# NVIDIA/makani

Measured on AMD Instinct MI355X. Metric: SFNO train samples/sec at 721x1440x73ch, higher is better.
Workload: dtype bf16; 1 GPU; sfno_sc3_layers8_edim384; grid=721x1440, channels=73, global_batch=1, parallelism=dp1, spectral_arithmetic=x3, multistep_count=1, multistep_checkpoint=False, launch=hipGraph replay of the captured step, channel_gemm=hip (csrc/conv1x1.hip)

## Files before the change

include/makani_amd.h:

```cpp
#ifndef MAKANI_AMD_H
#define MAKANI_AMD_H

#ifdef __cplusplus
extern "C" {
#endif

#define MK_F32 0
#define MK_BF16 1

#define MK_EINVAL -1
#define MK_EUNSUP -2

#define MK_TRI_NONE 0
#define MK_TRI_ROW_GE 1
#define MK_TRI_K_GE 2
#define MK_TRI_ROW_LE 3
#define MK_TRI_K_LE 4

typedef struct MkGemm {
    const float* A;
    const float* B;
    float* C;
    long long a_batch, a_row, a_k;
    long long b_batch, b_col, b_k;
    long long c_batch, c_row, c_col;
    long long a_inner, b_inner, c_inner;
    long long a_im, b_im, c_im;
    int M, N, K, batch;
    int inner;
    int tri_mode;
    int tri_off;
    int conj_a, conj_b;
    int beta;
} MkGemm;

const char* mk_last_error(void);
int mk_version(void);

int mk_sgemm_batched(const MkGemm* g, void* stream);
int mk_cgemm_batched(const MkGemm* g, void* stream);
int mk_sgemm_split_batched(const MkGemm* g, int limbs, void* stream);
int mk_cgemm_split_batched(const MkGemm* g, int limbs, void* stream);
int mk_cgemm_split2_batched(const MkGemm* g, int limbs, void* stream);
long long mk_cgemm_split2_ssq_count(const MkGemm* g);
int mk_cgemm_split2_batched_ssq(const MkGemm* g, int limbs, float* ssq_part, void* stream);
int mk_sgemm_presplit_batched(const MkGemm* g, const void* a_planes, long long pl_stride, long long pl_batch,
                              long long pl_k, int limbs, const int* band_lo, const int* band_hi, int band_mode,
                              void* stream);

int mk_vlegendre(const void* planes0, const void* planes1, long long pl_stride, long long pl_batch, long long pl_k,
                 int limbs, const float* in, float* out, int mode, int rows, int K, int orders, int Rp, int tri_off,
                 const int* band_lo, const int* band_hi, void* stream);

int mk_rfft_rows(const void* x, int x_dtype, float* F, const float* twiddle, const int* radix, int nradix,
                 int B, int C, int Cp, int nlat, int nlon, int mmax, float w_dc, float w_pos, float w_nyq,
                 void* stream);
int mk_irfft_rows(const float* F, void* x, int x_dtype, const float* twiddle, const int* radix, int nradix,
                  int B, int C, int Cp, int nlat, int nlon, int mmax, float w_dc, float w_pos, float w_nyq,
                  void* stream);

#define MK_FFT_SEG_MAX 8
typedef struct MkFftSeg {
    int nw, nh;
    int m_off[MK_FFT_SEG_MAX + 1];
    int r_off[MK_FFT_SEG_MAX + 1];
    long long base[MK_FFT_SEG_MAX][MK_FFT_SEG_MAX];
    int xseg;
    long long x_stride;
    int x_nlat;
} MkFftSeg;
int mk_fft_seg_supported(int nlon);
int mk_rfft_rows_seg(const void* x, int x_dtype, float* F, const float* twiddle, int C, int nlat, int nlon, int mmax,
                     float w_dc, float w_pos, float w_nyq, const MkFftSeg* seg, void* stream);
int mk_irfft_rows_seg(const float* F, void* x, int x_dtype, const float* twiddle, int C, int nlat, int nlon, int mmax,
                      float w_dc, float w_pos, float w_nyq, const MkFftSeg* seg, void* stream);

int mk_weight_to_wlayout(const float* w_c64, float* W, int cin, int cout, int cip, int cop, int L, void* stream);
int mk_wlayout_to_weight_grad(const float* gW, float* gw_c64, int cin, int cout, int cip, int cop, int L, void* stream);
int mk_slayout_to_complex(const float* S, float* out_c64, int B, int C, int Cp, int L, int M, int l_off, int m_off,
                          void* stream);
int mk_complex_to_slayout(const float* in_c64, float* S, int B, int C, int Cp, int L, int M, void* stream);

int mk_pointwise_chunks(long long hw, int dtype, long long planes);
int mk_plane_sums(const void* x, int dtype, float* sums, float* ws, long long planes, long long hw, void* stream);
int mk_instnorm_stats(const void* x, int dtype, float* stats, float* ws, long long planes, long long hw, float eps,
                      const float* quad, float quad_sum, void* stream);
int mk_instnorm_merge(const float* all_stats, const float* counts, float* stats, long long planes, int nranks, float eps,
                      void* stream);
int mk_instnorm_apply(const void* x, void* y, int dtype, const float* stats, const float* gamma, const float* beta,
                      long long planes, int channels, long long hw, int fuse_gelu, void* stream);
int mk_instnorm_fwd(const void* x, void* y, int dtype, float* stats, float* ws, const float* gamma, const float* beta,
                    const float* pre_bias, const float* quad, float quad_sum, long long planes, int channels, long long hw,
                    float eps, int fuse_gelu, void* stream);
int mk_instnorm_bwd(const void* x, const void* gy, void* gx, int dtype, const float* stats, const float* gamma,
                    const float* beta, const float* pre_bias, const float* quad, float quad_sum, float* sums, float* ws, long long planes, int channels, long long hw,
                    long long hw_total, int phase, int fuse_gelu, void* stream);
int mk_instnorm_fused_chunks(long long hw, int dtype, long long planes, int kind);
int mk_instnorm_fwd_fused(const void* x, void* y, int dtype, float* stats, const float* gamma, const float* beta,
                          const float* pre_bias, void* slots, void* depart, long long planes, int channels, long long hw,
                          float eps, int fuse_gelu, void* stream);
int mk_instnorm_bwd_fused(const void* x, const void* gy, void* gx, int dtype, const float* stats, const float* gamma,
                          const float* beta, const float* pre_bias, float* sums, void* slots, void* depart, long long planes,
                          int channels, long long hw, int fuse_gelu, void* stream);
int mk_bias_gelu_fwd(const void* x, const float* bias, void* y, int dtype, long long planes, int channels,
                     long long hw, void* stream);
int mk_bias_gelu_bwd(const void* x, const float* bias, const void* gy, void* gx, float* sums, float* ws, int dtype,
                     long long planes, int channels, long long hw, void* stream);

int mk_quad_lp_chunks(long long hw);
int mk_quad_lp_fwd(const void* a, int a_dtype, const void* b, int b_dtype, const float* wgt, const float* q,
                   float* sums, float* ws, long long planes, long long hw, int mode, float p, void* stream);
int mk_quad_lp_bwd(const void* a, int a_dtype, const void* b, int b_dtype, const float* wgt, const float* q,
                   const float* g, void* da, void* db, long long planes, long long hw, int mode, float p, void* stream);

long long mk_spec_lp_blocks(int L, int M);
int mk_spec_lp_fwd(const float* S, const float* wgt, float* partial, int L, int M, long long R, int tri_off, int m_off,
                   float p, float w0, float w1, void* stream);
int mk_spec_lp_bwd(const float* S, const float* wgt, const float* g, float* dS, int L, int M, long long R, int tri_off,
                   int m_off, float p, float w0, float w1, void* stream);

int mk_spec_sep_mul(const float* x, const float* w, float* y, int L, int M, int Mw, int B, int Cp, int tri_off, int conj_w,
                    void* stream);
int mk_spec_sep_wgrad(const float* x, const float* gy, float* gw, int L, int M, int Mw, int B, int Cp, int tri_off, void* stream);
int mk_spec_diag_apply(const float* x, const float* w_c64, float* y, int L, int M, int B, int Cin, int Cout, int x_ld, int y_ld,
                       int y_pad, int tri_off, int dgrad, void* stream);
int mk_spec_diag_wgrad(const float* x, const float* gy, float* gw_c64, int L, int M, int B, int Cin, int Cout, int x_ld, int y_ld,
                       int tri_off, void* stream);

int mk_conv1x1_nn(const void* A, const void* X, void* Y, void* Ypre, const float* bias, const void* R, const void* G,
                  int M, int K, int lda, int B, long long N, int act, void* stream);
long long mk_conv1x1_wgrad_workspace(int M, int K, int B, long long N);
int mk_conv1x1_wgrad(const void* G, const void* X, float* dW, float* part, int M, int K, int B, long long N,
                     int accumulate, void* stream);
int mk_conv1x1_wgrad_fuses_bias(int M, int K, int B, long long N);
int mk_conv1x1_wgrad_bias(const void* G, const void* X, float* dW, float* dbias, float* part, int M, int K, int B, long long N,
                          int accumulate, void* stream);

int mk_adamw_step(float* p, const float* g, float* m, float* v, long long n, const float* grad_scale, float lr,
                  float beta1, float beta2, float eps, float weight_decay, int step, const float* step_state, void* stream);
int mk_adamw_advance(float* state, float beta1, float beta2, void* stream);
typedef struct MkAdamTensor {
    float* p;
    const float* g;
    float* m;
    float* v;
    long long n;
    void* p_bf16;
    void* p_bf16_t;
    int cols;
    int ld, ld_t;
} MkAdamTensor;
int mk_adamw_multi(const MkAdamTensor* tensors, int count, const float* grad_scale, float lr, float beta1, float beta2,
                   float eps, float weight_decay, int step, const float* step_state, void* stream);
long long mk_grad_norm_workspace(const MkAdamTensor* tensors, int count);
int mk_grad_clip_coef(const MkAdamTensor* tensors, int count, float max_norm, float* partial, float* out, void* stream);
long long mk_grad_norm_workspace_pre(const MkAdamTensor* tensors, int count, const MkAdamTensor* pre, int npre);
int mk_grad_clip_coef_pre(const MkAdamTensor* tensors, int count, const MkAdamTensor* pre, int npre, float max_norm, float* partial,
                          float* out, void* stream);

int mk_chan_layernorm_chunks(int C, long long P);
int mk_chan_layernorm_fwd(const void* x, int x_dtype, void* y, int y_dtype, float* stats, const float* gamma, const float* beta,
                          int B, int C, long long P, float eps, void* stream);
int mk_chan_layernorm_bwd(const void* x, int x_dtype, const void* gy, int g_dtype, void* gx, const float* stats,
                          const float* gamma, int B, int C, long long P, void* stream);
int mk_chan_layernorm_wgrad(const void* x, int x_dtype, const void* gy, int g_dtype, const float* stats, float* partial, int B,
                            int C, long long P, void* stream);

int mk_crps_chunks(long long hw);
int mk_crps(const void* f, int f_dtype, const void* obs, int o_dtype, const float* q, const float* w, const float* gout,
            float* partial, void* gf, int B, int E, int C, long long hw, int type, float alpha, float eps, int grad,
            const float* ens_w, void* stream);
int mk_crps_complex(const void* f, const void* obs, const float* q, const float* w, const float* gout, float* partial, void* gf,
                    int B, int E, int C, long long hw, float alpha, int grad, void* stream);

long long mk_escore_sums_workspace(int B, int E, int C, long long N, int S, int nanmode);
int mk_escore_sums(const void* f, int kind, const void* obs, const float* q, const float* w, float* sums, float* ws, int B, int E,
                   int C, long long N, int S, int nanmode, float p, void* stream);
int mk_escore_finish(const float* sums, const float* scale, int nscale, float* loss, float* table, int B, int E, int C, int S,
                     int reduce, float p, float beta, float alpha, float eps, void* stream);
int mk_escore_grad(const void* f, int kind, const void* obs, const float* q, const float* w, const float* table, const float* gout,
                   void* gf, int B, int E, int C, int Cout, long long N, int S, int nanmode, float p, void* stream);

int mk_mmd_finish(const float* sums, float* loss, float* table, int B, int E, int C, int reduce, float sigma, float alpha, void* stream);

int mk_amse_sums(const float* X, const float* Y, const float* wgt, float* sums, long long R, int L, int M, int tri_off, int m_off,
                 void* stream);
int mk_amse_grad(const float* X, const float* Y, const float* wgt, const float* t, float* dX, float* dY, long long R, int L, int M,
                 int tri_off, int m_off, void* stream);

int mk_ens_nll_chunks(long long hw);
int mk_ens_nll(const void* f, int f_dtype, const float* obs, const float* q, const float* w, const float* gout, float* partial, void* gf,
               int B, int E, int C, long long hw, float eps, int grad, void* stream);

#define MK_NOISE_WHITE 0
#define MK_NOISE_AR 1
#define MK_NOISE_REPLACE 2
int mk_noise_update(float* state, const float* xi, const float* sigma, const float* phi, const long long* rng, int mode, int B,
                    int T, int C, int L, int M, int reflect, void* stream);
int mk_noise_advance(long long* rng, long long n, void* stream);

int mk_disco_fwd(const void* x, void* y, int dtype, const int* off, const int* nrow, const int* nlon, const float* nval,
                 const int* lat_lo, const int* lat_n, int max_rows, int planes, int K, int nlat_in, int nlon_in,
                 int nlat_out, int nlon_out, void* stream);
int mk_disco_bwd(const void* gy, void* gx, int dtype, const int* off, const int* nk, const int* nt, const int* nlon,
                 const float* nval, int planes, int K, int nlat_in, int nlon_in, int nlat_out, int nlon_out, void* stream);
int mk_disco_bwd_same(const void* gy, void* gx, int dtype, const int* off, const int* nrow, const int* nlon_l,
                      const float* nval, const int* t_lo, const int* t_n, int max_rows, int planes, int K, int nlat_in,
                      int nlon, int nlat_out, void* stream);
int mk_disco_runs_shape(int nlon, int max_rows, int planes, int dtype, int img_bf16, int* R_out, int* PB_out);
int mk_disco_fused_shape(int nlon, int K, int max_rows, int planes, int* LG_out, int* PB_out);
int mk_disco_fwd_fused(const void* x, void* y, int dtype, const int* seg_off, const int* runs, const float* vals,
                       const int* lat_lo, const int* lat_n, int max_rows, int planes, int K, int nlat_in, int nlon, int nlat_out,
                       void* stream);
int mk_disco_fwd_runs(const void* x, void* y, int dtype, const int* seg_off, const int* runs, const float* vals,
                      const int* lat_lo, const int* lat_n, int max_rows, int planes, int K, int nlat_in, int nlon, int nlat_out,
                      int R, int PB, int img_bf16, void* stream);
int mk_disco_bwd_runs(const void* gy, void* gx, int dtype, const int* seg_off, const int* runs, const float* vals,
                      const int* t_lo, const int* t_n, int max_rows, int planes, int K, int nlat_in, int nlon, int nlat_out,
                      int R, int PB, int img_bf16, int lat_group, void* stream);
int mk_group_mix_supported(int CG, int RG);
int mk_group_mix_blocks(long long N, int dtype, int BG);
int mk_group_mix(const void* x, const float* W, void* z, int dtype, int B, int G, int CG, int RG, long long N, void* stream);
int mk_group_mix_wgrad(const void* x, const void* dz, float* partial, int dtype, int B, int G, int CG, int RG, long long N,
                       void* stream);
int mk_resample_fwd(const void* x, void* y, int dtype, const int* lat_a, const int* lat_b, const float* lat_w,
                    const int* lon_l, const int* lon_r, const float* lon_w, int planes, int nlat_in, int nlon_in,
                    int nlat_out, int nlon_out, void* stream);
int mk_resample_bwd(const void* gy, void* gx, int dtype, const int* lat_off, const int* lat_t, const float* lat_wt,
                    const int* lon_off, const int* lon_p, const float* lon_wt, const int* pole_off, const int* pole_t,
                    const float* pole_wt, int planes, int nlat_in, int nlon_in, int nlat_out, int nlon_out, void* stream);

#ifdef __cplusplus
}
#endif
#endif
```

makani_amd/_lib.py:

```python
import ctypes as C
import os

import torch

_HERE = os.path.dirname(os.path.abspath(__file__))
LIB_PATH = os.environ.get("MAKANI_AMD_LIB") or os.path.join(_HERE, "libmakani_amd.so")

MK_F32, MK_BF16 = 0, 1
TRI_NONE, TRI_ROW_GE, TRI_K_GE, TRI_ROW_LE, TRI_K_LE = 0, 1, 2, 3, 4

c_ll, c_int, c_f, c_vp = C.c_longlong, C.c_int, C.c_float, C.c_void_p


class MkAdamTensor(C.Structure):
    _fields_ = [("p", C.c_void_p), ("g", C.c_void_p), ("m", C.c_void_p), ("v", C.c_void_p), ("n", C.c_longlong),
                ("p_bf16", C.c_void_p), ("p_bf16_t", C.c_void_p), ("cols", C.c_int), ("ld", C.c_int), ("ld_t", C.c_int)]


class MkGemm(C.Structure):
    _fields_ = [
        ("A", c_vp), ("B", c_vp), ("C", c_vp),
        ("a_batch", c_ll), ("a_row", c_ll), ("a_k", c_ll),
        ("b_batch", c_ll), ("b_col", c_ll), ("b_k", c_ll),
        ("c_batch", c_ll), ("c_row", c_ll), ("c_col", c_ll),
        ("a_inner", c_ll), ("b_inner", c_ll), ("c_inner", c_ll),
        ("a_im", c_ll), ("b_im", c_ll), ("c_im", c_ll),
        ("M", c_int), ("N", c_int), ("K", c_int), ("batch", c_int),
        ("inner", c_int), ("tri_mode", c_int), ("tri_off", c_int),
        ("conj_a", c_int), ("conj_b", c_int), ("beta", c_int),
    ]


MK_FFT_SEG_MAX = 8


class MkFftSeg(C.Structure):
    _fields_ = [("nw", c_int), ("nh", c_int), ("m_off", c_int * (MK_FFT_SEG_MAX + 1)), ("r_off", c_int * (MK_FFT_SEG_MAX + 1)),
                ("base", (c_ll * MK_FFT_SEG_MAX) * MK_FFT_SEG_MAX), ("xseg", c_int), ("x_stride", c_ll), ("x_nlat", c_int)]


_SIGS = {
    "mk_version": ([], c_int),
    "mk_sgemm_batched": ([C.POINTER(MkGemm), c_vp], c_int),
    "mk_cgemm_batched": ([C.POINTER(MkGemm), c_vp], c_int),
    "mk_sgemm_split_batched": ([C.POINTER(MkGemm), c_int, c_vp], c_int),
    "mk_cgemm_split_batched": ([C.POINTER(MkGemm), c_int, c_vp], c_int),
    "mk_cgemm_split2_batched": ([C.POINTER(MkGemm), c_int, c_vp], c_int),
    "mk_cgemm_split2_ssq_count": ([C.POINTER(MkGemm)], c_ll),
    "mk_cgemm_split2_batched_ssq": ([C.POINTER(MkGemm), c_int, c_vp, c_vp], c_int),
    "mk_sgemm_presplit_batched": ([C.POINTER(MkGemm), c_vp, c_ll, c_ll, c_ll, c_int, c_vp, c_vp, c_int, c_vp], c_int),
    "mk_vlegendre": ([c_vp, c_vp, c_ll, c_ll, c_ll, c_int, c_vp, c_vp, c_int, c_int, c_int, c_int, c_int, c_int, c_vp, c_vp, c_vp], c_int),
    "mk_rfft_rows": ([c_vp, c_int, c_vp, c_vp, C.POINTER(c_int), c_int, c_int, c_int, c_int, c_int, c_int, c_int,
                      c_f, c_f, c_f, c_vp], c_int),
    "mk_irfft_rows": ([c_vp, c_vp, c_int, c_vp, C.POINTER(c_int), c_int, c_int, c_int, c_int, c_int, c_int, c_int,
                       c_f, c_f, c_f, c_vp], c_int),
    "mk_fft_seg_supported": ([c_int], c_int),
    "mk_rfft_rows_seg": ([c_vp, c_int, c_vp, c_vp, c_int, c_int, c_int, c_int, c_f, c_f, c_f, C.POINTER(MkFftSeg), c_vp], c_int),
    "mk_irfft_rows_seg": ([c_vp, c_vp, c_int, c_vp, c_int, c_int, c_int, c_int, c_f, c_f, c_f, C.POINTER(MkFftSeg), c_vp], c_int),
    "mk_weight_to_wlayout": ([c_vp, c_vp, c_int, c_int, c_int, c_int, c_int, c_vp], c_int),
    "mk_wlayout_to_weight_grad": ([c_vp, c_vp, c_int, c_int, c_int, c_int, c_int, c_vp], c_int),
    "mk_slayout_to_complex": ([c_vp, c_vp, c_int, c_int, c_int, c_int, c_int, c_int, c_int, c_vp], c_int),
    "mk_complex_to_slayout": ([c_vp, c_vp, c_int, c_int, c_int, c_int, c_int, c_vp], c_int),
    "mk_spec_sep_mul": ([c_vp, c_vp, c_vp, c_int, c_int, c_int, c_int, c_int, c_int, c_int, c_vp], c_int),
    "mk_spec_sep_wgrad": ([c_vp, c_vp, c_vp, c_int, c_int, c_int, c_int, c_int, c_int, c_vp], c_int),
    "mk_spec_diag_apply": ([c_vp, c_vp, c_vp, c_int, c_int, c_int, c_int, c_int, c_int, c_int, c_int, c_int, c_int, c_vp], c_int),
    "mk_spec_diag_wgrad": ([c_vp, c_vp, c_vp, c_int, c_int, c_int, c_int, c_int, c_int, c_int, c_int, c_vp], c_int),
    "mk_pointwise_chunks": ([c_ll, c_int, c_ll], c_int),
    "mk_plane_sums": ([c_vp, c_int, c_vp, c_vp, c_ll, c_ll, c_vp], c_int),
    "mk_instnorm_stats": ([c_vp, c_int, c_vp, c_vp, c_ll, c_ll, c_f, c_vp, c_f, c_vp], c_int),
    "mk_instnorm_merge": ([c_vp, c_vp, c_vp, c_ll, c_int, c_f, c_vp], c_int),
    "mk_instnorm_apply": ([c_vp, c_vp, c_int, c_vp, c_vp, c_vp, c_ll, c_int, c_ll, c_int, c_vp], c_int),
    "mk_instnorm_fused_chunks": ([c_ll, c_int, c_ll, c_int], c_int),
    "mk_instnorm_fwd_fused": ([c_vp, c_vp, c_int, c_vp, c_vp, c_vp, c_vp, c_vp, c_vp, c_ll, c_int, c_ll, c_f, c_int, c_vp], c_int),
    "mk_instnorm_bwd_fused": ([c_vp, c_vp, c_vp, c_int, c_vp, c_vp, c_vp, c_vp, c_vp, c_vp, c_vp, c_ll, c_int, c_ll, c_int, c_vp], c_int),
    "mk_instnorm_bwd": ([c_vp, c_vp, c_vp, c_int, c_vp, c_vp, c_vp, c_vp, c_vp, c_f, c_vp, c_vp, c_ll, c_int, c_ll, c_ll, c_int, c_int, c_vp], c_int),
    "mk_chan_layernorm_chunks": ([c_int, c_ll], c_int),
    "mk_chan_layernorm_fwd": ([c_vp, c_int, c_vp, c_int, c_vp, c_vp, c_vp, c_int, c_int, c_ll, c_f, c_vp], c_int),
    "mk_chan_layernorm_bwd": ([c_vp, c_int, c_vp, c_int, c_vp, c_vp, c_vp, c_int, c_int, c_ll, c_vp], c_int),
    "mk_chan_layernorm_wgrad": ([c_vp, c_int, c_vp, c_int, c_vp, c_vp, c_int, c_int, c_ll, c_vp], c_int),
    "mk_bias_gelu_fwd": ([c_vp, c_vp, c_vp, c_int, c_ll, c_int, c_ll, c_vp], c_int),
    "mk_conv1x1_nn": ([c_vp, c_vp, c_vp, c_vp, c_vp, c_vp, c_vp, c_int, c_int, c_int, c_int, c_ll, c_int, c_vp], c_int),
    "mk_conv1x1_wgrad_workspace": ([c_int, c_int, c_int, c_ll], c_ll),
    "mk_conv1x1_wgrad": ([c_vp, c_vp, c_vp, c_vp, c_int, c_int, c_int, c_ll, c_int, c_vp], c_int),
    "mk_conv1x1_wgrad_fuses_bias": ([c_int, c_int, c_int, c_ll], c_int),
    "mk_conv1x1_wgrad_bias": ([c_vp, c_vp, c_vp, c_vp, c_vp, c_int, c_int, c_int, c_ll, c_int, c_vp], c_int),
    "mk_adamw_step": ([c_vp, c_vp, c_vp, c_vp, c_ll, c_vp, c_f, c_f, c_f, c_f, c_f, c_int, c_vp, c_vp], c_int),
    "mk_adamw_advance": ([c_vp, c_f, c_f, c_vp], c_int),
    "mk_bias_gelu_bwd": ([c_vp, c_vp, c_vp, c_vp, c_vp, c_vp, c_int, c_ll, c_int, c_ll, c_vp], c_int),
    "mk_adamw_multi": ([c_vp, c_int, c_vp, c_f, c_f, c_f, c_f, c_f, c_int, c_vp, c_vp], c_int),
    "mk_instnorm_fwd": ([c_vp, c_vp, c_int, c_vp, c_vp, c_vp, c_vp, c_vp, c_vp, c_f, c_ll, c_int, c_ll, c_f, c_int, c_vp], c_int),
    "mk_grad_norm_workspace": ([c_vp, c_int], c_ll),
    "mk_grad_clip_coef": ([c_vp, c_int, c_f, c_vp, c_vp, c_vp], c_int),
    "mk_grad_norm_workspace_pre": ([c_vp, c_int, c_vp, c_int], c_ll),
    "mk_grad_clip_coef_pre": ([c_vp, c_int, c_vp, c_int, c_f, c_vp, c_vp, c_vp], c_int),
    "mk_spec_lp_blocks": ([c_int, c_int], c_ll),
    "mk_spec_lp_fwd": ([c_vp, c_vp, c_vp, c_int, c_int, c_ll, c_int, c_int, c_f, c_f, c_f, c_vp], c_int),
    "mk_spec_lp_bwd": ([c_vp, c_vp, c_vp, c_vp, c_int, c_int, c_ll, c_int, c_int, c_f, c_f, c_f, c_vp], c_int),
    "mk_crps_chunks": ([c_ll], c_int),
    "mk_crps": ([c_vp, c_int, c_vp, c_int, c_vp, c_vp, c_vp, c_vp, c_vp, c_int, c_int, c_int, c_ll, c_int, c_f, c_f, c_int, c_vp, c_vp], c_int),
    "mk_crps_complex": ([c_vp, c_vp, c_vp, c_vp, c_vp, c_vp, c_vp, c_int, c_int, c_int, c_ll, c_f, c_int, c_vp], c_int),
    "mk_escore_sums_workspace": ([c_int, c_int, c_int, c_ll, c_int, c_int], c_ll),
    "mk_escore_sums": ([c_vp, c_int, c_vp, c_vp, c_vp, c_vp, c_vp, c_int, c_int, c_int, c_ll, c_int, c_int, c_f, c_vp], c_int),
    "mk_escore_finish": ([c_vp, c_vp, c_int, c_vp, c_vp, c_int, c_int, c_int, c_int, c_int, c_f, c_f, c_f, c_f, c_vp], c_int),
    "mk_escore_grad": ([c_vp, c_int, c_vp, c_vp, c_vp, c_vp, c_vp, c_vp, c_int, c_int, c_int, c_int, c_ll, c_int, c_int, c_f, c_vp], c_int),
    "mk_mmd_finish": ([c_vp, c_vp, c_vp, c_int, c_int, c_int, c_int, c_f, c_f, c_vp], c_int),
    "mk_amse_sums": ([c_vp, c_vp, c_vp, c_vp, c_ll, c_int, c_int, c_int, c_int, c_vp], c_int),
    "mk_amse_grad": ([c_vp, c_vp, c_vp, c_vp, c_vp, c_vp, c_ll, c_int, c_int, c_int, c_int, c_vp], c_int),
    "mk_ens_nll_chunks": ([c_ll], c_int),
    "mk_ens_nll": ([c_vp, c_int, c_vp, c_vp, c_vp, c_vp, c_vp, c_vp, c_int, c_int, c_int, c_ll, c_f, c_int, c_vp], c_int),
    "mk_noise_update": ([c_vp, c_vp, c_vp, c_vp, c_vp, c_int, c_int, c_int, c_int, c_int, c_int, c_int, c_vp], c_int),
    "mk_noise_advance": ([c_vp, c_ll, c_vp], c_int),
    "mk_disco_fwd": ([c_vp, c_vp, c_int, c_vp, c_vp, c_vp, c_vp, c_vp, c_vp, c_int, c_int, c_int, c_int, c_int, c_int, c_int, c_vp], c_int),
    "mk_disco_bwd": ([c_vp, c_vp, c_int, c_vp, c_vp, c_vp, c_vp, c_vp, c_int, c_int, c_int, c_int, c_int, c_int, c_vp], c_int),
    "mk_disco_bwd_same": ([c_vp, c_vp, c_int, c_vp, c_vp, c_vp, c_vp, c_vp, c_vp, c_int, c_int, c_int, c_int, c_int, c_int, c_vp], c_int),
    "mk_disco_runs_shape": ([c_int, c_int, c_int, c_int, c_int, c_vp, c_vp], c_int),
    "mk_disco_fused_shape": ([c_int, c_int, c_int, c_int, c_vp, c_vp], c_int),
    "mk_disco_fwd_fused": ([c_vp, c_vp, c_int, c_vp, c_vp, c_vp, c_vp, c_vp, c_int, c_int, c_int, c_int, c_int, c_int, c_vp], c_int),
    "mk_disco_fwd_runs": ([c_vp, c_vp, c_int, c_vp, c_vp, c_vp, c_vp, c_vp, c_int, c_int, c_int, c_int, c_int, c_int, c_int, c_int, c_int, c_vp], c_int),
    "mk_disco_bwd_runs": ([c_vp, c_vp, c_int, c_vp, c_vp, c_vp, c_vp, c_vp, c_int, c_int, c_int, c_int, c_int, c_int, c_int, c_int, c_int, c_int, c_vp], c_int),
    "mk_group_mix_supported": ([c_int, c_int], c_int),
    "mk_group_mix_blocks": ([c_ll, c_int, c_int], c_int),
    "mk_group_mix": ([c_vp, c_vp, c_vp, c_int, c_int, c_int, c_int, c_int, c_ll, c_vp], c_int),
    "mk_group_mix_wgrad": ([c_vp, c_vp, c_vp, c_int, c_int, c_int, c_int, c_int, c_ll, c_vp], c_int),
    "mk_resample_fwd": ([c_vp, c_vp, c_int, c_vp, c_vp, c_vp, c_vp, c_vp, c_vp, c_int, c_int, c_int, c_int, c_int, c_vp], c_int),
    "mk_resample_bwd": ([c_vp, c_vp, c_int, c_vp, c_vp, c_vp, c_vp, c_vp, c_vp, c_vp, c_vp, c_vp, c_int, c_int, c_int, c_int, c_int, c_vp], c_int),
    "mk_quad_lp_chunks": ([c_ll], c_int),
    "mk_quad_lp_fwd": ([c_vp, c_int, c_vp, c_int, c_vp, c_vp, c_vp, c_vp, c_ll, c_ll, c_int, c_f, c_vp], c_int),
    "mk_quad_lp_bwd": ([c_vp, c_int, c_vp, c_int, c_vp, c_vp, c_vp, c_vp, c_vp, c_ll, c_ll, c_int, c_f, c_vp], c_int),
}

EXPORTS = sorted(list(_SIGS) + ["mk_last_error"])

_lib = None


def lib():
    global _lib
    if _lib is None:
        if not os.path.exists(LIB_PATH):
            raise RuntimeError(
                f"{LIB_PATH} is missing: the MI355X HIP library has not been built "
                "(run `python -m makani_amd.build`).  There is no CPU fallback."
            )
        L = C.CDLL(LIB_PATH)
        for name, (args, res) in _SIGS.items():
            fn = getattr(L, name)
            fn.argtypes = args
            fn.restype = res
        L.mk_last_error.argtypes = []
        L.mk_last_error.restype = C.c_char_p
        _lib = L
    return _lib


def check(rc, what=""):
    if rc != 0:
        msg = lib().mk_last_error().decode()
        raise RuntimeError(f"libmakani_amd {what} failed (code {rc}): {msg}")


def stream():
    return c_vp(torch.cuda.current_stream().cuda_stream)


def device_guard(fn):
    import functools

    @functools.wraps(fn)
    def wrapped(self, *args, **kwargs):
        for a in (*args, *kwargs.values()):
            if isinstance(a, torch.Tensor) and a.is_cuda:
                if a.device.index != torch.cuda.current_device():
                    with torch.cuda.device(a.device):
                        return fn(self, *args, **kwargs)
                break
        return fn(self, *args, **kwargs)

    return wrapped


def ptr(t):
    if t is None:
        return c_vp(0)
    if not t.is_cuda:
        raise RuntimeError("makani_amd ops need GPU tensors (the HIP path has no CPU fallback)")
    return c_vp(t.data_ptr())


def dtype_code(t):
    if t.dtype == torch.float32:
        return MK_F32
    if t.dtype == torch.bfloat16:
        return MK_BF16
    raise TypeError(f"unsupported dtype {t.dtype} (float32 / bfloat16 only)")


def dense_view(t):
    if t.is_contiguous():
        return t
    order = sorted(range(t.dim()), key=lambda d: (-t.stride(d), -t.size(d)))
    v = t.permute(order)
    return v if v.is_contiguous() else None
```

makani_amd/csrc/conv1x1.hip:

```cpp
#include <stdlib.h>
#include <type_traits>

#include "common.h"
#include "conv1x1_plan.h"

#ifndef MK_ASTAT_DIAG
#define MK_ASTAT_DIAG 0
#endif
#if MK_ASTAT_DIAG
__device__ unsigned long long g_astat_diag[16];
#define MK_AS_STAMP(k)                                              \
    do {                                                            \
        const unsigned long long t_ = __builtin_readcyclecounter(); \
        dg[k] += t_ - tprev;                                        \
        tprev = t_;                                                 \
    } while (0)
#else
#define MK_AS_STAMP(k)
#endif

namespace {

typedef __bf16 bf16x8 __attribute__((ext_vector_type(8)));
typedef __attribute__((address_space(3))) s16x4 lds_s16x4;

constexpr int NT = 256;

struct ConvNN {
    const u16* A;
    const u16* X;
    u16* Y;
    u16* Ypre;
    const float* bias;
    const u16* R;
    const u16* G;
    int M, K, lda, B;
    long long N;
    int act;
    int nt;
};

__device__ __forceinline__ uint4 ld16(const u16* p) { return *reinterpret_cast<const uint4*>(p); }
__device__ __forceinline__ void mk_st16(u16* p, uint4 v, int nt) {
    typedef unsigned int u32x4_nt __attribute__((ext_vector_type(4)));
    if (nt) __builtin_nontemporal_store(u32x4_nt{v.x, v.y, v.z, v.w}, reinterpret_cast<u32x4_nt*>(p));
    else *reinterpret_cast<uint4*>(p) = v;
}
#define MK_BUF_ST16(VAL, RS, VOFF, NT)                                            \
    do {                                                                          \
        if (NT) __builtin_amdgcn_raw_buffer_store_b128(VAL, RS, VOFF, 0, 2);      \
        else __builtin_amdgcn_raw_buffer_store_b128(VAL, RS, VOFF, 0, 0);         \
    } while (0)

typedef __attribute__((address_space(3))) void lds_void_t;
typedef int v4i_t __attribute__((ext_vector_type(4)));

template <int N_> __device__ __forceinline__ void wait_vmcnt() { asm volatile("s_waitcnt vmcnt(%0)" ::"n"(N_) : "memory"); }

__device__ __forceinline__ v4i_t make_rsrc(const void* ptr) {
    const unsigned long long a = (unsigned long long)ptr;
    v4i_t r;
    r[0] = __builtin_amdgcn_readfirstlane((int)(unsigned)a);
    r[1] = __builtin_amdgcn_readfirstlane((int)(unsigned)(a >> 32));
    r[2] = (int)0x80000000u;
    r[3] = 0x00020000;
    return r;
}
__device__ __forceinline__ v4i_t make_rsrc_n(const void* ptr, unsigned bytes) {
    v4i_t r = make_rsrc(ptr);
    r[2] = __builtin_amdgcn_readfirstlane((int)bytes);
    return r;
}
__device__ __forceinline__ unsigned lds_addr(const void* ptr) { return (unsigned)(unsigned long long)(lds_void_t*)ptr; }

template <int STEP>
__device__ __forceinline__ void dma4(unsigned lds0, v4i_t rs, unsigned soff, unsigned v0, unsigned v1, unsigned v2, unsigned v3) {
    unsigned keep;
    asm volatile(
        "s_mov_b32 %0, m0\n\ts_nop 4\n\t"
        "s_mov_b32 m0, %1\n\ts_nop 0\n\tbuffer_load_dwordx4 %4, %2, %3 offen lds\n\t"
        "s_add_u32 m0, m0, %8\n\ts_nop 0\n\tbuffer_load_dwordx4 %5, %2, %3 offen lds\n\t"
        "s_add_u32 m0, m0, %8\n\ts_nop 0\n\tbuffer_load_dwordx4 %6, %2, %3 offen lds\n\t"
        "s_add_u32 m0, m0, %8\n\ts_nop 0\n\tbuffer_load_dwordx4 %7, %2, %3 offen lds\n\t"
        "s_mov_b32 m0, %0"
        : "=&s"(keep)
        : "s"(lds0), "s"(rs), "s"(soff), "v"(v0), "v"(v1), "v"(v2), "v"(v3), "i"(STEP)
        : "memory", "scc");
}
__device__ __forceinline__ void dma1(unsigned lds0, v4i_t rs, unsigned soff, unsigned v0) {
    unsigned keep;
    asm volatile(
        "s_mov_b32 %0, m0\n\ts_nop 4\n\t"
        "s_mov_b32 m0, %1\n\ts_nop 0\n\tbuffer_load_dwordx4 %4, %2, %3 offen lds\n\t"
        "s_mov_b32 m0, %0"
        : "=&s"(keep)
        : "s"(lds0), "s"(rs), "s"(soff), "v"(v0)
        : "memory");
}
template <int STEP>
__device__ __forceinline__ void dma2(unsigned lds0, v4i_t rs, unsigned soff, unsigned v0, unsigned v1) {
    unsigned keep;
    asm volatile(
        "s_mov_b32 %0, m0\n\ts_nop 4\n\t"
        "s_mov_b32 m0, %1\n\ts_nop 0\n\tbuffer_load_dwordx4 %4, %2, %3 offen lds\n\t"
        "s_add_u32 m0, m0, %6\n\ts_nop 0\n\tbuffer_load_dwordx4 %5, %2, %3 offen lds\n\t"
        "s_mov_b32 m0, %0"
        : "=&s"(keep)
        : "s"(lds0), "s"(rs), "s"(soff), "v"(v0), "v"(v1), "i"(STEP)
        : "memory", "scc");
}
template <int STEP>
__device__ __forceinline__ void dma3(unsigned lds0, v4i_t rs, unsigned soff, unsigned v0, unsigned v1, unsigned v2) {
    unsigned keep;
    asm volatile(
        "s_mov_b32 %0, m0\n\ts_nop 4\n\t"
        "s_mov_b32 m0, %1\n\ts_nop 0\n\tbuffer_load_dwordx4 %4, %2, %3 offen lds\n\t"
        "s_add_u32 m0, m0, %7\n\ts_nop 0\n\tbuffer_load_dwordx4 %5, %2, %3 offen lds\n\t"
        "s_add_u32 m0, m0, %7\n\ts_nop 0\n\tbuffer_load_dwordx4 %6, %2, %3 offen lds\n\t"
        "s_mov_b32 m0, %0"
        : "=&s"(keep)
        : "s"(lds0), "s"(rs), "s"(soff), "v"(v0), "v"(v1), "v"(v2), "i"(STEP)
        : "memory", "scc");
}

template <int BM, int BN, int DEPTH, int BKT, int WGS>
__global__ __launch_bounds__(NT, WGS) void conv_nn_kernel(const ConvNN p, int tilesM, long long tilesN) {
    constexpr int WM = BM / 2, WN = BN / 2;
    constexpr int TM = WM / 32, TN = WN / 32;
    constexpr int BK = BKT;
    constexpr int LDSB = (BKT == 32) ? 2 : 1;
    constexpr int PA = BK + 8;
    constexpr int PB = BN + 32;
    constexpr int NA = (BM * BK / 8) / NT;
    constexpr int NB_ = (BK * BN / 8) / NT;
    constexpr int PE = BN + 4;
    static_assert(NA >= 1 && NB_ >= 1, "tile too small");
    static_assert(WM == 64, "the epilogue stages one wave row (64 output channels) at a time");
    constexpr int OPER = LDSB * (BM * PA + BK * PB) * 2;
    constexpr int EPI = WM * PE * 4;
    __shared__ __attribute__((aligned(16))) unsigned char smem_raw[OPER > EPI ? OPER : EPI];
    u16* As = reinterpret_cast<u16*>(smem_raw);
    u16* Bs = As + LDSB * BM * PA;
    float* Es = reinterpret_cast<float*>(smem_raw);

    const long long bid = xcd_remap(blockIdx.x, gridDim.x);
    const int tm = (int)(bid % tilesM);
    const long long tnb = bid / tilesM;
    const int b = (int)(tnb / tilesN);
    const long long tn = tnb % tilesN;
    const int m0 = tm * BM;
    const long long n0 = tn * BN;

    const int tid = threadIdx.x, lane = tid & 63, wave = tid >> 6;
    const int wm = wave >> 1, wn = wave & 1;
    const int l31 = lane & 31, lh = lane >> 5;

    const u16* Xb = p.X + (long long)b * p.K * p.N;

    f32x16 acc[TM][TN];
#pragma unroll
    for (int i = 0; i < TM; ++i)
#pragma unroll
        for (int j = 0; j < TN; ++j)
#pragma unroll
            for (int r = 0; r < 16; ++r) acc[i][j][r] = 0.f;

    uint4 ra[DEPTH][NA], rb[DEPTH][NB_];
    const bool tile_full = (m0 + BM <= p.M) && (n0 + BN <= p.N);
    auto load_tiles = [&](uint4* qa, uint4* qb, int k0) {
        if (tile_full && k0 + BK <= p.K) {
#pragma unroll
            for (int q = 0; q < NA; ++q) {
                const int f = tid + q * NT;
                qa[q] = ld16(p.A + (long long)(m0 + f / (BK / 8)) * p.lda + k0 + (f % (BK / 8)) * 8);
            }
#pragma unroll
            for (int q = 0; q < NB_; ++q) {
                const int f = tid + q * NT;
                qb[q] = ld16(Xb + (long long)(k0 + f / (BN / 8)) * p.N + n0 + (f % (BN / 8)) * 8);
            }
            return;
        }
#pragma unroll
        for (int q = 0; q < NA; ++q) {
            const int f = tid + q * NT;
            const int row = f / (BK / 8), c = f % (BK / 8);
            uint4 v = make_uint4(0, 0, 0, 0);
            if (m0 + row < p.M && k0 + c * 8 < p.lda) v = ld16(p.A + (long long)(m0 + row) * p.lda + k0 + c * 8);
            qa[q] = v;
        }
#pragma unroll
        for (int q = 0; q < NB_; ++q) {
// ... 540 lines not shown
        for (int kc = 0; kc < NCH; ++kc) {
            const int c = ts * NCH + kc;
            const int nfull = (LOOK - kc + NCH - 1) / NCH;
            if (c + LOOK > nchunks) {
                wait_vmcnt<0>();
            } else if (SMALLK && EPI_LOADS) {
                if (ts < LOOK) wait_vmcnt<0>(); else wait_vmcnt_le<SMALLK_EPI_WAIT>();
            } else if (EPI_LOADS) {
                if (ts < NEPI_MAX) {
                    wait_vmcnt<0>();
                } else if (kc == 0) {
                    if (nfull == 1) wait_vmcnt_le<NP * (LOOK - 1) + NSTORE>();
                    else if (nfull == 2) wait_vmcnt_le<NP * (LOOK - 1) + 2 * NSTORE + EPIECES>();
                    else wait_vmcnt_le<NP * (LOOK - 1) + 3 * NSTORE + 2 * EPIECES>();
                } else {
                    if (nfull == 1) wait_vmcnt_le<NP * (LOOK - 1) + NSTORE + EPIECES>();
                    else if (nfull == 2) wait_vmcnt_le<NP * (LOOK - 1) + 2 * NSTORE + 2 * EPIECES>();
                    else wait_vmcnt_le<NP * (LOOK - 1) + 3 * NSTORE + 3 * EPIECES>();
                }
            } else {
                const int nepi = min(nfull, ts);
                if (nepi == 0) wait_vmcnt_le<NP * (LOOK - 1)>();
                else if (nepi == 1) wait_vmcnt_le<NP * (LOOK - 1) + NSTORE>();
                else if (nepi == 2) wait_vmcnt_le<NP * (LOOK - 1) + 2 * NSTORE>();
                else wait_vmcnt_le<NP * (LOOK - 1) + 3 * NSTORE>();
            }
            __builtin_amdgcn_s_barrier();
            MK_AS_STAMP(0);
            if (EPI_LOADS && kc == 0) issue_epi(cn0);
            const unsigned char* sb = smem + c_slot * CH;
            c_slot = c_slot + 1 == NSLOT ? 0 : c_slot + 1;
#pragma unroll
            for (int k4 = 0; k4 < K4; ++k4) {
                bf16x8 xf[TN];
#pragma unroll
                for (int j = 0; j < TN; ++j) {
                    const unsigned char* q0 = sb + xoff[j] + k4 * 16 * 128;
                    const s16x4 lo = __builtin_amdgcn_ds_read_tr16_b64_v4i16((lds_s16x4*)(q0));
                    const s16x4 hi = __builtin_amdgcn_ds_read_tr16_b64_v4i16((lds_s16x4*)(q0 + 4 * 128));
                    const s16x8 v = {lo[0], lo[1], lo[2], lo[3], hi[0], hi[1], hi[2], hi[3]};
                    xf[j] = __builtin_bit_cast(bf16x8, v);
                }
#pragma unroll
                for (int i = 0; i < TM; ++i)
#pragma unroll
                    for (int j = 0; j < TN; ++j)
                        acc[i][j] = __builtin_amdgcn_mfma_f32_32x32x16_bf16(xf[j], af[i][kc * K4 + k4], acc[i][j], 0, 0, 0);
            }
#if MK_ASTAT_DIAG
            asm volatile("s_nop 0" : "+v"(acc[TM - 1][TN - 1]));
#endif
            MK_AS_STAMP(1);
            if (c + LOOK < nchunks) issue_next();
            MK_AS_STAMP(2);
        }

        if constexpr (EPI_LOADS) {
            if ((ts + 1) * NCH - 1 + LOOK < nchunks) wait_vmcnt_le<NP * NCH>(); else wait_vmcnt<0>();
        }
#pragma unroll
        for (int i = 0; i < TM; ++i) {
            unsigned voff[4];
#pragma unroll
            for (int u4 = 0; u4 < 4; ++u4) {
                const int idx = tid + NT_ * u4;
                const int row = idx >> 3, ch = idx & 7;
                const int m = slab * BM + (row >> 5) * (TM * 32) + i * 32 + (row & 31);
                const long long n = cn0 + ch * 8;
                const bool live = m < p.M && n < p.N;
                const long long o = (long long)m * p.N + n;
                voff[u4] = live ? (unsigned)(o * 2) : 0xC0000000u;
            }
            const float bv = bvr[i];
            const int lrow = wave * 32 + l31;
#pragma unroll
            for (int j = 0; j < TN; ++j)
#pragma unroll
                for (int q = 0; q < 4; ++q) {
                    const int px = j * 32 + 8 * q + 4 * lh;
                    uint2 u;
                    u.x = pack_bf16x2(acc[i][j][4 * q] + bv, acc[i][j][4 * q + 1] + bv);
                    u.y = pack_bf16x2(acc[i][j][4 * q + 2] + bv, acc[i][j][4 * q + 3] + bv);
                    *reinterpret_cast<uint2*>(stg + lrow * 128 + (((px >> 3) ^ ((lrow >> 1) & 7)) * 16) + ((px >> 2) & 1) * 8) = u;
                }
            asm volatile("s_waitcnt lgkmcnt(0)" ::: "memory");
            MK_AS_STAMP(3);
            __builtin_amdgcn_s_barrier();
            MK_AS_STAMP(4);
#pragma unroll
            for (int u4 = 0; u4 < 4; ++u4) {
                const int idx = tid + NT_ * u4;
                const int row = idx >> 3, ch = idx & 7;
                const uint4 raw = *reinterpret_cast<const uint4*>(stg + row * 128 + ((ch ^ ((row >> 1) & 7)) * 16));
                typedef unsigned int u32x4_t __attribute__((ext_vector_type(4)));
                if (PRE) MK_BUF_ST16((u32x4_t{raw.x, raw.y, raw.z, raw.w}), rsP, voff[u4], nt_st);
                uint4 ev = make_uint4(0, 0, 0, 0);
                if constexpr (EPI_LOADS) ev = *reinterpret_cast<const uint4*>(ebuf + i * 16384 + row * 128 + ch * 16);
                uint4 out = raw;
                if (p.act || EPI_LOADS) {
                    const uint32_t w[4] = {raw.x, raw.y, raw.z, raw.w};
                    float v[8];
#pragma unroll
                    for (int e = 0; e < 4; ++e) {
                        v[2 * e] = __uint_as_float(w[e] << 16);
                        v[2 * e + 1] = __uint_as_float(w[e] & 0xffff0000u);
                    }
                    if (p.act) {
                        gelu_fast_n<8>(v);
                    }
                    if (EPI_LOADS && p.G) {
                        const uint32_t gw[4] = {ev.x, ev.y, ev.z, ev.w};
#pragma unroll
                        for (int e = 0; e < 4; ++e) {
                            const float ga2[2] = {__uint_as_float(gw[e] << 16), __uint_as_float(gw[e] & 0xffff0000u)};
                            float gd2[2];
                            gelu_grad_fast_n<2>(ga2, gd2);
                            v[2 * e] *= gd2[0];
                            v[2 * e + 1] *= gd2[1];
                        }
                    }
                    if (EPI_LOADS && !p.G) {
                        const uint32_t rw[4] = {ev.x, ev.y, ev.z, ev.w};
#pragma unroll
                        for (int e = 0; e < 4; ++e) {
                            v[2 * e] += __uint_as_float(rw[e] << 16);
                            v[2 * e + 1] += __uint_as_float(rw[e] & 0xffff0000u);
                        }
                    }
                    out.x = pack_bf16x2(v[0], v[1]);
                    out.y = pack_bf16x2(v[2], v[3]);
                    out.z = pack_bf16x2(v[4], v[5]);
                    out.w = pack_bf16x2(v[6], v[7]);
                }
                MK_BUF_ST16((u32x4_t{out.x, out.y, out.z, out.w}), rsY, voff[u4], nt_st);
            }
            asm volatile("s_waitcnt lgkmcnt(0)" ::: "memory");
            MK_AS_STAMP(5);
            __builtin_amdgcn_s_barrier();
            MK_AS_STAMP(6);
        }
    }
#if MK_ASTAT_DIAG
    if (lane == 0) {
#pragma unroll
        for (int k = 0; k < 8; ++k) atomicAdd(&g_astat_diag[k], dg[k]);
        atomicAdd(&g_astat_diag[8], tprev - tstart);
        atomicAdd(&g_astat_diag[9], 1ull);
        atomicAdd(&g_astat_diag[10], (unsigned long long)my_tiles);
    }
#endif
#endif
}

template <bool PRE, bool EPI_LOADS>
__global__ __launch_bounds__(512) void conv_nn_astat2_kernel(const ConvNN p, int slabs, long long tilesN) {
#if defined(__HIP_DEVICE_COMPILE__)
    typedef float f32x4_t __attribute__((ext_vector_type(4)));
    constexpr int KS = 12;
    constexpr int KCH = 128, NCH = 3, K4 = 4;
    constexpr int CH = KCH * 128;
    constexpr int NSLOT = 4, NP = 2;
    constexpr int PT = 4, CT = 3;
    constexpr int PER = 7, OFF = 3;
    constexpr int NS3 = 2 * (PRE ? 2 : 1);
    constexpr int EPIECES = EPI_LOADS ? 6 : 0;
    constexpr int WA[2][3] = {{3, 2, 1}, {3, 2, 1}};
    constexpr int WB[2][3] = {{3, 2, 1}, {3, 1, 2}};
    constexpr int WE[2][3] = {{1, 1, 1}, {1, 0, 0}};
#define MK_A2_WAIT(G, K) (WA[G][K] * NP + WB[G][K] * NS3 + WE[G][K] * EPIECES)
    static_assert(MK_A2_WAIT(0, 0) <= 63 && MK_A2_WAIT(1, 2) <= 63, "vmcnt is a 6-bit counter");
    constexpr int EBYTES = EPI_LOADS ? 2 * 192 * 128 : 0;
    __shared__ __attribute__((aligned(1024))) unsigned char smem[NSLOT * CH + 2 * 192 * 128 + EBYTES];
    unsigned char* const stg = smem + NSLOT * CH;
    unsigned char* const ebuf = stg + 2 * 192 * 128;

    const int tid = threadIdx.x, lane = tid & 63;
    const bool nt_st = p.nt != 0;
    const int wave = __builtin_amdgcn_readfirstlane(tid >> 6);
    const int grp = wave >> 2, wg = wave & 3;
    const int c16 = lane & 15, q4 = lane >> 4;
#if MK_ASTAT_DIAG
    unsigned long long dg[8] = {0, 0, 0, 0, 0, 0, 0, 0};
    unsigned long long tprev = __builtin_readcyclecounter();
    const unsigned long long tstart = tprev;
#endif
    auto lane_here = [&]() __attribute__((always_inline)) {
        int l = lane;
        asm volatile("" : "+v"(l));
        return l;
    };

    const int vid = xcd_remap(blockIdx.x, gridDim.x);
    const int slab = vid % slabs;
    const int pstride = gridDim.x / slabs;
    const int pfirst = vid / slabs;
    const int tilesN32 = (int)tilesN;
    const int T = pfirst < tilesN32 ? (tilesN32 - pfirst + pstride - 1) / pstride : 0;
    const int nchunks = NCH * T;
    const int cb = blockIdx.y;
    const int m_base = slab * 384 + wave * 48;
    const unsigned nbytes = (unsigned)(p.N * 2);

    bf16x8 wf[CT][KS];
#pragma unroll
    for (int ct = 0; ct < CT; ++ct) {
        const int row = min(m_base + ct * 16 + c16, p.M - 1);
        const u16* src = p.A + (long long)row * p.lda + q4 * 8;
#pragma unroll
        for (int ks = 0; ks < KS; ++ks) wf[ct][ks] = __builtin_bit_cast(bf16x8, ld16(src + ks * 32));
    }
    float bvr[CT];
#pragma unroll
    for (int ct = 0; ct < CT; ++ct) {
        const int mrow = m_base + ct * 16 + c16;
        bvr[ct] = (p.bias && mrow < p.M) ? p.bias[mrow] : 0.f;
    }
#pragma unroll
    for (int ct = 0; ct < CT; ++ct) {
#pragma unroll
        for (int ks = 0; ks < KS; ++ks) asm volatile("" : "+v"(wf[ct][ks]));
        asm volatile("" : "+v"(bvr[ct]));
    }

    const unsigned lds0 = lds_addr(smem) + (unsigned)wave * (NP * 1024);
    const v4i_t rsX = make_rsrc(p.X + (long long)cb * p.K * p.N);
    const unsigned kstride = (unsigned)KCH * nbytes;
    auto issue_chunk = [&](int ts, int kc, int slot) __attribute__((always_inline)) {
        const unsigned n0b = (unsigned)(pfirst + ts * pstride) * 128u;
        const int cmax = min(7, (int)((nbytes - n0b) / 16) - 1);
        const unsigned soff = (unsigned)__builtin_amdgcn_readfirstlane((int)((unsigned)kc * kstride + n0b));
        const int ln = lane_here();
        const int c0 = (ln & 7) ^ ((((ln >> 3) >> 1) & 1) << 2), c1 = c0 ^ 2;
        const unsigned r0 = (unsigned)(wave * 16 + (ln >> 3)) * nbytes;
        dma2<1024>((unsigned)__builtin_amdgcn_readfirstlane((int)(lds0 + (unsigned)slot * CH)), rsX, soff,
                   r0 + (unsigned)min(c0, cmax) * 16u, r0 + 8u * nbytes + (unsigned)min(c1, cmax) * 16u);
    };

    const u16* const eop = p.G ? p.G : p.R;
    const v4i_t rsE = make_rsrc(EPI_LOADS ? (const void*)(eop + (long long)cb * p.M * p.N) : (const void*)p.X);
    const unsigned ldsE = lds_addr(ebuf) + (unsigned)grp * (192 * 128) + (unsigned)wg * (6 * 1024);
    auto issue_epi = [&](int ts) __attribute__((always_inline)) {
        const unsigned n0b = (unsigned)(pfirst + ts * pstride) * 128u;
        const int cmax = min(7, (int)((nbytes - n0b) / 16) - 1);
        const int ln = lane_here();
        const unsigned col = (unsigned)min(ln & 7, cmax) * 16u;
        const unsigned soff = (unsigned)__builtin_amdgcn_readfirstlane((int)n0b);
        const unsigned le = (unsigned)__builtin_amdgcn_readfirstlane((int)ldsE);
#pragma unroll
        for (int h = 0; h < 2; ++h) {
            unsigned v[3];
#pragma unroll
            for (int q = 0; q < 3; ++q) {
                const int r = 48 * wg + 8 * (3 * h + q) + (ln >> 3);
                v[q] = (unsigned)min(slab * 384 + 192 * grp + r, p.M - 1) * nbytes + col;
            }
            dma3<1024>(le + (unsigned)h * 3072u, rsE, soff, v[0], v[1], v[2]);
            __builtin_amdgcn_sched_barrier(0);
        }
    };

    int xoff[PT];
    {
        const int kk = q4 * 8 + (c16 >> 2);
        const int swz = ((((kk >> 1) & 1) << 2) ^ ((q4 & 1) << 1));
#pragma unroll
        for (int pt = 0; pt < PT; ++pt) xoff[pt] = kk * 128 + (((2 * pt + ((c16 & 3) >> 1)) ^ swz) * 16) + (c16 & 1) * 8;
    }

    f32x4_t acc[PT][CT];
    const long long plane0 = (long long)cb * p.M * p.N;
    const __amdgpu_buffer_rsrc_t rsY = __builtin_amdgcn_make_buffer_rsrc((void*)(p.Y + plane0), 0, 0x80000000u, 0x00020000);
    const __amdgpu_buffer_rsrc_t rsP = __builtin_amdgcn_make_buffer_rsrc((void*)((PRE ? p.Ypre : p.Y) + plane0), 0, 0x80000000u, 0x00020000);
    unsigned char* const stgG = stg + grp * (192 * 128);
    const unsigned char* const ebufG = ebuf + grp * (192 * 128);

    auto mult = [&](int ts, auto kc_) __attribute__((always_inline)) {
        constexpr int kc = decltype(kc_)::value;
        if constexpr (kc == 0) {
#pragma unroll
            for (int pt = 0; pt < PT; ++pt)
#pragma unroll
                for (int ct = 0; ct < CT; ++ct) acc[pt][ct] = f32x4_t{0.f, 0.f, 0.f, 0.f};
        }
        const unsigned char* sb = smem + ((NCH * ts + kc) & (NSLOT - 1)) * CH;
        auto frags = [&](bf16x8* xf, int sub) __attribute__((always_inline)) {
            const int k4 = sub >> 1, hp = sub & 1;
#pragma unroll
            for (int j = 0; j < 2; ++j) {
                const unsigned char* q0 = sb + xoff[2 * hp + j] + k4 * 32 * 128;
                const s16x4 lo = __builtin_amdgcn_ds_read_tr16_b64_v4i16((lds_s16x4*)(q0));
                const s16x4 hi = __builtin_amdgcn_ds_read_tr16_b64_v4i16((lds_s16x4*)(q0 + 4 * 128));
                const s16x8 v = {lo[0], lo[1], lo[2], lo[3], hi[0], hi[1], hi[2], hi[3]};
                xf[j] = __builtin_bit_cast(bf16x8, v);
            }
        };
        bf16x8 xf[2][2];
        frags(xf[0], 0);
        __builtin_amdgcn_s_setprio(1);
#pragma unroll
        for (int sub = 0; sub < 2 * K4; ++sub) {
            if (sub + 1 < 2 * K4) frags(xf[(sub + 1) & 1], sub + 1);
            const int k4 = sub >> 1, hp = sub & 1;
#pragma unroll
            for (int ct = 0; ct < CT; ++ct)
#pragma unroll
                for (int j = 0; j < 2; ++j)
                    acc[2 * hp + j][ct] = __builtin_amdgcn_mfma_f32_16x16x32_bf16(xf[sub & 1][j], wf[ct][kc * K4 + k4], acc[2 * hp + j][ct], 0, 0, 0);
            __builtin_amdgcn_sched_barrier(0);
        }
        __builtin_amdgcn_s_setprio(0);
    };
    auto stage = [&]() __attribute__((always_inline)) {
        const int ln = lane_here();
        const int c16 = ln & 15, q4 = ln >> 4;
#pragma unroll
        for (int ct = 0; ct < CT; ++ct) {
            const float bv = bvr[ct];
            const int lrow = ct * 64 + wg * 16 + c16;
#pragma unroll
            for (int pt = 0; pt < PT; ++pt) {
                uint2 u;
                u.x = pack_bf16x2(acc[pt][ct][0] + bv, acc[pt][ct][1] + bv);
                u.y = pack_bf16x2(acc[pt][ct][2] + bv, acc[pt][ct][3] + bv);
                const int chunk = 2 * pt + (q4 >> 1);
                *reinterpret_cast<uint2*>(stgG + lrow * 128 + ((chunk ^ ((lrow >> 1) & 7)) * 16) + (q4 & 1) * 8) = u;
            }
        }
    };
    auto readback_store = [&](int ts, int ct) __attribute__((always_inline)) {
        const unsigned cn0b = (unsigned)(pfirst + ts * pstride) * 128u;
        typedef unsigned int u32x4_t __attribute__((ext_vector_type(4)));
        const int tg = (wg << 6) | lane_here();
#pragma unroll
        for (int u2 = 0; u2 < 2; ++u2) {
            const int idx = tg + 256 * u2;
            const int row = idx >> 3, ch = idx & 7;
            const int srow = ct * 64 + row;
            const int grow = (row >> 4) * 48 + ct * 16 + (row & 15);
            const int m = slab * 384 + grp * 192 + grow;
            const unsigned nb = cn0b + (unsigned)ch * 16u;
            const bool live = m < p.M && nb < nbytes;
            const unsigned voff = live ? (unsigned)m * nbytes + nb : 0xC0000000u;
            const uint4 raw = *reinterpret_cast<const uint4*>(stgG + srow * 128 + ((ch ^ ((srow >> 1) & 7)) * 16));
            if (PRE) MK_BUF_ST16((u32x4_t{raw.x, raw.y, raw.z, raw.w}), rsP, voff, nt_st);
            uint4 ev = make_uint4(0, 0, 0, 0);
            if constexpr (EPI_LOADS) ev = *reinterpret_cast<const uint4*>(ebufG + grow * 128 + ch * 16);
            uint4 out = raw;
            if (p.act || EPI_LOADS) {
                const uint32_t w[4] = {raw.x, raw.y, raw.z, raw.w};
                float v[8];
#pragma unroll
                for (int e = 0; e < 4; ++e) {
                    v[2 * e] = __uint_as_float(w[e] << 16);
                    v[2 * e + 1] = __uint_as_float(w[e] & 0xffff0000u);
                }
                if (p.act) {
                    gelu_fast_n<8>(v);
                }
                if (EPI_LOADS && p.G) {
                    const uint32_t gw[4] = {ev.x, ev.y, ev.z, ev.w};
#pragma unroll
                    for (int e = 0; e < 4; ++e) {
                        const float ga2[2] = {__uint_as_float(gw[e] << 16), __uint_as_float(gw[e] & 0xffff0000u)};
                        float gd2[2];
                        gelu_grad_fast_n<2>(ga2, gd2);
                        v[2 * e] *= gd2[0];
                        v[2 * e + 1] *= gd2[1];
                    }
                }
                if (EPI_LOADS && !p.G) {
                    const uint32_t rw[4] = {ev.x, ev.y, ev.z, ev.w};
#pragma unroll
                    for (int e = 0; e < 4; ++e) {
                        v[2 * e] += __uint_as_float(rw[e] << 16);
                        v[2 * e + 1] += __uint_as_float(rw[e] & 0xffff0000u);
                    }
                }
                out.x = pack_bf16x2(v[0], v[1]);
                out.y = pack_bf16x2(v[2], v[3]);
                out.z = pack_bf16x2(v[4], v[5]);
                out.w = pack_bf16x2(v[6], v[7]);
            }
            MK_BUF_ST16((u32x4_t{out.x, out.y, out.z, out.w}), rsY, voff, nt_st);
        }
    };

    using I0 = std::integral_constant<int, 0>;
    using I1 = std::integral_constant<int, 1>;
    using I2 = std::integral_constant<int, 2>;

    MK_AS_STAMP(7);
    for (int c = 0; c < NSLOT && c < nchunks; ++c) issue_chunk(c / NCH, c % NCH, c);

    auto tick = [&](int gts, auto gph_, auto grp_) __attribute__((always_inline)) {
        constexpr int gph = decltype(gph_)::value, g = decltype(grp_)::value;
        if constexpr (gph < NCH) {
            if (gts < T) {
                if (gts <= 1 || gts >= T - 1) wait_vmcnt<0>(); else wait_vmcnt<MK_A2_WAIT(g, gph)>();
            }
        }
        asm volatile("s_waitcnt lgkmcnt(0)" ::: "memory");
        __builtin_amdgcn_s_barrier();
        MK_AS_STAMP(0);
    };
    auto tick_end = [&](int gts, auto gph_) __attribute__((always_inline)) {
        constexpr int gph = decltype(gph_)::value;
        if constexpr (gph > OFF) {
            const int ts = gts + (gph == 6 ? 2 : 1);
            if (ts < T) issue_chunk(ts, gph == 6 ? 0 : gph - 3, (NCH * gts + gph) & (NSLOT - 1));
        }
        MK_AS_STAMP(2);
    };
    auto tile = [&](int lts, auto grp_) __attribute__((always_inline)) {
        constexpr int g = decltype(grp_)::value;
#define MK_A2_TICK(P) tick(lts + ((P) + OFF * g) / PER, std::integral_constant<int, ((P) + OFF * g) % PER>{}, grp_)
#define MK_A2_END(P) tick_end(lts + ((P) + OFF * g) / PER, std::integral_constant<int, ((P) + OFF * g) % PER>{})
#if MK_ASTAT_DIAG
#define MK_A2_SEG(K) do { asm volatile("s_waitcnt lgkmcnt(0)" ::: "memory"); asm volatile("s_nop 0" : "+v"(acc[PT - 1][CT - 1])); MK_AS_STAMP(K); } while (0)
#else
#define MK_A2_SEG(K)
#endif
        MK_A2_TICK(0);
        if constexpr (EPI_LOADS) issue_epi(lts);
        MK_AS_STAMP(2);
        mult(lts, I0{});
        MK_A2_SEG(1);
        MK_A2_END(0);
        MK_A2_TICK(1);
        mult(lts, I1{});
        MK_A2_SEG(1);
        MK_A2_END(1);
        MK_A2_TICK(2);
        mult(lts, I2{});
        MK_A2_SEG(1);
        MK_A2_END(2);
        MK_A2_TICK(3);
        stage();
        MK_A2_SEG(3);
        MK_A2_END(3);
        if constexpr (EPI_LOADS) {
            if (g == 0 || lts >= T - 2) wait_vmcnt<0>(); else wait_vmcnt<3 * NP>();
        }
        MK_A2_TICK(4);
        MK_AS_STAMP(4);
        readback_store(lts, 0);
        MK_A2_SEG(5);
        MK_A2_END(4);
        MK_A2_TICK(5);
        readback_store(lts, 1);
        MK_A2_SEG(5);
        MK_A2_END(5);
        MK_A2_TICK(6);
        readback_store(lts, 2);
        MK_A2_SEG(5);
        MK_A2_END(6);
#undef MK_A2_SEG
#undef MK_A2_TICK
#undef MK_A2_END
    };
    if (T > 0) {
        if (grp == 0) {
            for (int lts = 0; lts < T; ++lts) tile(lts, I0{});
            tick(T, I0{}, I0{});
            tick(T, I1{}, I0{});
            tick(T, I2{}, I0{});
        } else {
            tick(0, I0{}, I1{});
            tick(0, I1{}, I1{});
            tick(0, I2{}, I1{});
            for (int lts = 0; lts < T; ++lts) tile(lts, I1{});
        }
    }
#if MK_ASTAT_DIAG
    if (lane == 0) {
#pragma unroll
        for (int q = 0; q < 8; ++q) atomicAdd(&g_astat_diag[q], dg[q]);
        atomicAdd(&g_astat_diag[8], tprev - tstart);
        atomicAdd(&g_astat_diag[9], 1ull);
        atomicAdd(&g_astat_diag[10], (unsigned long long)T);
    }
#endif
#undef MK_A2_WAIT
#endif
}

struct ConvWg {
    const u16* G;
    const u16* X;
    float* part;
    int M, K, B, S;
    long long N;
    long long chunk;
};

template <int BKT>
__global__ __launch_bounds__(NT, 2) void conv_wgrad_kernel(const ConvWg p, int tilesM, int tilesK) {
    constexpr int BM = 128, BN = 128;
    constexpr int BK = BKT;
    constexpr int LDSB = BKT == 64 ? 2 : 1, SETS = BKT == 64 ? 2 : 1;
    constexpr int PA = BK + 8;
    constexpr int NA = (BM * BK / 8) / NT;
    __shared__ __attribute__((aligned(16))) u16 smem[LDSB * (BM + BN) * PA];
    u16* As = smem;
    u16* Bs = smem + LDSB * BM * PA;

    const int bid = xcd_remap(blockIdx.x, gridDim.x);
    const int tm = bid % tilesM;
    const int tk = (bid / tilesM) % tilesK;
    const int sp = bid / (tilesM * tilesK);
    const int m0 = tm * BM, c0 = tk * BN;
    const int splits_per_b = p.S / p.B;
    const int b = sp / splits_per_b;
    const long long nbeg = (long long)(sp % splits_per_b) * p.chunk;
    const long long nend = min(p.N, nbeg + p.chunk);

    const int tid = threadIdx.x, lane = tid & 63, wave = tid >> 6;
    const int wm = wave >> 1, wn = wave & 1;
    const int l31 = lane & 31, lh = lane >> 5;
    const u16* Gb = p.G + (long long)b * p.M * p.N;
    const u16* Xb = p.X + (long long)b * p.K * p.N;

    f32x16 acc[2][2];
#pragma unroll
    for (int i = 0; i < 2; ++i)
#pragma unroll
        for (int j = 0; j < 2; ++j)
#pragma unroll
            for (int r = 0; r < 16; ++r) acc[i][j][r] = 0.f;

    uint4 ra[SETS][NA], rb[SETS][NA];
    const bool rows_full = (m0 + BM <= p.M) && (c0 + BN <= p.K);
    auto load_tiles = [&](uint4* qa, uint4* qb, long long n) {
        if (rows_full && n + BK <= nend) {
#pragma unroll
            for (int q = 0; q < NA; ++q) {
                const int f = tid + q * NT;
                const int row = f / (BK / 8), c = f % (BK / 8);
                qa[q] = ld16(Gb + (long long)(m0 + row) * p.N + n + c * 8);
                qb[q] = ld16(Xb + (long long)(c0 + row) * p.N + n + c * 8);
            }
            return;
        }
#pragma unroll
        for (int q = 0; q < NA; ++q) {
            const int f = tid + q * NT;
            const int row = f / (BK / 8), c = f % (BK / 8);
            uint4 va = make_uint4(0, 0, 0, 0), vb = make_uint4(0, 0, 0, 0);
            if (n + c * 8 < nend) {
                if (m0 + row < p.M) va = ld16(Gb + (long long)(m0 + row) * p.N + n + c * 8);
                if (c0 + row < p.K) vb = ld16(Xb + (long long)(c0 + row) * p.N + n + c * 8);
            }
            qa[q] = va;
            qb[q] = vb;
        }
    };
    auto store_tiles = [&](const uint4* qa, const uint4* qb, int buf) {
#pragma unroll
        for (int q = 0; q < NA; ++q) {
            const int f = tid + q * NT;
            const int row = f / (BK / 8), c = f % (BK / 8);
            *reinterpret_cast<uint4*>(As + buf * BM * PA + row * PA + c * 8) = qa[q];
            *reinterpret_cast<uint4*>(Bs + buf * BN * PA + row * PA + c * 8) = qb[q];
        }
    };
    const int a_off = (wm * 64 + l31) * PA + lh * 8;
    const int b_off = (wn * 64 + l31) * PA + lh * 8;
    auto compute = [&](int buf) {
        const u16* Ab = As + buf * BM * PA;
        const u16* Bb = Bs + buf * BN * PA;
#pragma unroll
        for (int ks = 0; ks < BK / 16; ++ks) {
            bf16x8 af[2], bfr[2];
#pragma unroll
            for (int i = 0; i < 2; ++i) {
                af[i] = __builtin_bit_cast(bf16x8, *reinterpret_cast<const s16x8*>(Ab + a_off + i * 32 * PA + ks * 16));
                bfr[i] = __builtin_bit_cast(bf16x8, *reinterpret_cast<const s16x8*>(Bb + b_off + i * 32 * PA + ks * 16));
            }
#pragma unroll
            for (int i = 0; i < 2; ++i)
#pragma unroll
                for (int j = 0; j < 2; ++j)
                    acc[i][j] = __builtin_amdgcn_mfma_f32_32x32x16_bf16(af[i], bfr[j], acc[i][j], 0, 0, 0);
        }
    };

    const int nk = (int)((nend - nbeg + BK - 1) / BK);
    if constexpr (SETS == 2) {
        if (nk > 0) load_tiles(ra[0], rb[0], nbeg);
        if (nk > 1) load_tiles(ra[1], rb[1], nbeg + BK);
        if (nk > 0) store_tiles(ra[0], rb[0], 0);
        __syncthreads();
        for (int kt = 0; kt < nk; kt += 2) {
            if (kt + 2 < nk) load_tiles(ra[0], rb[0], nbeg + (long long)(kt + 2) * BK);
            compute(0);
            if (kt + 1 < nk) store_tiles(ra[1], rb[1], 1);
            __syncthreads();
            if (kt + 1 >= nk) break;
            if (kt + 3 < nk) load_tiles(ra[1], rb[1], nbeg + (long long)(kt + 3) * BK);
            compute(1);
            if (kt + 2 < nk) store_tiles(ra[0], rb[0], 0);
            __syncthreads();
        }
    } else {
        if (nk > 0) {
            load_tiles(ra[0], rb[0], nbeg);
            store_tiles(ra[0], rb[0], 0);
        }
        __syncthreads();
        for (int kt = 0; kt < nk; ++kt) {
            if (kt + 1 < nk) load_tiles(ra[0], rb[0], nbeg + (long long)(kt + 1) * BK);
            compute(0);
            __syncthreads();
            if (kt + 1 < nk) {
                store_tiles(ra[0], rb[0], 0);
                __syncthreads();
            }
        }
    }

    float* out = p.part + (long long)sp * p.M * p.K;
#pragma unroll
    for (int i = 0; i < 2; ++i)
#pragma unroll
        for (int j = 0; j < 2; ++j) {
            const int c = c0 + wn * 64 + j * 32 + l31;
#pragma unroll
            for (int r = 0; r < 16; ++r) {
                const int m = m0 + wm * 64 + i * 32 + (r & 3) + 8 * (r >> 2) + 4 * lh;
                if (m < p.M && c < p.K) out[(long long)m * p.K + c] = acc[i][j][r];
            }
        }
}

struct ConvWgR {
    const u16* P;
    const u16* Q;
    float* part;
    int RP, RQ, B, S, slabs, qslabs;
// ... 57 lines not shown
        if constexpr (NIP == 4) dma4<8192>(dst, rsP, soff, v[0], v[1], v[2], v[3]);
        else dma3<8192>(dst, rsP, soff, v[0], v[1], v[2]);
        dma3<8192>(dst + NIP * 8192, rsQ, soff, v[NIP], v[NIP + 1], v[NIP + 2]);
        dma3<8192>(dst + (NIP + 3) * 8192, rsQ, soff, v[NIP + 3], v[NIP + 4], v[NIP + 5]);
    };

    const int swz = (l31 >> 1) & 7;
    int pa[4], qa[4];
#pragma unroll
    for (int ks = 0; ks < 4; ++ks) {
        const int ch = ((ks * 2 + lh) ^ swz) * 16;
        pa[ks] = (wp * WTP * 32 + l31) * 128 + ch;
        qa[ks] = (TP + wq * WTQ * 32 + l31) * 128 + ch;
    }

    f32x16 acc[WTP][WTQ];
#pragma unroll
    for (int i = 0; i < WTP; ++i)
#pragma unroll
        for (int j = 0; j < WTQ; ++j)
#pragma unroll
            for (int r = 0; r < 16; ++r) acc[i][j][r] = 0.f;

    constexpr int WTG = SWAP ? WTQ : WTP;
    constexpr int NSH = 1;
    const int bshare = 0;
    const bool bias_wave = p.bias_part != nullptr && (SWAP ? (wp == 0 && slab == 0) : (wq == 0 && qs == 0));
    float rsum[WTG];
#pragma unroll
    for (int i = 0; i < WTG; ++i) rsum[i] = 0.f;
    typedef __bf16 bf16x2_t __attribute__((ext_vector_type(2)));
    auto add8 = [](float s, bf16x8 v) {
        const bf16x2_t one = {(__bf16)1.0f, (__bf16)1.0f};
        s = __builtin_amdgcn_fdot2_f32_bf16(bf16x2_t{v[0], v[1]}, one, s, false);
        s = __builtin_amdgcn_fdot2_f32_bf16(bf16x2_t{v[2], v[3]}, one, s, false);
        s = __builtin_amdgcn_fdot2_f32_bf16(bf16x2_t{v[4], v[5]}, one, s, false);
        return __builtin_amdgcn_fdot2_f32_bf16(bf16x2_t{v[6], v[7]}, one, s, false);
    };

    auto compute = [&](int stage) {
        const unsigned char* sb = smem + stage * STAGE;
#pragma unroll
        for (int ks = 0; ks < 4; ++ks) {
            bf16x8 pf[WTP], qf[WTQ];
#pragma unroll
            for (int i = 0; i < WTP; ++i) pf[i] = __builtin_bit_cast(bf16x8, *reinterpret_cast<const s16x8*>(sb + pa[ks] + i * 4096));
#pragma unroll
            for (int j = 0; j < WTQ; ++j) qf[j] = __builtin_bit_cast(bf16x8, *reinterpret_cast<const s16x8*>(sb + qa[ks] + j * 4096));
            if (bias_wave && (ks & (NSH - 1)) == bshare) {
#pragma unroll
                for (int i = 0; i < WTG; ++i) rsum[i] = add8(rsum[i], SWAP ? qf[i] : pf[i]);
            }
#pragma unroll
            for (int i = 0; i < WTP; ++i)
#pragma unroll
                for (int j = 0; j < WTQ; ++j)
                    acc[i][j] = SWAP ? __builtin_amdgcn_mfma_f32_32x32x16_bf16(qf[j], pf[i], acc[i][j], 0, 0, 0)
                                     : __builtin_amdgcn_mfma_f32_32x32x16_bf16(pf[i], qf[j], acc[i][j], 0, 0, 0);
        }
    };

    if (nk > 0) issue(0, 0);
    if (nk > 1) issue(1, 1);
    for (int kt = 0; kt < nk; ++kt) {
        if (kt + 1 < nk) wait_vmcnt<NI>(); else wait_vmcnt<0>();
        __builtin_amdgcn_s_barrier();
        compute(kt & 1);
        asm volatile("s_waitcnt lgkmcnt(0)" ::: "memory");
        __builtin_amdgcn_s_barrier();
        if (kt + 2 < nk) issue(kt + 2, kt & 1);
    }

    if (bias_wave) {
        const int RG = SWAP ? p.RQ : p.RP;
#pragma unroll
        for (int i = 0; i < WTG; ++i) {
            const float tot = rsum[i] + __shfl_xor(rsum[i], 32);
            const int m = SWAP ? q0 + (wq * WTQ + i) * 32 + l31 : slab * TP + (wp * WTP + i) * 32 + l31;
            if (lh == 0 && m < RG) p.bias_part[((long long)sp * NSH + bshare) * RG + m] = tot;
        }
    }

    float* out = p.part + (long long)sp * ((long long)(SWAP ? p.RQ : p.RP) * p.ldo);
#pragma unroll
    for (int i = 0; i < WTP; ++i)
#pragma unroll
        for (int j = 0; j < WTQ; ++j) {
            const int prow0 = slab * TP + (wp * WTP + i) * 32, qrow0 = q0 + (wq * WTQ + j) * 32;
#pragma unroll
            for (int r = 0; r < 16; ++r) {
                const int rr = (r & 3) + 8 * (r >> 2) + 4 * lh;
                const int m = SWAP ? qrow0 + rr : prow0 + rr;
                const int k = SWAP ? prow0 + l31 : qrow0 + l31;
                const bool ok = SWAP ? (m < p.RQ && k < p.RP) : (m < p.RP && k < p.RQ);
                if (ok) out[(long long)m * p.ldo + k] = acc[i][j][r];
            }
        }
#endif
}

__global__ void reduce_splits(const float* __restrict__ part, float* __restrict__ out, long long n, int S, int accumulate) {
    const long long i = (long long)blockIdx.x * blockDim.x + threadIdx.x;
    if (i >= n) return;
    float s = accumulate ? out[i] : 0.f;
    int k = 0;
    for (; k + 8 <= S; k += 8) {
        float v[8];
#pragma unroll
        for (int u = 0; u < 8; ++u) v[u] = part[(long long)(k + u) * n + i];
#pragma unroll
        for (int u = 0; u < 8; ++u) s += v[u];
    }
    for (; k < S; ++k) s += part[(long long)k * n + i];
    out[i] = s;
}

__global__ void reduce_splits4(const float4* __restrict__ part, float4* __restrict__ out, long long n4, int S, int accumulate) {
    const long long i = (long long)blockIdx.x * blockDim.x + threadIdx.x;
    if (i >= n4) return;
    float4 s = accumulate ? out[i] : make_float4(0.f, 0.f, 0.f, 0.f);
    int k = 0;
    for (; k + 8 <= S; k += 8) {
        float4 v[8];
#pragma unroll
        for (int u = 0; u < 8; ++u) v[u] = part[(long long)(k + u) * n4 + i];
#pragma unroll
        for (int u = 0; u < 8; ++u) s.x += v[u].x, s.y += v[u].y, s.z += v[u].z, s.w += v[u].w;
    }
    for (; k < S; ++k) {
        const float4 v = part[(long long)k * n4 + i];
        s.x += v.x, s.y += v.y, s.z += v.z, s.w += v.w;
    }
    out[i] = s;
}

}

#if MK_ASTAT_DIAG
extern "C" int mk_astat_diag_read(unsigned long long* out, int reset) {
    if (hipMemcpyFromSymbol(out, HIP_SYMBOL(g_astat_diag), sizeof(unsigned long long) * 16) != hipSuccess) return 1;
    if (reset) {
        unsigned long long z[16] = {};
        if (hipMemcpyToSymbol(HIP_SYMBOL(g_astat_diag), z, sizeof(z)) != hipSuccess) return 1;
    }
    return 0;
}
#endif

static int env_int(const char* name) {
    const char* e = getenv(name);
    return e ? atoi(e) : -1;
}

extern "C" int mk_conv1x1_nn(const void* A, const void* X, void* Y, void* Ypre, const float* bias, const void* R,
                             const void* G, int M, int K, int lda, int B, long long N, int act, void* stream) {
    MK_REQUIRE(A && X && Y, "conv1x1_nn: null pointer");
    MK_REQUIRE(M > 0 && K > 0 && B > 0 && N > 0, "conv1x1_nn: bad shape M=%d K=%d B=%d N=%lld", M, K, B, N);
    MK_REQUIRE((lda % 8) == 0 && lda >= K, "conv1x1_nn: lda=%d must be a multiple of 8 and >= K=%d", lda, K);
    MK_REQUIRE((N % 8) == 0, "conv1x1_nn: pixel count %lld must be a multiple of 8", N);
    MK_REQUIRE((((uintptr_t)A | (uintptr_t)X) & 15) == 0, "conv1x1_nn: operands must be 16-byte aligned");
    static const int nt_env = env_int("MAKANI_AMD_CONV_NT"), astat2_env = env_int("MAKANI_AMD_ASTAT2");
    const long long out_bytes = (long long)B * M * N * 2;
    const int nt = nt_env == 0 ? 0 : (nt_env == 1 ? 1 : out_bytes <= (256ll << 20));
    ConvNN p{(const u16*)A, (const u16*)X, (u16*)Y, (u16*)Ypre, bias, (const u16*)R, (const u16*)G, M, K, lda, B, N, act, nt};
    hipStream_t s = (hipStream_t)stream;
    const bool pre = act && Ypre, epi_loads = R || G;
    const int slabs = (M + 383) / 384;
    const long long tn64 = (N + 63) / 64;
    auto stationary_grid = [&](int wgs) {
        const long long streams = tn64 < wgs / slabs ? tn64 : wgs / slabs;
        return dim3((unsigned)(streams * slabs), (unsigned)B);
    };
    switch (conv_nn_plan(M, K, lda, B, N, pre, R != nullptr, G != nullptr, astat2_env)) {
    case ConvNnKernel::astat73: {
        const dim3 grid = stationary_grid(epi_loads ? 256 : 512), blk(256);
        if (epi_loads) hipLaunchKernelGGL((conv_nn_astat_kernel<3, 96, false, true, 5>), grid, blk, 0, s, p, slabs, tn64);
        else if (pre) hipLaunchKernelGGL((conv_nn_astat_kernel<3, 96, true, false, 5>), grid, blk, 0, s, p, slabs, tn64);
        else hipLaunchKernelGGL((conv_nn_astat_kernel<3, 96, false, false, 5>), grid, blk, 0, s, p, slabs, tn64);
        break;
    }
    case ConvNnKernel::astat2: {
        const dim3 grid = stationary_grid(256), blk(512);
        if (epi_loads && pre) hipLaunchKernelGGL((conv_nn_astat2_kernel<true, true>), grid, blk, 0, s, p, slabs, tn64);
        else if (epi_loads) hipLaunchKernelGGL((conv_nn_astat2_kernel<false, true>), grid, blk, 0, s, p, slabs, tn64);
        else if (pre) hipLaunchKernelGGL((conv_nn_astat2_kernel<true, false>), grid, blk, 0, s, p, slabs, tn64);
        else hipLaunchKernelGGL((conv_nn_astat2_kernel<false, false>), grid, blk, 0, s, p, slabs, tn64);
        break;
    }
    case ConvNnKernel::astat1: {
        const dim3 grid = stationary_grid(256), blk(256);
#define MK_ASTAT(TM_, KCH_)                                                                                              \
    do {                                                                                                                  \
        if (epi_loads && pre) hipLaunchKernelGGL((conv_nn_astat_kernel<TM_, KCH_, true, true>), grid, blk, 0, s, p, slabs, tn64);   \
        else if (epi_loads) hipLaunchKernelGGL((conv_nn_astat_kernel<TM_, KCH_, false, true>), grid, blk, 0, s, p, slabs, tn64);    \
        else if (pre) hipLaunchKernelGGL((conv_nn_astat_kernel<TM_, KCH_, true, false>), grid, blk, 0, s, p, slabs, tn64);          \
        else hipLaunchKernelGGL((conv_nn_astat_kernel<TM_, KCH_, false, false>), grid, blk, 0, s, p, slabs, tn64);                  \
    } while (0)
        if (epi_loads) MK_ASTAT(3, 64);
        else MK_ASTAT(3, 128);
#undef MK_ASTAT
        break;
    }
    case ConvNnKernel::ring: {
        const bool big = (M % 256 == 0) || M > 576;
        const int bm = big ? 256 : 192;
        const int tm = (M + bm - 1) / bm;
        const long long tn = (N + 255) / 256;
        const long long nt = (long long)tm * tn * B;
        const unsigned grid = (unsigned)(nt < 256 ? nt : 256);
        if (big) hipLaunchKernelGGL((conv_nn_ring_kernel<4>), dim3(grid), dim3(512), 0, s, p, tm, tn, nt);
        else hipLaunchKernelGGL((conv_nn_ring_kernel<3>), dim3(grid), dim3(512), 0, s, p, tm, tn, nt);
        break;
    }
    case ConvNnKernel::tile: {
        constexpr int BM = 128;
        const int tm = (M + BM - 1) / BM;
        const int BN = N >= (1ll << 19) ? 256 : 128;
        const long long tn = (N + BN - 1) / BN;
        const long long nb = (long long)tm * tn * B;
        MK_REQUIRE(nb < (1ll << 31), "conv1x1_nn: grid too large");
        if (BN == 256) hipLaunchKernelGGL((conv_nn_kernel<BM, 256, 1, 64, 2>), dim3((unsigned)nb), dim3(NT), 0, s, p, tm, tn);
        else hipLaunchKernelGGL((conv_nn_kernel<BM, 128, 1, 64, 3>), dim3((unsigned)nb), dim3(NT), 0, s, p, tm, tn);
        break;
    }
    }
    return mk_check_launch("mk_conv1x1_nn");
}

namespace {
struct WgPlan {
    bool ring;
    bool swap;
    int tp;
    int slabs;
    int qslabs;
    long long S;
    long long chunk;
};

WgPlan wgrad_plan(int M, int K, int B, long long N) {
    WgPlan pl{};
    const int big = M > K ? M : K, small = M > K ? K : M;
    if (big >= 96 && N * 2 * 384 < (1ll << 31) && N >= 2048) {
        pl.ring = true;
        int q, pr;
        if (big <= 384) { q = big; pr = small; }
        else if (small <= 384) { q = small; pr = big; }
        else { q = big; pr = small; }
        const bool q_is_x = (K == q) && !(M == q && M > K);
        pl.swap = !q_is_x;
        pl.tp = (pr > 192 && pr % 256 != 192 && (pr % 192 != 0 || pr % 256 == 0)) ? 256 : 192;
        if (pr <= 192) pl.tp = 192;
        pl.slabs = (pr + pl.tp - 1) / pl.tp;
        pl.qslabs = (q + 383) / 384;
        long long per_b = 256 / ((long long)pl.slabs * pl.qslabs * B);
        if (per_b < 1) per_b = 1;
        const long long maxs = (N + 511) / 512;
        if (per_b > maxs) per_b = maxs;
        long long chunk = ((N + per_b - 1) / per_b + 63) / 64 * 64;
        per_b = (N + chunk - 1) / chunk;
        pl.chunk = chunk;
        pl.S = per_b * B;
        return pl;
    }
    const int tiles = ((M + 127) / 128) * ((K + 127) / 128);
    long long per_b = 1024 / ((long long)tiles * B);
    if (per_b < 1) per_b = 1;
    const long long maxs = (N + 2047) / 2048;
    if (per_b > maxs) per_b = maxs;
    long long chunk = (N + per_b - 1) / per_b;
    chunk = (chunk + 127) / 128 * 128;
    pl.chunk = chunk;
    pl.S = per_b * B;
    return pl;
}
}

extern "C" long long mk_conv1x1_wgrad_workspace(int M, int K, int B, long long N) {
    const WgPlan pl = wgrad_plan(M, K, B, N);
    return pl.S * (long long)M * K + pl.S * (long long)M;
}

extern "C" int mk_conv1x1_wgrad_fuses_bias(int M, int K, int B, long long N) {
    return wgrad_plan(M, K, B, N).ring ? 1 : 0;
}

static int conv1x1_wgrad_impl(const void* G, const void* X, float* dW, float* dbias, float* part, int M, int K, int B, long long N,
                              int accumulate, void* stream);

extern "C" int mk_conv1x1_wgrad(const void* G, const void* X, float* dW, float* part, int M, int K, int B, long long N,
                                int accumulate, void* stream) {
    return conv1x1_wgrad_impl(G, X, dW, nullptr, part, M, K, B, N, accumulate, stream);
}

extern "C" int mk_conv1x1_wgrad_bias(const void* G, const void* X, float* dW, float* dbias, float* part, int M, int K, int B,
                                     long long N, int accumulate, void* stream) {
    MK_REQUIRE(dbias, "conv1x1_wgrad_bias: null pointer");
    MK_REQUIRE(wgrad_plan(M, K, B, N).ring, "conv1x1_wgrad_bias: this shape runs the tile kernel, which does not form the bias gradient");
    return conv1x1_wgrad_impl(G, X, dW, dbias, part, M, K, B, N, accumulate, stream);
}

static int conv1x1_wgrad_impl(const void* G, const void* X, float* dW, float* dbias, float* part, int M, int K, int B, long long N,
                              int accumulate, void* stream) {
    MK_REQUIRE(G && X && dW && part, "conv1x1_wgrad: null pointer");
    MK_REQUIRE(M > 0 && K > 0 && B > 0 && N > 0 && (N % 8) == 0, "conv1x1_wgrad: bad shape");
    const WgPlan pl = wgrad_plan(M, K, B, N);
    hipStream_t s = (hipStream_t)stream;
    if (pl.ring) {
        ConvWgR p{};
        p.P = (const u16*)(pl.swap ? X : G);
        p.Q = (const u16*)(pl.swap ? G : X);
        p.RP = pl.swap ? K : M;
        p.RQ = pl.swap ? M : K;
        p.part = part, p.B = B, p.S = (int)pl.S, p.slabs = pl.slabs, p.qslabs = pl.qslabs, p.ldo = K, p.N = N, p.chunk = pl.chunk;
        p.bias_part = dbias ? part + pl.S * (long long)M * K : nullptr;
        const dim3 grid((unsigned)(pl.slabs * pl.qslabs * pl.S)), blk(512);
        if (pl.tp == 256) {
            if (pl.swap) hipLaunchKernelGGL((conv_wgrad_ring_kernel<2, 4, 4, 3, true>), grid, blk, 0, s, p);
            else hipLaunchKernelGGL((conv_wgrad_ring_kernel<2, 4, 4, 3, false>), grid, blk, 0, s, p);
        } else {
            if (pl.swap) hipLaunchKernelGGL((conv_wgrad_ring_kernel<2, 4, 3, 3, true>), grid, blk, 0, s, p);
            else hipLaunchKernelGGL((conv_wgrad_ring_kernel<2, 4, 3, 3, false>), grid, blk, 0, s, p);
        }
    } else {
        const int tm = (M + 127) / 128, tk = (K + 127) / 128;
        ConvWg p{(const u16*)G, (const u16*)X, part, M, K, B, (int)pl.S, N, pl.chunk};
        hipLaunchKernelGGL(conv_wgrad_kernel<128>, dim3((unsigned)(tm * tk * pl.S)), dim3(NT), 0, s, p, tm, tk);
    }
    const long long n = (long long)M * K;
    if (n % 4 == 0 && (((uintptr_t)part | (uintptr_t)dW) & 15) == 0)
        hipLaunchKernelGGL(reduce_splits4, dim3((unsigned)((n / 4 + 255) / 256)), dim3(256), 0, s, (const float4*)part, (float4*)dW,
                           n / 4, (int)pl.S, accumulate);
    else
        hipLaunchKernelGGL(reduce_splits, dim3((unsigned)((n + 255) / 256)), dim3(256), 0, s, part, dW, n, (int)pl.S, accumulate);
    if (dbias)
        hipLaunchKernelGGL(reduce_splits, dim3((unsigned)((M + 255) / 256)), dim3(256), 0, s, part + pl.S * n, dbias, (long long)M,
                           (int)pl.S, 0);
    return mk_check_launch("mk_conv1x1_wgrad");
}
```

makani_amd/csrc/conv1x1_plan.h:

```cpp
#pragma once

enum class ConvNnKernel {
    astat73,
    astat2,
    astat1,
    ring,
    tile
};

inline ConvNnKernel conv_nn_plan(int M, int K, int lda, int B, long long N, bool pre, bool has_r, bool has_g, int astat2_env) {
    const bool stationary = M >= 256 && (long long)M * N * 2 < (1ll << 31) && N >= 64 && !(has_r && has_g);
    if (stationary && lda == 80 && K > 64 && K <= 80 && (long long)K * N * 2 < (1ll << 32) && !((has_r || has_g) && pre))
        return ConvNnKernel::astat73;
    const bool small_ring = M == 384 && (long long)B * N <= 32768 && !pre && astat2_env != 1;
    if (stationary && K == 384 && !small_ring) return astat2_env == 0 ? ConvNnKernel::astat1 : ConvNnKernel::astat2;
    if (K >= 64 && M >= 192 && N * 2 * 64 < (1ll << 31) && (long long)M * lda * 2 < (1ll << 31) && N >= 256) return ConvNnKernel::ring;
    return ConvNnKernel::tile;
}
```

makani_amd/csrc/pointwise.hip:

```cpp
#include "common.h"
#include <type_traits>


namespace {

constexpr int NT = 256;
constexpr int UNROLL = 4;

template <typename T>
struct VecIO;
typedef unsigned int u32x4 __attribute__((ext_vector_type(4)));
template <>
struct VecIO<float> {
    static constexpr int N = 4;
    typedef f32x4 Raw;
    __device__ static __forceinline__ Raw load_raw(const float* p) { return *reinterpret_cast<const f32x4*>(p); }
    __device__ static __forceinline__ Raw load_raw_nt(const float* p) { return __builtin_nontemporal_load(reinterpret_cast<const f32x4*>(p)); }
    __device__ static __forceinline__ void unpack(const Raw& r, float* v) {
#pragma unroll
        for (int i = 0; i < 4; ++i) v[i] = r[i];
    }
    __device__ static __forceinline__ void load(const float* p, float* v) { unpack(load_raw(p), v); }
    __device__ static __forceinline__ void store(float* p, const float* v) {
        f32x4 r;
// ... 371 lines not shown
        plane_totals(ws, plane, chunks, d1, d2, redd);
        t1 = (float)d1, t2 = (float)d2;
        if (chunk == 0 && threadIdx.x == 0) {
            sums[plane] = t1;
            sums[planes + plane] = t2;
        }
    } else {
        t1 = sums[plane], t2 = sums[planes + plane];
    }
    const float m1 = q ? t1 : t1 * inv_total, m2 = q ? t2 : t2 * inv_total;
    const float cq = q ? mean * rstd * (1.f - qsum) : 0.f;
    const float k = rstd * g;
    const T* xp = x + plane * hw;
    const T* gp = gy + plane * hw;
    T* op = gx + plane * hw;
    for_chunk<T, 2, true>(hw, chunks, chunk, xp, gp, [&](long long e, auto cnt, const float* v, const float* d) {
        float o[cnt()], nn[cnt()], dg[cnt()];
#pragma unroll
        for (int i = 0; i < cnt(); ++i) nn[i] = (pre<T>(v[i], pb, pre_bias != nullptr) - mean) * rstd;
        if (GELU) gelu_grad_affine_n<T, cnt()>(nn, g, b, dg);
#pragma unroll
        for (int i = 0; i < cnt(); ++i) {
            const float n = nn[i];
            float ga = d[i];
            if (GELU) ga *= dg[i];
            const float w = q ? q[e + i] : 1.f;
            o[i] = k * (ga - w * (m1 + (n - cq) * m2));
        }
        store_n(op + e, o, cnt);
    });
}

#define MK_FUSED_SLOTS_FWD 8
#define MK_FUSED_SLOTS_BWD 8
#define MK_FUSED_SLOTS_BWD_GELU 5
__host__ __device__ constexpr int fused_slots(int kind) { return kind == 0 ? MK_FUSED_SLOTS_FWD : (kind == 1 ? MK_FUSED_SLOTS_BWD : MK_FUSED_SLOTS_BWD_GELU); }
constexpr unsigned long long FUSED_SENTINEL = ~0ull;

template <typename T>
__host__ __device__ constexpr long long fused_chunk_cap(int kind) {
    return (long long)NT * VecIO<T>::N * fused_slots(kind);
}

__device__ __forceinline__ void fused_publish(unsigned long long* slot, float s1, float s2) {
    unsigned long long v = ((unsigned long long)__float_as_uint(s2) << 32) | (unsigned long long)__float_as_uint(s1);
    if (v == FUSED_SENTINEL) v ^= 1ull;
    __hip_atomic_store(slot, v, __ATOMIC_RELAXED, __HIP_MEMORY_SCOPE_AGENT);
}

__device__ __forceinline__ void fused_gather(unsigned long long* slots, unsigned* depart, long long plane, int chunks, double& t1,
                                             double& t2, double* redd ) {
    double a = 0.0, b = 0.0;
    if ((int)threadIdx.x < chunks) {
        unsigned long long* sp = slots + plane * chunks + threadIdx.x;
        unsigned long long v;
        while ((v = __hip_atomic_load(sp, __ATOMIC_RELAXED, __HIP_MEMORY_SCOPE_AGENT)) == FUSED_SENTINEL) __builtin_amdgcn_s_sleep(4);
        a = (double)__uint_as_float((unsigned)(v & 0xffffffffull));
        b = (double)__uint_as_float((unsigned)(v >> 32));
    }
#pragma unroll
    for (int o = 32; o > 0; o >>= 1) {
        a += __shfl_down(a, o, 64);
        b += __shfl_down(b, o, 64);
    }
    const int lane = threadIdx.x & 63, w = threadIdx.x >> 6;
    if (lane == 0) {
        redd[2 * w] = a;
        redd[2 * w + 1] = b;
    }
    __syncthreads();
    t1 = 0.0, t2 = 0.0;
    for (int i = 0; i < NT / 64; ++i) {
        t1 += redd[2 * i];
        t2 += redd[2 * i + 1];
    }
    if (threadIdx.x == 0) {
        const unsigned old = __hip_atomic_fetch_add(depart + plane, 1u, __ATOMIC_RELAXED, __HIP_MEMORY_SCOPE_AGENT);
        if (old == (unsigned)chunks - 1u) {
            for (int c = 0; c < chunks; ++c)
                __hip_atomic_store(slots + plane * chunks + c, FUSED_SENTINEL, __ATOMIC_RELAXED, __HIP_MEMORY_SCOPE_AGENT);
            __hip_atomic_store(depart + plane, 0u, __ATOMIC_RELAXED, __HIP_MEMORY_SCOPE_AGENT);
        }
    }
}

template <typename T, bool GELU>
__global__ __launch_bounds__(NT) void in_fwd_fused(const T* __restrict__ x, T* __restrict__ y, float* __restrict__ stats,
                                                   const float* __restrict__ gamma, const float* __restrict__ beta,
                                                   unsigned long long* __restrict__ slots, unsigned* __restrict__ depart, float eps,
                                                   int channels, long long hw, int chunks, const float* __restrict__ pre_bias) {
    constexpr int VEC = VecIO<T>::N;
    constexpr int FUSED_SLOTS = fused_slots(0);
    typedef typename VecIO<T>::Raw Raw;
    __shared__ float red[2 * NT / 64];
    __shared__ double redd[2 * NT / 64];
    const long long plane = blockIdx.x / chunks;
    const int chunk = blockIdx.x % chunks;
    const int c = (int)(plane % channels);
    const bool has_pb = pre_bias != nullptr;
    const float pb = has_pb ? pre_bias[c] : 0.f;
    const T* xp = x + plane * hw;
    T* yp = y + plane * hw;
    const long long len = chunk_len(hw, chunks, VEC);
    const long long c0 = (long long)chunk * len;
    const long long c1 = min(hw, c0 + len);
    Raw raw[FUSED_SLOTS];
#pragma unroll
    for (int s = 0; s < FUSED_SLOTS; ++s) {
        const long long e = c0 + ((long long)s * NT + threadIdx.x) * VEC;
        raw[s] = VecIO<T>::load_raw_nt(xp + (e < c1 ? e : c0));
    }
    const float pivot = pre<T>(VecIO<T>::load1(xp), pb, has_pb);
    float s1 = 0.f, s2 = 0.f;
#pragma unroll
    for (int s = 0; s < FUSED_SLOTS; ++s) {
        const long long e = c0 + ((long long)s * NT + threadIdx.x) * VEC;
        if (e < c1) {
            float v[VEC];
            VecIO<T>::unpack(raw[s], v);
#pragma unroll
            for (int i = 0; i < VEC; ++i) {
                const float d = pre<T>(v[i], pb, has_pb) - pivot;
                s1 += d;
                s2 += d * d;
            }
        }
    }
    block_reduce2(s1, s2, red);
    if (threadIdx.x == 0) fused_publish(slots + plane * chunks + chunk, s1, s2);
    double t1, t2;
    fused_gather(slots, depart, plane, chunks, t1, t2, redd);
    const double m = t1 / (double)hw;
    double var = t2 / (double)hw - m * m;
    if (var < 0.0) var = 0.0;
    const float mean = (float)((double)pivot + m);
    const float rstd = (float)(1.0 / sqrt(var + (double)eps));
    if (chunk == 0 && threadIdx.x == 0) {
        stats[2 * plane] = mean;
        stats[2 * plane + 1] = rstd;
    }
    const float g = gamma ? gamma[c] : 1.f, b = beta ? beta[c] : 0.f;
    const float sc = rstd * g, sh = b - mean * rstd * g;
#pragma unroll
    for (int s = 0; s < FUSED_SLOTS; ++s) {
        const long long e = c0 + ((long long)s * NT + threadIdx.x) * VEC;
        if (e < c1) {
            float v[VEC], o[VEC];
            VecIO<T>::unpack(raw[s], v);
#pragma unroll
            for (int i = 0; i < VEC; ++i) o[i] = pre<T>(v[i], pb, has_pb) * sc + sh;
            if (GELU) gelu_n<T, VEC>(o);
            VecIO<T>::store(yp + e, o);
        }
    }
}

template <typename T, bool GELU>
__global__ __launch_bounds__(NT) void in_bwd_fused(const T* __restrict__ x, const T* __restrict__ gy, T* __restrict__ gx,
                                                   const float* __restrict__ stats, const float* __restrict__ gamma,
                                                   const float* __restrict__ beta, float* __restrict__ sums,
                                                   unsigned long long* __restrict__ slots, unsigned* __restrict__ depart, int channels,
                                                   long long hw, int chunks, float inv_total, const float* __restrict__ pre_bias) {
    constexpr int VEC = VecIO<T>::N;
    constexpr int FUSED_SLOTS = fused_slots(GELU ? 2 : 1);
    typedef typename VecIO<T>::Raw Raw;
    __shared__ float red[2 * NT / 64];
    __shared__ double redd[2 * NT / 64];
    const long long plane = blockIdx.x / chunks;
    const int chunk = blockIdx.x % chunks;
    const long long planes = gridDim.x / chunks;
    const int c = (int)(plane % channels);
    const bool has_pb = pre_bias != nullptr;
    const float pb = has_pb ? pre_bias[c] : 0.f;
    const float mean = stats[2 * plane], rstd = stats[2 * plane + 1];
    const float g = gamma ? gamma[c] : 1.f, b = beta ? beta[c] : 0.f;
    const T* xp = x + plane * hw;
    const T* gp = gy + plane * hw;
    T* op = gx + plane * hw;
    const long long len = chunk_len(hw, chunks, VEC);
    const long long c0 = (long long)chunk * len;
    const long long c1 = min(hw, c0 + len);
    Raw rx[FUSED_SLOTS], rg[FUSED_SLOTS];
#pragma unroll
    for (int s = 0; s < FUSED_SLOTS; ++s) {
        const long long e = c0 + ((long long)s * NT + threadIdx.x) * VEC;
        const long long a = e < c1 ? e : c0;
        rx[s] = VecIO<T>::load_raw_nt(xp + a);
        rg[s] = VecIO<T>::load_raw_nt(gp + a);
    }
    constexpr int NGA = GELU ? FUSED_SLOTS * VEC : 1;
    float gak[NGA];
    float s1 = 0.f, s2 = 0.f;
#pragma unroll
    for (int s = 0; s < FUSED_SLOTS; ++s) {
        const long long e = c0 + ((long long)s * NT + threadIdx.x) * VEC;
        if (e < c1) {
            float v[VEC], d[VEC], nn[VEC], dg[VEC];
            VecIO<T>::unpack(rx[s], v);
            VecIO<T>::unpack(rg[s], d);
#pragma unroll
            for (int i = 0; i < VEC; ++i) nn[i] = (pre<T>(v[i], pb, has_pb) - mean) * rstd;
            if (GELU) gelu_grad_affine_n<T, VEC>(nn, g, b, dg);
#pragma unroll
            for (int i = 0; i < VEC; ++i) {
                const float n = nn[i];
                float ga = d[i];
                if (GELU) {
                    ga *= dg[i];
                    gak[s * VEC + i] = ga;
                }
                s1 += ga;
                s2 += ga * n;
            }
        }
    }
    block_reduce2(s1, s2, red);
    if (threadIdx.x == 0) fused_publish(slots + plane * chunks + chunk, s1, s2);
    double d1, d2;
    fused_gather(slots, depart, plane, chunks, d1, d2, redd);
    const float t1 = (float)d1, t2 = (float)d2;
    if (chunk == 0 && threadIdx.x == 0) {
        sums[plane] = t1;
        sums[planes + plane] = t2;
    }
    const float m1 = t1 * inv_total, m2 = t2 * inv_total;
    const float k = rstd * g;
#pragma unroll
    for (int s = 0; s < FUSED_SLOTS; ++s) {
        const long long e = c0 + ((long long)s * NT + threadIdx.x) * VEC;
        if (e < c1) {
            float v[VEC], d[VEC], o[VEC];
            VecIO<T>::unpack(rx[s], v);
            VecIO<T>::unpack(rg[s], d);
#pragma unroll
            for (int i = 0; i < VEC; ++i) {
                const float n = (pre<T>(v[i], pb, has_pb) - mean) * rstd;
                const float ga = GELU ? gak[s * VEC + i] : d[i];
                o[i] = k * (ga - (m1 + n * m2));
            }
            VecIO<T>::store(op + e, o);
        }
    }
}

template <typename T>
__global__ __launch_bounds__(NT) void bias_gelu_fwd(const T* __restrict__ x, const float* __restrict__ bias,
                                                    T* __restrict__ y, int channels, long long hw, int chunks) {
    const long long plane = blockIdx.x / chunks;
    const int chunk = blockIdx.x % chunks;
    const float b = bias ? bias[plane % channels] : 0.f;
    const T* xp = x + plane * hw;
    T* yp = y + plane * hw;
    for_chunk<T, 1>(hw, chunks, chunk, xp, xp, [&](long long e, auto cnt, const float* v, const float*) {
        float o[cnt()];
#pragma unroll
        for (int i = 0; i < cnt(); ++i) o[i] = gelu_f(v[i] + b);
        store_n(yp + e, o, cnt);
    });
}

template <typename T>
__global__ __launch_bounds__(NT) void bias_gelu_bwd(const T* __restrict__ x, const float* __restrict__ bias,
                                                    const T* __restrict__ gy, T* __restrict__ gx,
                                                    float* __restrict__ ws, int channels, long long hw, int chunks) {
    __shared__ float red[2 * NT / 64];
    const long long plane = blockIdx.x / chunks;
    const int chunk = blockIdx.x % chunks;
    const float b = bias ? bias[plane % channels] : 0.f;
    const T* xp = x + plane * hw;
    const T* gp = gy + plane * hw;
    T* op = gx + plane * hw;
    float s1 = 0.f, s2 = 0.f;
    for_chunk<T, 2>(hw, chunks, chunk, xp, gp, [&](long long e, auto cnt, const float* v, const float* d) {
        float o[cnt()];
#pragma unroll
        for (int i = 0; i < cnt(); ++i) {
            o[i] = d[i] * gelu_grad_f(v[i] + b);
            s1 += o[i];
        }
        store_n(op + e, o, cnt);
    });
    if (ws) {
        block_reduce2(s1, s2, red);
        if (threadIdx.x == 0) {
            ws[2 * (long long)blockIdx.x] = s1;
            ws[2 * (long long)blockIdx.x + 1] = 0.f;
        }
    }
}


constexpr int LP_UNROLL = 8;
constexpr long long LP_CHUNK = (long long)NT * 4 * LP_UNROLL;

__device__ __forceinline__ void load4(const float* p, float* v) {
    const f32x4 r = *reinterpret_cast<const f32x4*>(p);
    v[0] = r[0], v[1] = r[1], v[2] = r[2], v[3] = r[3];
}
__device__ __forceinline__ void load4(const u16* p, float* v) {
    const uint2 r = *reinterpret_cast<const uint2*>(p);
    v[0] = __uint_as_float(r.x << 16), v[1] = __uint_as_float(r.x & 0xffff0000u);
    v[2] = __uint_as_float(r.y << 16), v[3] = __uint_as_float(r.y & 0xffff0000u);
}
__device__ __forceinline__ void store4(float* p, const float* v) {
    f32x4 r = {v[0], v[1], v[2], v[3]};
    *reinterpret_cast<f32x4*>(p) = r;
// ... 160 lines not shown
    } else {
        const int ch = chunks_for<u16>(hw, planes);
        hipLaunchKernelGGL(in_stats_partial<u16>, dim3((unsigned)(planes * ch)), dim3(NT), 0, s, (const u16*)x, ws, hw, ch, nullptr, 1, quad);
        hipLaunchKernelGGL(in_stats_final<u16>, dim3(fb), dim3(256), 0, s, (const u16*)x, ws, stats, planes, hw, ch, eps, qs);
    }
    return mk_check_launch("mk_instnorm_stats");
}

static int instnorm_apply_impl(const void* x, void* y, int dtype, float* stats, const float* gamma, const float* beta,
                               const float* ws, float eps, long long planes, int channels, long long hw, int fuse_gelu,
                               const float* pre_bias, float qsum, hipStream_t s);

__global__ void in_merge_stats(const float* __restrict__ all, const float* __restrict__ counts, float* __restrict__ out,
                               long long planes, int P, float eps) {
    const long long p = (long long)blockIdx.x * blockDim.x + threadIdx.x;
    if (p >= planes) return;
    double n = 0.0, mean = 0.0, m2 = 0.0;
    for (int r = 0; r < P; ++r) {
        const double c = (double)counts[r];
        if (!(c > 0.0)) continue;
        const double mu = (double)all[((long long)r * planes + p) * 2];
        const double rs = (double)all[((long long)r * planes + p) * 2 + 1];
        double var = 1.0 / (rs * rs) - (double)eps;
        if (var < 0.0) var = 0.0;
        const double nn = n + c, delta = mu - mean;
        mean += delta * (c / nn);
        m2 += var * c + delta * delta * (n * c / nn);
        n = nn;
    }
    out[2 * p] = (float)mean;
    out[2 * p + 1] = (float)(1.0 / sqrt((n > 0.0 ? m2 / n : 0.0) + (double)eps));
}

extern "C" int mk_instnorm_merge(const float* all_stats, const float* counts, float* stats, long long planes, int nranks,
                                 float eps, void* stream) {
    MK_REQUIRE(all_stats && counts && stats && planes > 0 && nranks > 0, "instnorm_merge: bad args");
    hipLaunchKernelGGL(in_merge_stats, dim3((unsigned)((planes + 255) / 256)), dim3(256), 0, (hipStream_t)stream, all_stats, counts,
                       stats, planes, nranks, eps);
    return mk_check_launch("mk_instnorm_merge");
}

extern "C" int mk_instnorm_apply(const void* x, void* y, int dtype, const float* stats, const float* gamma,
                                 const float* beta, long long planes, int channels, long long hw, int fuse_gelu,
                                 void* stream) {
    int rc = check_common(x, planes, hw, dtype, "instnorm_apply");
    if (rc) return rc;
    MK_REQUIRE(y && stats && channels > 0, "instnorm_apply: bad args");
    return instnorm_apply_impl(x, y, dtype, const_cast<float*>(stats), gamma, beta, nullptr, 0.f, planes, channels, hw,
                               fuse_gelu, nullptr, 0.f, (hipStream_t)stream);
}

extern "C" int mk_instnorm_fwd(const void* x, void* y, int dtype, float* stats, float* ws, const float* gamma,
                               const float* beta, const float* pre_bias, const float* quad, float quad_sum,
                               long long planes, int channels, long long hw, float eps, int fuse_gelu, void* stream) {
    int rc = check_common(x, planes, hw, dtype, "instnorm_fwd");
    if (rc) return rc;
    MK_REQUIRE(y && stats && ws && channels > 0, "instnorm_fwd: bad args");
    hipStream_t s = (hipStream_t)stream;
    if (dtype == MK_F32)
        hipLaunchKernelGGL(in_stats_partial<float>, dim3((unsigned)(planes * chunks_for<float>(hw, planes))), dim3(NT), 0, s, (const float*)x, ws, hw, chunks_for<float>(hw, planes), pre_bias, channels, quad);
    else
        hipLaunchKernelGGL(in_stats_partial<u16>, dim3((unsigned)(planes * chunks_for<u16>(hw, planes))), dim3(NT), 0, s, (const u16*)x, ws, hw, chunks_for<u16>(hw, planes), pre_bias, channels, quad);
    MK_REQUIRE(quad == nullptr || quad_sum > 0.f, "instnorm_fwd: quadrature weights need their (positive) sum");
    return instnorm_apply_impl(x, y, dtype, stats, gamma, beta, ws, eps, planes, channels, hw, fuse_gelu, pre_bias,
                               quad ? quad_sum : 0.f, s);
}

static int instnorm_apply_impl(const void* x, void* y, int dtype, float* stats, const float* gamma, const float* beta,
                               const float* ws, float eps, long long planes, int channels, long long hw, int fuse_gelu,
                               const float* pre_bias, float qsum, hipStream_t s) {
    if (dtype == MK_F32) {
        const int ch = chunks_for<float>(hw, planes);
        dim3 g((unsigned)(planes * ch));
        if (fuse_gelu)
            hipLaunchKernelGGL((in_apply<float, true>), g, dim3(NT), 0, s, (const float*)x, (float*)y, stats, gamma, beta, ws, eps, channels, hw, ch, pre_bias, qsum);
        else
            hipLaunchKernelGGL((in_apply<float, false>), g, dim3(NT), 0, s, (const float*)x, (float*)y, stats, gamma, beta, ws, eps, channels, hw, ch, pre_bias, qsum);
    } else {
        const int ch = chunks_for<u16>(hw, planes);
        dim3 g((unsigned)(planes * ch));
        if (fuse_gelu)
            hipLaunchKernelGGL((in_apply<u16, true>), g, dim3(NT), 0, s, (const u16*)x, (u16*)y, stats, gamma, beta, ws, eps, channels, hw, ch, pre_bias, qsum);
        else
            hipLaunchKernelGGL((in_apply<u16, false>), g, dim3(NT), 0, s, (const u16*)x, (u16*)y, stats, gamma, beta, ws, eps, channels, hw, ch, pre_bias, qsum);
    }
    return mk_check_launch("mk_instnorm_apply");
}

extern "C" int mk_instnorm_bwd(const void* x, const void* gy, void* gx, int dtype, const float* stats,
                               const float* gamma, const float* beta, const float* pre_bias, const float* quad,
                               float quad_sum, float* sums, float* ws, long long planes, int channels, long long hw,
                               long long hw_total, int phase, int fuse_gelu, void* stream) {
    int rc = check_common(x, planes, hw, dtype, "instnorm_bwd");
    if (rc) return rc;
    MK_REQUIRE(gy && gx && stats && sums && ws && channels > 0, "instnorm_bwd: bad args");
    MK_REQUIRE(phase >= 0 && phase <= 2 && hw_total >= hw, "instnorm_bwd: bad phase / hw_total");
    hipStream_t s = (hipStream_t)stream;
    const int fb = (int)((planes + 255) / 256);
    const float inv_total = 1.0f / (float)hw_total;
#define IN_BWD(T, G)                                                                                                   \
    do {                                                                                                               \
        const int ch = chunks_for<T>(hw, planes);                                                                              \
        dim3 g((unsigned)(planes * ch));                                                                               \
        if (phase != 2)                                                                                                \
            hipLaunchKernelGGL((in_bwd_partial<T, G>), g, dim3(NT), 0, s, (const T*)x, (const T*)gy, stats, gamma,    \
                               beta, ws, channels, hw, ch, pre_bias);                                                  \
        if (phase == 1)                                                                                                \
            hipLaunchKernelGGL(sum_chunks_final, dim3(fb), dim3(256), 0, s, ws, sums, planes, ch);                     \
        if (phase != 1)              \
            hipLaunchKernelGGL((in_bwd_apply<T, G>), g, dim3(NT), 0, s, (const T*)x, (const T*)gy, (T*)gx, stats,     \
                               gamma, beta, sums, phase == 0 ? ws : nullptr, channels, hw, ch, inv_total, pre_bias,    \
                               quad, quad_sum);                                                                        \
    } while (0)
    if (dtype == MK_F32) {
        if (fuse_gelu) IN_BWD(float, true); else IN_BWD(float, false);
    } else {
        if (fuse_gelu) IN_BWD(u16, true); else IN_BWD(u16, false);
    }
#undef IN_BWD
    return mk_check_launch("mk_instnorm_bwd");
}

extern "C" int mk_instnorm_fused_chunks(long long hw, int dtype, long long planes, int kind) {
    if (hw <= 0 || planes <= 0 || kind < 0 || kind > 2) return 0;
    const int vec = dtype == MK_BF16 ? VecIO<u16>::N : VecIO<float>::N;
    if (hw % vec) return 0;
    const int c = dtype == MK_BF16 ? fused_chunks_for<u16>(hw, planes, kind) : fused_chunks_for<float>(hw, planes, kind);
    if (c > NT || planes * (long long)c >= (1ll << 31)) return 0;
    return c;
}

extern "C" int mk_instnorm_fwd_fused(const void* x, void* y, int dtype, float* stats, const float* gamma, const float* beta,
                                     const float* pre_bias, void* slots, void* depart, long long planes, int channels, long long hw,
                                     float eps, int fuse_gelu, void* stream) {
    int rc = check_common(x, planes, hw, dtype, "instnorm_fwd_fused");
    if (rc) return rc;
    const int ch = mk_instnorm_fused_chunks(hw, dtype, planes, 0);
    MK_REQUIRE(ch > 0, "instnorm_fwd_fused: plane shape not served (hw = %lld)", hw);
    MK_REQUIRE(y && stats && slots && depart && channels > 0, "instnorm_fwd_fused: bad args");
    hipStream_t s = (hipStream_t)stream;
    const dim3 g((unsigned)(planes * ch));
    unsigned long long* sl = (unsigned long long*)slots;
    unsigned* dp = (unsigned*)depart;
#define IN_FF(T, G) hipLaunchKernelGGL((in_fwd_fused<T, G>), g, dim3(NT), 0, s, (const T*)x, (T*)y, stats, gamma, beta, sl, dp, eps, channels, hw, ch, pre_bias)
    if (dtype == MK_F32) {
        if (fuse_gelu) IN_FF(float, true); else IN_FF(float, false);
    } else {
        if (fuse_gelu) IN_FF(u16, true); else IN_FF(u16, false);
    }
#undef IN_FF
    return mk_check_launch("mk_instnorm_fwd_fused");
}

extern "C" int mk_instnorm_bwd_fused(const void* x, const void* gy, void* gx, int dtype, const float* stats, const float* gamma,
                                     const float* beta, const float* pre_bias, float* sums, void* slots, void* depart, long long planes,
                                     int channels, long long hw, int fuse_gelu, void* stream) {
    int rc = check_common(x, planes, hw, dtype, "instnorm_bwd_fused");
    if (rc) return rc;
    const int ch = mk_instnorm_fused_chunks(hw, dtype, planes, fuse_gelu ? 2 : 1);
    MK_REQUIRE(ch > 0, "instnorm_bwd_fused: plane shape not served (hw = %lld)", hw);
    MK_REQUIRE(gy && gx && stats && sums && slots && depart && channels > 0, "instnorm_bwd_fused: bad args");
    hipStream_t s = (hipStream_t)stream;
    const dim3 g((unsigned)(planes * ch));
    const float inv_total = 1.0f / (float)hw;
    unsigned long long* sl = (unsigned long long*)slots;
    unsigned* dp = (unsigned*)depart;
#define IN_BF(T, G) hipLaunchKernelGGL((in_bwd_fused<T, G>), g, dim3(NT), 0, s, (const T*)x, (const T*)gy, (T*)gx, stats, gamma, beta, sums, sl, dp, channels, hw, ch, inv_total, pre_bias)
    if (dtype == MK_F32) {
        if (fuse_gelu) IN_BF(float, true); else IN_BF(float, false);
    } else {
        if (fuse_gelu) IN_BF(u16, true); else IN_BF(u16, false);
    }
#undef IN_BF
    return mk_check_launch("mk_instnorm_bwd_fused");
}

extern "C" int mk_plane_sums(const void* x, int dtype, float* sums, float* ws, long long planes, long long hw, void* stream) {
    int rc = check_common(x, planes, hw, dtype, "plane_sums");
    if (rc) return rc;
    MK_REQUIRE(sums && ws, "plane_sums: null sums/ws");
    hipStream_t s = (hipStream_t)stream;
    const int fb = (int)((planes + 255) / 256);
    if (dtype == MK_F32) {
        const int ch = chunks_for<float>(hw, planes);
        hipLaunchKernelGGL(plane_sum_partial<float>, dim3((unsigned)(planes * ch)), dim3(NT), 0, s, (const float*)x, ws, hw, ch);
        hipLaunchKernelGGL(sum_chunks_final, dim3(fb), dim3(256), 0, s, ws, sums, planes, ch);
    } else {
        const int ch = chunks_for<u16>(hw, planes);
        hipLaunchKernelGGL(plane_sum_partial<u16>, dim3((unsigned)(planes * ch)), dim3(NT), 0, s, (const u16*)x, ws, hw, ch);
        hipLaunchKernelGGL(sum_chunks_final, dim3(fb), dim3(256), 0, s, ws, sums, planes, ch);
    }
    return mk_check_launch("mk_plane_sums");
}

extern "C" int mk_bias_gelu_fwd(const void* x, const float* bias, void* y, int dtype, long long planes, int channels,
                                long long hw, void* stream) {
    int rc = check_common(x, planes, hw, dtype, "bias_gelu_fwd");
    if (rc) return rc;
    MK_REQUIRE(y && channels > 0, "bias_gelu_fwd: bad args");
    hipStream_t s = (hipStream_t)stream;
    if (dtype == MK_F32) {
        const int ch = chunks_for<float>(hw, planes);
        hipLaunchKernelGGL(bias_gelu_fwd<float>, dim3((unsigned)(planes * ch)), dim3(NT), 0, s, (const float*)x, bias, (float*)y, channels, hw, ch);
    } else {
        const int ch = chunks_for<u16>(hw, planes);
        hipLaunchKernelGGL(bias_gelu_fwd<u16>, dim3((unsigned)(planes * ch)), dim3(NT), 0, s, (const u16*)x, bias, (u16*)y, channels, hw, ch);
    }
    return mk_check_launch("mk_bias_gelu_fwd");
}

extern "C" int mk_bias_gelu_bwd(const void* x, const float* bias, const void* gy, void* gx, float* sums, float* ws,
                                int dtype, long long planes, int channels, long long hw, void* stream) {
    int rc = check_common(x, planes, hw, dtype, "bias_gelu_bwd");
    if (rc) return rc;
    MK_REQUIRE(gy && gx && channels > 0, "bias_gelu_bwd: bad args");
    MK_REQUIRE((sums == nullptr) == (ws == nullptr), "bias_gelu_bwd: sums and ws go together");
    hipStream_t s = (hipStream_t)stream;
    const int fb = (int)((planes + 255) / 256);
    if (dtype == MK_F32) {
        const int ch = chunks_for<float>(hw, planes);
        hipLaunchKernelGGL(bias_gelu_bwd<float>, dim3((unsigned)(planes * ch)), dim3(NT), 0, s, (const float*)x, bias, (const float*)gy, (float*)gx, ws, channels, hw, ch);
        if (sums) hipLaunchKernelGGL(sum_chunks_final, dim3(fb), dim3(256), 0, s, ws, sums, planes, ch);
    } else {
        const int ch = chunks_for<u16>(hw, planes);
        hipLaunchKernelGGL(bias_gelu_bwd<u16>, dim3((unsigned)(planes * ch)), dim3(NT), 0, s, (const u16*)x, bias, (const u16*)gy, (u16*)gx, ws, channels, hw, ch);
        if (sums) hipLaunchKernelGGL(sum_chunks_final, dim3(fb), dim3(256), 0, s, ws, sums, planes, ch);
    }
    return mk_check_launch("mk_bias_gelu_bwd");
}

extern "C" int mk_quad_lp_chunks(long long hw) { return (int)((hw + LP_CHUNK - 1) / LP_CHUNK); }

#define MK_LP_DISPATCH(KERN, ...)                                                                         \
    do {                                                                                                  \
        if (a_dtype == MK_F32 && b_dtype == MK_F32)                                                       \
            hipLaunchKernelGGL((KERN<float, float>), grid, dim3(NT), 0, s, (const float*)a, (const float*)b, __VA_ARGS__); \
        else if (a_dtype == MK_F32)                                                                       \
            hipLaunchKernelGGL((KERN<float, u16>), grid, dim3(NT), 0, s, (const float*)a, (const u16*)b, __VA_ARGS__);     \
        else if (b_dtype == MK_F32)                                                                       \
            hipLaunchKernelGGL((KERN<u16, float>), grid, dim3(NT), 0, s, (const u16*)a, (const float*)b, __VA_ARGS__);     \
        else                                                                                              \
            hipLaunchKernelGGL((KERN<u16, u16>), grid, dim3(NT), 0, s, (const u16*)a, (const u16*)b, __VA_ARGS__);         \
    } while (0)

extern "C" int mk_quad_lp_fwd(const void* a, int a_dtype, const void* b, int b_dtype, const float* wgt, const float* q,
                              float* sums, float* ws, long long planes, long long hw, int mode, float p, void* stream) {
    int rc = check_common(a, planes, hw, a_dtype, "quad_lp_fwd");
    if (rc) return rc;
    MK_REQUIRE(q && sums && ws, "quad_lp_fwd: null pointer");
    MK_REQUIRE(b_dtype == MK_F32 || b_dtype == MK_BF16, "quad_lp_fwd: bad dtype %d", b_dtype);
    MK_REQUIRE(mode == 0 || mode == 1, "quad_lp_fwd: mode %d", mode);
    MK_REQUIRE(mode == 0 || p > 0.f, "quad_lp_fwd: p = %f must be positive", p);
    if (mode == 0) b = nullptr;
    hipStream_t s = (hipStream_t)stream;
    const int ch = mk_quad_lp_chunks(hw);
    const dim3 grid((unsigned)(planes * ch));
    MK_LP_DISPATCH(quad_lp_fwd, wgt, q, ws, hw, ch, mode, p);
    hipLaunchKernelGGL(sum_chunks_final, dim3((unsigned)((planes + 255) / 256)), dim3(256), 0, s, ws, sums, planes, ch);
    return mk_check_launch("mk_quad_lp_fwd");
}

extern "C" int mk_quad_lp_bwd(const void* a, int a_dtype, const void* b, int b_dtype, const float* wgt, const float* q,
                              const float* g, void* da, void* db, long long planes, long long hw, int mode, float p,
                              void* stream) {
    int rc = check_common(a, planes, hw, a_dtype, "quad_lp_bwd");
    if (rc) return rc;
    MK_REQUIRE(q && g && (da || db), "quad_lp_bwd: null pointer");
    MK_REQUIRE(b_dtype == MK_F32 || b_dtype == MK_BF16, "quad_lp_bwd: bad dtype %d", b_dtype);
    MK_REQUIRE(mode == 0 || mode == 1, "quad_lp_bwd: mode %d", mode);
    MK_REQUIRE(db == nullptr || b != nullptr, "quad_lp_bwd: db without b");
    hipStream_t s = (hipStream_t)stream;
    const int ch = mk_quad_lp_chunks(hw);
    const dim3 grid((unsigned)(planes * ch));
    if (a_dtype == MK_F32 && b_dtype == MK_F32)
        hipLaunchKernelGGL((quad_lp_bwd<float, float>), grid, dim3(NT), 0, s, (const float*)a, (const float*)b, wgt, q, g, (float*)da, (float*)db, hw, ch, mode, p);
    else if (a_dtype == MK_F32)
        hipLaunchKernelGGL((quad_lp_bwd<float, u16>), grid, dim3(NT), 0, s, (const float*)a, (const u16*)b, wgt, q, g, (float*)da, (u16*)db, hw, ch, mode, p);
    else if (b_dtype == MK_F32)
        hipLaunchKernelGGL((quad_lp_bwd<u16, float>), grid, dim3(NT), 0, s, (const u16*)a, (const float*)b, wgt, q, g, (u16*)da, (float*)db, hw, ch, mode, p);
    else
        hipLaunchKernelGGL((quad_lp_bwd<u16, u16>), grid, dim3(NT), 0, s, (const u16*)a, (const u16*)b, wgt, q, g, (u16*)da, (u16*)db, hw, ch, mode, p);
    return mk_check_launch("mk_quad_lp_bwd");
}
```

makani_amd/ops.py:

```python
import ctypes as C
import os
import weakref
from dataclasses import dataclass

import numpy as np
import torch

from . import _lib
from ._lib import MkGemm, check, dtype_code, lib, ptr, stream
from . import legendre as _leg


def round4(n: int) -> int:
    return (n + 3) // 4 * 4


GEMM_MODE = os.environ.get("MAKANI_AMD_GEMM", "auto")
if GEMM_MODE not in ("auto", "x6", "x3", "fp32"):
    raise ValueError(f"MAKANI_AMD_GEMM={GEMM_MODE!r}: expected auto, x6, x3 or fp32")


def gemm_mode() -> str:
    if GEMM_MODE != "auto":
        return GEMM_MODE
# ... 687 lines not shown


def round32(n: int) -> int:
    return (n + 31) // 32 * 32


class VectorMats:

    def __init__(self, nat, tr, band, L, nlat):
        self.nat, self.tr, self.band, self.L, self.nlat = nat, tr, band, L, nlat


def vector_legendre(X: torch.Tensor, vm: VectorMats, mode: int) -> torch.Tensor:
    gm = gemm_mode()
    if gm == "fp32":
        raise NotImplementedError("the vector Legendre kernels run on the split-bf16 engine (MAKANI_AMD_GEMM=auto, x6 or x3)")
    limbs = 3 if gm == "x6" else 2
    assert X.is_contiguous() and X.dtype == torch.float32
    ana = mode in (0, 2)
    if ana:
        M, nlat, _, R = X.shape
        Rp = R // 2
        assert nlat == vm.nlat
        out = torch.empty((vm.L, M, 2, Rp if mode == 2 else 2 * Rp), dtype=torch.float32, device=X.device)
        m0, m1, rows, K = vm.tr[0], vm.tr[1], vm.L, nlat
    else:
        L, M, _, R = X.shape
        Rp = R if mode == 3 else R // 2
        assert L == vm.L
        out = torch.empty((M, vm.nlat, 2, 2 * Rp), dtype=torch.float32, device=X.device)
        m0, m1, rows, K = vm.nat[0], vm.nat[1], vm.nlat, L
    assert m0.shape[0] == M and Rp % 32 == 0
    p0, p1 = limb_planes(m0), limb_planes(m1)
    lo, hi = vm.band if vm.band is not None else (None, None)
    prods = 1 if mode == 3 else 2
    with _timed(f"vlegendre_{'analysis' if ana else 'synthesis'}_k{vm.nlat}", flops=2.0 * prods * out.shape[-1] * 2 * vm.nlat * vm.L * M,
                nbytes=4.0 * (X.numel() + out.numel() + 2 * M * vm.L * vm.nlat)):
        check(lib().mk_vlegendre(ptr(p0), ptr(p1), p0.stride(0), p0.stride(1), p0.stride(2), limbs, ptr(X), ptr(out), mode,
                                 rows, K, M, Rp, 0, ptr(lo), ptr(hi), stream()), "mk_vlegendre")
    return out


class VAnalysisFn(torch.autograd.Function):

    @staticmethod
    def forward(ctx, F, vm, s_only=False):
        ctx.vm, ctx.s_only = vm, s_only
        return vector_legendre(F, vm, 2 if s_only else 0)

    @staticmethod
    def backward(ctx, gS):
        return vector_legendre(gS.contiguous(), ctx.vm, 3 if ctx.s_only else 1), None, None


class VSynthesisFn(torch.autograd.Function):

    @staticmethod
    def forward(ctx, S, vm, t_zero=False):
        ctx.vm, ctx.t_zero = vm, t_zero
        return vector_legendre(S, vm, 3 if t_zero else 1)

    @staticmethod
    def backward(ctx, gF):
        return vector_legendre(gF.contiguous(), ctx.vm, 2 if ctx.t_zero else 0), None, None


class VSToComplexFn(torch.autograd.Function):

    @staticmethod
    def forward(ctx, S, B, Cc):
        ctx.Cp = S.shape[3] // B
        return s_to_complex(S, B, Cc)

    @staticmethod
    def backward(ctx, gc):
        return complex_to_s(gc, ctx.Cp), None, None


class VComplexToSFn(torch.autograd.Function):
    @staticmethod
    def forward(ctx, c, Cp):
        ctx.meta = c.shape[:2]
        return complex_to_s(c, Cp)

    @staticmethod
    def backward(ctx, gS):
        B, Cc = ctx.meta
        return s_to_complex(gS.contiguous(), B, Cc), None


def _ws(planes, hw, dtype, device):
    ch = lib().mk_pointwise_chunks(hw, _lib.MK_BF16 if dtype == torch.bfloat16 else _lib.MK_F32, planes)
    return torch.empty((planes * ch * 2,), dtype=torch.float32, device=device)


def _batch_sum(sums, B, Cc):
    return sums if B == 1 else sums.view(2, B, Cc).sum(1)


_FUSED_SYNC = {}


def _fused_sync(nslots: int, planes: int, device):
    key = str(device)
    hit = _FUSED_SYNC.get(key)
    if hit is None or hit[0].numel() < nslots or hit[1].numel() < planes:
        if torch.cuda.is_current_stream_capturing():
            raise RuntimeError("one-pass instance norm: its hand-over buffers must exist before the step is captured (run a warm-up step)")
        torch.cuda.synchronize(device)
        slots = torch.full((max(nslots, 1 << 20),), -1, dtype=torch.int64, device=device)
        depart = torch.zeros((max(planes, 1 << 16),), dtype=torch.int32, device=device)
        hit = _FUSED_SYNC[key] = (slots, depart)
    return hit


def _fused_norm_chunks(x, planes, hw, quad, kind):
    if quad is not None or os.environ.get("MAKANI_AMD_NORM_FUSED", "1") != "1":
        return 0
    return int(lib().mk_instnorm_fused_chunks(hw, dtype_code(x), planes, kind))


class InstanceNormFn(torch.autograd.Function):

    @staticmethod
    def forward(ctx, x, gamma, beta, eps, fuse_gelu, pre_bias=None, quad=None, quad_sum=0.0):
        x = x.contiguous()
        B, Cc, H, W = x.shape
        planes, hw = B * Cc, H * W
        dt = dtype_code(x)
        stats = torch.empty((planes, 2), dtype=torch.float32, device=x.device)
        g = gamma.float().contiguous() if gamma is not None else None
        b = beta.float().contiguous() if beta is not None else None
        pb = pre_bias.float().contiguous() if pre_bias is not None else None
        y = torch.empty_like(x)
        ch = _fused_norm_chunks(x, planes, hw, quad, 0)
        if ch:
            slots, depart = _fused_sync(planes * ch, planes, x.device)
            with _timed(f"instnorm_fwd{'_gelu' if fuse_gelu else ''}_n{hw}", nbytes=2.0 * x.numel() * x.element_size()):
                check(lib().mk_instnorm_fwd_fused(ptr(x), ptr(y), dt, ptr(stats), ptr(g), ptr(b), ptr(pb), ptr(slots), ptr(depart), planes, Cc, hw,
                                                  eps, 1 if fuse_gelu else 0, stream()), "instnorm_fwd_fused")
        else:
            ws = _ws(planes, hw, x.dtype, x.device)
            with _timed(f"instnorm_fwd{'_gelu' if fuse_gelu else ''}_n{hw}", nbytes=3.0 * x.numel() * x.element_size()):
                check(lib().mk_instnorm_fwd(ptr(x), ptr(y), dt, ptr(stats), ptr(ws), ptr(g), ptr(b), ptr(pb), ptr(quad), float(quad_sum),
                                            planes, Cc, hw, eps, 1 if fuse_gelu else 0, stream()), "instnorm_fwd")
        ctx.save_for_backward(x, stats, g, b, pb, quad)
        ctx.quad_sum = float(quad_sum)
        ctx.fuse_gelu = fuse_gelu
        return y

    @staticmethod
    def backward(ctx, gy):
        x, stats, g, b, pb, quad = ctx.saved_tensors
        B, Cc, H, W = x.shape
        planes, hw = B * Cc, H * W
        gy = gy.contiguous()
        if gy.dtype != x.dtype:
            gy = gy.to(x.dtype)
        gx = torch.empty_like(x)
        sums = torch.empty((2, planes), dtype=torch.float32, device=x.device)
        ch = _fused_norm_chunks(x, planes, hw, quad, 2 if ctx.fuse_gelu else 1)
        if ch:
            slots, depart = _fused_sync(planes * ch, planes, x.device)
            with _timed(f"instnorm_bwd{'_gelu' if ctx.fuse_gelu else ''}_n{hw}", nbytes=3.0 * x.numel() * x.element_size()):
                check(lib().mk_instnorm_bwd_fused(ptr(x), ptr(gy), ptr(gx), dtype_code(x), ptr(stats), ptr(g), ptr(b), ptr(pb), ptr(sums),
                                                  ptr(slots), ptr(depart), planes, Cc, hw, 1 if ctx.fuse_gelu else 0, stream()), "instnorm_bwd_fused")
        else:
            ws = _ws(planes, hw, x.dtype, x.device)
            with _timed(f"instnorm_bwd{'_gelu' if ctx.fuse_gelu else ''}_n{hw}", nbytes=5.0 * x.numel() * x.element_size()):
                check(lib().mk_instnorm_bwd(ptr(x), ptr(gy), ptr(gx), dtype_code(x), ptr(stats), ptr(g), ptr(b), ptr(pb), ptr(quad),
                                            ctx.quad_sum, ptr(sums), ptr(ws), planes, Cc, hw, hw, 0, 1 if ctx.fuse_gelu else 0,
                                            stream()), "instnorm_bwd")
        s = _batch_sum(sums, B, Cc)
        gpb = torch.zeros_like(pb) if (pb is not None and ctx.needs_input_grad[5]) else None
        return gx, (s[1] if g is not None else None), (s[0] if b is not None else None), None, None, gpb, None, None


class ChannelLayerNormFn(torch.autograd.Function):

    @staticmethod
    def forward(ctx, x, gamma, beta, eps, out_dtype):
        x = x.contiguous()
        B, Cc, H, W = x.shape
        P = H * W
        y = torch.empty((B, Cc, H, W), dtype=out_dtype, device=x.device)
        stats = torch.empty((B, 2, P), dtype=torch.float32, device=x.device)
        g = gamma.float().contiguous() if gamma is not None else None
        b = beta.float().contiguous() if beta is not None else None
        with _timed(f"chan_layernorm_fwd_n{P}", nbytes=float(x.numel()) * (2 * x.element_size() + y.element_size())):
            check(lib().mk_chan_layernorm_fwd(ptr(x), dtype_code(x), ptr(y), dtype_code(y), ptr(stats), ptr(g), ptr(b), B, Cc, P,
                                              float(eps), stream()), "mk_chan_layernorm_fwd")
        ctx.save_for_backward(x, stats, g)
        ctx.has = (gamma is not None, beta is not None)
        return y

    @staticmethod
    def backward(ctx, gy):
        x, stats, g = ctx.saved_tensors
        B, Cc, H, W = x.shape
        P = H * W
        gy = gy.contiguous()
        if gy.dtype not in (torch.float32, x.dtype):
            gy = gy.float()
        gx = dg = db = None
        if ctx.needs_input_grad[0]:
            gx = torch.empty_like(x)
            with _timed(f"chan_layernorm_bwd_n{P}", nbytes=float(x.numel()) * (3 * x.element_size() + 2 * gy.element_size())):
                check(lib().mk_chan_layernorm_bwd(ptr(x), dtype_code(x), ptr(gy), dtype_code(gy), ptr(gx), ptr(stats), ptr(g), B, Cc, P,
                                                  stream()), "mk_chan_layernorm_bwd")
        if (ctx.has[0] and ctx.needs_input_grad[1]) or (ctx.has[1] and ctx.needs_input_grad[2]):
            ch = lib().mk_chan_layernorm_chunks(Cc, P)
            part = torch.empty((2, Cc, ch), dtype=torch.float32, device=x.device)
            check(lib().mk_chan_layernorm_wgrad(ptr(x), dtype_code(x), ptr(gy), dtype_code(gy), ptr(stats), ptr(part), B, Cc, P,
                                                stream()), "mk_chan_layernorm_wgrad")
            sums = part.sum(dim=2)
            dg = sums[0] if ctx.has[0] else None
            db = sums[1] if ctx.has[1] else None
        return gx, dg, db, None, None


class BiasGeluFn(torch.autograd.Function):

    @staticmethod
    def forward(ctx, x, bias):
        x = x.contiguous()
        B, Cc, H, W = x.shape
        bf = bias.float().contiguous() if bias is not None else None
        y = torch.empty_like(x)
        check(lib().mk_bias_gelu_fwd(ptr(x), ptr(bf), ptr(y), dtype_code(x), B * Cc, Cc, H * W, stream()), "bias_gelu_fwd")
        ctx.save_for_backward(x, bf)
        return y

    @staticmethod
    def backward(ctx, gy):
        x, bf = ctx.saved_tensors
        B, Cc, H, W = x.shape
        planes, hw = B * Cc, H * W
        gy = gy.contiguous()
        if gy.dtype != x.dtype:
            gy = gy.to(x.dtype)
        gx = torch.empty_like(x)
        need_b = bf is not None and ctx.needs_input_grad[1]
        sums = torch.empty((2, planes), dtype=torch.float32, device=x.device) if need_b else None
        ws = _ws(planes, hw, x.dtype, x.device) if need_b else None
        check(lib().mk_bias_gelu_bwd(ptr(x), ptr(bf), ptr(gy), ptr(gx), ptr(sums), ptr(ws), dtype_code(x), planes, Cc,
                                     hw, stream()), "bias_gelu_bwd")
        gb = _batch_sum(sums, B, Cc)[0] if need_b else None
        return gx, gb


def round8(n: int) -> int:
    return (n + 7) // 8 * 8


def pad_weight_bf16(w2d: torch.Tensor) -> torch.Tensor:
    M, K = w2d.shape
    lda = round8(K)
    if lda == K:
        return w2d.to(torch.bfloat16).contiguous()
    out = torch.zeros((M, lda), dtype=torch.bfloat16, device=w2d.device)
    out[:, :K] = w2d
    return out


def conv1x1_nn(A: torch.Tensor, K: int, x: torch.Tensor, bias=None, act=False, want_pre=False, residual=None,
               gelu_grad_of=None):
    B, Kx, H, W = x.shape
    assert Kx == K and x.dtype == torch.bfloat16 and A.dtype == torch.bfloat16
    x = x.contiguous()
    M, lda = A.shape
    N = H * W
    y = torch.empty((B, M, H, W), dtype=torch.bfloat16, device=x.device)
    ypre = torch.empty_like(y) if (act and want_pre) else None
    bf = bias.float().contiguous() if bias is not None else None
    r = residual.contiguous() if residual is not None else None
    g = gelu_grad_of.contiguous() if gelu_grad_of is not None else None
    extra = (ypre is not None) + (r is not None) + (g is not None)
    with _timed(f"conv1x1_nn_m{M}_k{K}_n{N}", flops=2.0 * B * M * K * N, nbytes=2.0 * B * N * (M * (1 + extra) + K)):
        check(lib().mk_conv1x1_nn(ptr(A), ptr(x), ptr(y), ptr(ypre), ptr(bf), ptr(r), ptr(g), M, K, lda, B, N,
                                  1 if act else 0, stream()), "mk_conv1x1_nn")
    return y, ypre


def conv1x1_wgrad(g: torch.Tensor, x: torch.Tensor, want_bias: bool = False):
    B, M, H, W = g.shape
    K = x.shape[1]
    N = H * W
    g, x = g.contiguous(), x.contiguous()
    nws = lib().mk_conv1x1_wgrad_workspace(M, K, B, N)
    part = torch.empty((nws,), dtype=torch.float32, device=g.device)
    dW = torch.empty((M, K), dtype=torch.float32, device=g.device)
    fused = want_bias and bool(lib().mk_conv1x1_wgrad_fuses_bias(M, K, B, N))
    with _timed(f"conv1x1_wgrad_m{M}_k{K}_n{N}", flops=2.0 * B * M * K * N, nbytes=2.0 * B * N * (M + K)):
        if fused:
            db = torch.empty((M,), dtype=torch.float32, device=g.device)
            check(lib().mk_conv1x1_wgrad_bias(ptr(g), ptr(x), ptr(dW), ptr(db), ptr(part), M, K, B, N, 0, stream()), "mk_conv1x1_wgrad_bias")
        else:
            check(lib().mk_conv1x1_wgrad(ptr(g), ptr(x), ptr(dW), ptr(part), M, K, B, N, 0, stream()), "mk_conv1x1_wgrad")
    if not want_bias:
        return dW
    return dW, (db if fused else _sum_planes(g))


def _sum_planes(t: torch.Tensor) -> torch.Tensor:
    if not (t.is_cuda and t.dim() == 4 and t.dtype in (torch.bfloat16, torch.float32)):
        raise RuntimeError("makani_amd ops need 4-d bf16 / fp32 GPU tensors (the HIP path has no CPU fallback)")
    t = t.contiguous()
    B, Cc, H, W = t.shape
    sums = torch.empty((2, B * Cc), dtype=torch.float32, device=t.device)
    check(lib().mk_plane_sums(ptr(t), dtype_code(t), ptr(sums), ptr(_ws(B * Cc, H * W, t.dtype, t.device)), B * Cc, H * W,
                              stream()), "mk_plane_sums")
    return _batch_sum(sums, B, Cc)[0]


class Conv1x1Fn(torch.autograd.Function):

    @staticmethod
    def forward(ctx, x, weight, bias, residual):
        M, K = weight.shape[0], weight.shape[1]
        A, At = weight_operands(weight, need_t=ctx.needs_input_grad[0])
        y, _ = conv1x1_nn(A, K, x, bias=bias, residual=residual)
        ctx.save_for_backward(x, weight, At)
        ctx.has_bias = bias is not None
        ctx.has_res = residual is not None
        return y

    @staticmethod
    def backward(ctx, gy):
        x, weight, At = ctx.saved_tensors
        M, K = weight.shape[0], weight.shape[1]
        gy = gy.contiguous()
        gx = gw = gb = gr = None
        if ctx.needs_input_grad[0]:
            gx, _ = conv1x1_nn(At, M, gy)
        want_b = ctx.has_bias and ctx.needs_input_grad[2]
        if ctx.needs_input_grad[1]:
            if want_b:
                gw, gb = conv1x1_wgrad(gy, x, want_bias=True)
                gw = gw.view_as(weight)
            else:
                gw = conv1x1_wgrad(gy, x).view_as(weight)
        elif want_b:
            gb = _sum_planes(gy)
        if ctx.has_res and ctx.needs_input_grad[3]:
            gr = gy
        return gx, gw, gb, gr


class ConvGeluConvFn(torch.autograd.Function):

    @staticmethod
    def forward(ctx, x, w1, b1, w2, b2):
        H1, K = w1.shape[0], w1.shape[1]
        M = w2.shape[0]
        A1, A1t = weight_operands(w1, need_t=ctx.needs_input_grad[0])
        A2, A2t = weight_operands(w2, need_t=True)
        h, a1 = conv1x1_nn(A1, K, x, bias=b1, act=True, want_pre=True)
        y, _ = conv1x1_nn(A2, H1, h, bias=b2)
        ctx.save_for_backward(x, w1, w2, a1, h, A1t, A2t)
        ctx.has_b = (b1 is not None, b2 is not None)
        return y

    @staticmethod
    def backward(ctx, gy):
        x, w1, w2, a1, h, A1t, A2t = ctx.saved_tensors
        H1, K = w1.shape[0], w1.shape[1]
        M = w2.shape[0]
        gy = gy.contiguous()
        ga1, _ = conv1x1_nn(A2t, M, gy, gelu_grad_of=a1)
        gw2 = gb2 = gw1 = gb1 = None
        want_b2, want_b1 = ctx.has_b[1] and ctx.needs_input_grad[4], ctx.has_b[0] and ctx.needs_input_grad[2]
        if ctx.needs_input_grad[3] and want_b2:
            gw2, gb2 = conv1x1_wgrad(gy, h, want_bias=True)
            gw2 = gw2.view_as(w2)
        else:
            gw2 = conv1x1_wgrad(gy, h).view_as(w2) if ctx.needs_input_grad[3] else None
            gb2 = _sum_planes(gy) if want_b2 else None
        if ctx.needs_input_grad[1] and want_b1:
            gw1, gb1 = conv1x1_wgrad(ga1, x, want_bias=True)
            gw1 = gw1.view_as(w1)
        else:
            gw1 = conv1x1_wgrad(ga1, x).view_as(w1) if ctx.needs_input_grad[1] else None
            gb1 = _sum_planes(ga1) if want_b1 else None
        gx = None
        if ctx.needs_input_grad[0]:
            gx, _ = conv1x1_nn(A1t, H1, ga1)
        return gx, gw1, gb1, gw2, gb2


def want_bf16_shadow(param):
    param._mk_want_bf16 = True


def _shadow_valid(weight):
    return (getattr(weight, "_mk_shadow", None) is not None and getattr(weight, "_mk_shadow_version", -1) == weight._version
            and getattr(weight, "_mk_shadow_ptr", 0) == weight.data_ptr() and weight._mk_shadow.device == weight.device)


def cast_weight(weight, dtype):
    if dtype == weight.dtype:
        return weight
    if dtype == torch.bfloat16 and _shadow_valid(weight):
        K = weight.numel() // weight.shape[0]
        sh = weight._mk_shadow
        return sh.view(weight.shape) if sh.shape[1] == K else sh[:, :K]
    return weight.to(dtype)


def weight_operands(weight, need_t=False):
    M = weight.shape[0]
    K = weight.numel() // M
    if _shadow_valid(weight):
        return weight._mk_shadow, (weight._mk_shadow_t if need_t else None)
    w2 = weight.detach().view(M, K)
    return pad_weight_bf16(w2), (pad_weight_bf16(w2.t()) if need_t else None)


def _pad_last(t, mult):
    r = (-t.shape[-1]) % mult
    return t if r == 0 else torch.nn.functional.pad(t, (0, r))


def chan_gemm_f32(w: torch.Tensor, x: torch.Tensor, out: torch.Tensor = None, accumulate: bool = False, transposed: bool = False):
    grouped = w.dim() == 3
    w3 = w if grouped else w.unsqueeze(0)
    x4 = x if grouped else x.unsqueeze(1)
    o4 = None if out is None else (out if grouped else out.unsqueeze(1))
    B, G, Kx, N = x4.shape
    Gw, M, K = w3.shape
    rows, kdim = (K, M) if transposed else (M, K)
    assert Gw == G and Kx == kdim and x4.dtype == torch.float32 and w3.dtype == torch.float32
    if N % 4:
        r = chan_gemm_f32(w3, _pad_last(x4, 4), None if o4 is None else _pad_last(o4, 4), accumulate, transposed)[..., :N]
        if o4 is None:
            r = r.contiguous()
            return r if grouped else r[:, 0]
        o4.copy_(r)
        return out
    wp = _pad_last(w3.contiguous(), 4)
    K4 = wp.shape[2]
    x4 = x4.contiguous()
    if o4 is None:
        o4 = torch.empty((B, G, rows, N), dtype=torch.float32, device=x4.device)
        accumulate = False
    assert o4.is_contiguous()
    a = dict(a_row=1, a_k=K4) if transposed else dict(a_row=K4, a_k=1)
    g = _gemm(A=wp.data_ptr(), B=x4.data_ptr(), C=o4.data_ptr(), a_batch=0, a_inner=M * K4, **a,
              b_batch=G * kdim * N, b_inner=kdim * N, b_col=1, b_k=N, c_batch=G * rows * N, c_inner=rows * N, c_row=N,
              M=rows, N=N, K=kdim, batch=B * G, inner=G, beta=1 if accumulate else 0)
    with _timed(f"conv1x1_f32_m{rows}_k{kdim}_n{N}", flops=2.0 * B * G * M * K * N,
                nbytes=4.0 * B * G * N * (M + K) * (1 + int(accumulate))):
        _run_gemm(g, False, "chan_gemm_f32")
    if out is not None:
        return out
    return o4 if grouped else o4[:, 0]


def chan_wgrad_f32(gy: torch.Tensor, x: torch.Tensor) -> torch.Tensor:
    grouped = gy.dim() == 4
    gy4 = gy if grouped else gy.unsqueeze(1)
    x4 = x if grouped else x.unsqueeze(1)
    B, G, M, N = gy4.shape
    K = x4.shape[2]
    if N % 4:
        gy4, x4 = _pad_last(gy4, 4), _pad_last(x4, 4)
        N = gy4.shape[-1]
    gy4, x4 = gy4.contiguous(), x4.contiguous()
    ns = 1
    for cand in range(min(256, max(1, N // 2048)), 0, -1):
        if N % (4 * cand) == 0:
            ns = cand
            break
    chunk = N // ns
    Kp = round4(K)
    part = torch.empty((B, G, ns, M, Kp), dtype=torch.float32, device=gy4.device)
    for b in range(B):
        g = _gemm(A=gy4[b].data_ptr(), B=x4[b].data_ptr(), C=part[b].data_ptr(), a_batch=M * N, a_inner=chunk, a_row=N, a_k=1,
                  b_batch=K * N, b_inner=chunk, b_col=N, b_k=1, c_batch=ns * M * Kp, c_inner=M * Kp, c_row=Kp,
                  M=M, N=K, K=chunk, batch=G * ns, inner=ns)
        with _timed(f"conv1x1_f32_wgrad_m{M}_k{K}_n{N}", flops=2.0 * G * M * K * N, nbytes=4.0 * G * N * (M + K)):
            _run_gemm(g, False, "chan_wgrad_f32")
    dW = part.sum(dim=(0, 2))[..., :K]
    return dW if grouped else dW[0]


class GroupMmFn(torch.autograd.Function):

    @staticmethod
    def forward(ctx, x, W):
        ctx.save_for_backward(x, W)
        return chan_gemm_f32(W.detach().float(), x.float()).to(x.dtype)

    @staticmethod
    def backward(ctx, gz):
        x, W = ctx.saved_tensors
        gz = gz.contiguous().float()
        gx = chan_gemm_f32(W.detach().float(), gz, transposed=True).to(x.dtype) if ctx.needs_input_grad[0] else None
        gW = chan_wgrad_f32(gz, x.float()).to(W.dtype) if ctx.needs_input_grad[1] else None
        return gx, gW
# ... 152 lines not shown
```

makani_amd/sfno.py:

```python
import math
from functools import partial

import torch
import torch.nn as nn

from ._lib import device_guard
from torch.utils.checkpoint import checkpoint

from . import distributed as thd
from .layers import MLP, ChannelLayerNorm, DropPath, EncoderDecoder, GeometricInstanceNormS2, InstanceNorm2d, PointwiseConv
from .sht import InverseRealSHT, RealSHT
from .spectral_conv import SpectralConv


class SpectralFilterLayer(nn.Module):

    def __init__(self, forward_transform, inverse_transform, embed_dim, filter_type="linear", operator_type="diagonal",
                 hidden_size_factor=1, rank=1.0, separable=False, complex_activation="real", spectral_layers=1,
                 bias=False, drop_rate=0.0, gain=1.0):
        super().__init__()
        if filter_type != "linear":
            raise NotImplementedError("only filter_type='linear' (SpectralConv) is implemented")
        self.filter = SpectralConv(forward_transform, inverse_transform, embed_dim, embed_dim,
                                   operator_type=operator_type, separable=separable, bias=bias, gain=gain)

    @torch.compiler.disable(recursive=True)
    def forward(self, x):
        return self.filter(x)


class NeuralOperatorBlock(nn.Module):

    def __init__(self, forward_transform, inverse_transform, embed_dim, filter_type="linear", operator_type="diagonal",
                 mlp_ratio=2.0, mlp_drop_rate=0.0, path_drop_rate=0.0, act_layer=nn.GELU,
                 norm_layer=(nn.Identity, nn.Identity), rank=1.0, separable=False, inner_skip="linear",
                 outer_skip=None, use_mlp=False, comm_feature_name="matmul", complex_activation="real",
                 spectral_layers=1, bias=False, final_activation=False, checkpointing_level=0):
        super().__init__()
        if hasattr(forward_transform, "lat_shapes"):
            self.input_shape_loc = (forward_transform.lat_shapes[forward_transform.comm_rank_polar],
                                    forward_transform.lon_shapes[forward_transform.comm_rank_azimuth])
            self.output_shape_loc = (inverse_transform.lat_shapes[inverse_transform.comm_rank_polar],
                                     inverse_transform.lon_shapes[inverse_transform.comm_rank_azimuth])
        else:
            self.input_shape_loc = (forward_transform.nlat, forward_transform.nlon)
            self.output_shape_loc = (inverse_transform.nlat, inverse_transform.nlon)

        if inner_skip not in ("none", None):
            raise NotImplementedError(f"inner_skip={inner_skip!r}: the SFNO path uses inner_skip='none'")
        if outer_skip not in ("linear", "none", None):
            raise NotImplementedError(f"outer_skip={outer_skip!r}: the SFNO path uses outer_skip='linear' (or none)")
        has_act = act_layer is not nn.Identity
        self.norm0 = norm_layer[0]()
        self.filter = SpectralFilterLayer(forward_transform, inverse_transform, embed_dim, filter_type, operator_type,
                                          hidden_size_factor=mlp_ratio, rank=rank, separable=separable,
                                          complex_activation=complex_activation, spectral_layers=spectral_layers,
                                          bias=bias, drop_rate=path_drop_rate, gain=2.0 if has_act else 1.0)
        self.act_is_gelu = act_layer is nn.GELU
        self.act_layer0 = act_layer()
        self.norm1 = norm_layer[1]()
        gain = 2.0 if (final_activation and has_act) else 1.0
        if outer_skip == "linear":
            gain /= 2.0
            self.outer_skip = PointwiseConv(embed_dim, embed_dim, bias=False)
            nn.init.normal_(self.outer_skip.weight, std=math.sqrt(gain / embed_dim))
        if use_mlp:
            self.mlp = MLP(in_features=embed_dim, hidden_features=int(embed_dim * mlp_ratio), act_layer=act_layer,
                           drop_rate=mlp_drop_rate, drop_type="features", checkpointing=(checkpointing_level >= 2), gain=gain)
        self.drop_path = DropPath(path_drop_rate) if path_drop_rate > 0.0 else nn.Identity()
        if final_activation:
            self.act_layer1 = act_layer()

    @torch.compiler.disable(recursive=True)
    def forward(self, x):
        x, residual = self.filter(x)
        norms = (InstanceNorm2d, GeometricInstanceNormS2, thd.DistributedInstanceNorm2d)
        if self.act_is_gelu and isinstance(self.norm0, norms):
            x = self.norm0(x, fuse_gelu=True)
        else:
            x = self.act_layer0(self.norm0(x))

        if hasattr(self, "mlp") and type(self.norm1) is InstanceNorm2d and self.mlp.can_defer_output_bias(x):
            x, pb = self.mlp.forward_deferred_bias(x)
            x = self.norm1(x, pre_bias=pb)
        else:
            if hasattr(self, "mlp"):
                x = self.mlp(x)
            x = self.norm1(x)
        x = self.drop_path(x)

        if hasattr(self, "outer_skip"):
            fresh = (hasattr(self, "mlp") or isinstance(self.norm1, norms)) and isinstance(self.drop_path, nn.Identity)
            x = self.outer_skip(residual, add_to=x, add_to_is_fresh=fresh)
        if hasattr(self, "act_layer1"):
            x = self.act_layer1(x)
        return x


class SphericalFourierNeuralOperatorNet(nn.Module):

    def __init__(self, spectral_transform="sht", model_grid_type="equiangular", sht_grid_type="legendre-gauss",
                 filter_type="linear", operator_type="dhconv", inp_shape=(721, 1440), out_shape=(721, 1440),
                 scale_factor=8, inp_chans=2, out_chans=2, embed_dim=32, num_layers=4, use_mlp=True, mlp_ratio=2.0,
                 encoder_ratio=1, decoder_ratio=1, activation_function="gelu", encoder_layers=1, pos_embed="none",
                 pos_drop_rate=0.0, path_drop_rate=0.0, mlp_drop_rate=0.0, normalization_layer="instance_norm",
                 max_modes=None, hard_thresholding_fraction=1.0, big_skip=True, rank=1.0, separable=False,
                 complex_activation="real", spectral_layers=3, bias=False, checkpointing_level=0, **kwargs):
        super().__init__()
        if spectral_transform != "sht":
            raise NotImplementedError("only spectral_transform='sht' is implemented")
        if pos_embed not in ("none", "None", None, "direct", "frequency"):
            raise ValueError("Unknown position embedding type")

        self.inp_shape, self.out_shape = tuple(inp_shape), tuple(out_shape)
        self.inp_chans, self.out_chans, self.embed_dim = inp_chans, out_chans, embed_dim
        self.big_skip = big_skip
        self.checkpointing_level = checkpointing_level
        self.h = int(self.inp_shape[0] // scale_factor)
        self.w = int(self.inp_shape[1] // scale_factor)
        self._init_spectral_transforms(model_grid_type, sht_grid_type, hard_thresholding_fraction, max_modes)

        try:
            act = {"relu": nn.ReLU, "gelu": nn.GELU, "silu": nn.SiLU}[activation_function]
        except KeyError:
            raise ValueError(f"Unknown activation function {activation_function}")

        self.encoder = EncoderDecoder(num_layers=encoder_layers, input_dim=inp_chans, output_dim=embed_dim,
                                      hidden_dim=int(encoder_ratio * embed_dim), act_layer=act, input_format="nchw")
        self.pos_drop = nn.Dropout(p=pos_drop_rate) if pos_drop_rate > 0.0 else nn.Identity()
        dpr = [v.item() for v in torch.linspace(0, path_drop_rate, num_layers)]

        if normalization_layer == "layer_norm":
            norm = partial(ChannelLayerNorm, normalized_shape=embed_dim, elementwise_affine=True, eps=1e-6)
        elif normalization_layer == "instance_norm":
            if self.spatial_parallel:
                norm = partial(thd.DistributedInstanceNorm2d, num_features=embed_dim, eps=1e-6, affine=True)
            else:
                norm = partial(InstanceNorm2d, num_features=embed_dim, eps=1e-6, affine=True, track_running_stats=False)
        elif normalization_layer == "instance_norm_s2":
            handle = thd.DistributedGeometricInstanceNormS2 if self.spatial_parallel else GeometricInstanceNormS2
            norm = partial(handle, img_shape=(self.h, self.w), crop_shape=(self.h, self.w), crop_offset=(0, 0),
                           grid_type=model_grid_type, num_features=embed_dim, eps=1e-6, affine=True)
            norm_out = partial(handle, img_shape=self.out_shape, crop_shape=self.out_shape, crop_offset=(0, 0),
                               grid_type=model_grid_type, num_features=embed_dim, eps=1e-6, affine=True)
        elif normalization_layer == "none":
            norm = nn.Identity
        else:
            raise NotImplementedError(f"Error, normalization {normalization_layer} not implemented.")
        if normalization_layer != "instance_norm_s2":
            norm_out = norm

        self.blocks = nn.ModuleList([])
        for i in range(num_layers):
            first, last = i == 0, i == num_layers - 1
            self.blocks.append(NeuralOperatorBlock(
                self.trans_down if first else self.trans,
                self.itrans_up if last else self.itrans,
                embed_dim, filter_type=filter_type, operator_type=operator_type, mlp_ratio=mlp_ratio,
                mlp_drop_rate=mlp_drop_rate, path_drop_rate=dpr[i], act_layer=act,
                norm_layer=(norm, norm) if (first or not last) else (norm_out, norm_out),
                inner_skip="none", outer_skip="linear", use_mlp=use_mlp, rank=rank, separable=separable,
                complex_activation=complex_activation, spectral_layers=spectral_layers, bias=bias,
                checkpointing_level=checkpointing_level))

        self.decoder = EncoderDecoder(num_layers=encoder_layers, input_dim=embed_dim, output_dim=out_chans,
                                      hidden_dim=int(decoder_ratio * embed_dim), act_layer=act,
                                      gain=0.5 if big_skip else 1.0, input_format="nchw")
        if big_skip:
            self.residual_transform = PointwiseConv(inp_chans, out_chans, bias=False)
            self.residual_transform.weight.is_shared_mp = ["spatial"]
            self.residual_transform.weight.sharded_dims_mp = [None, None, None, None]
            nn.init.normal_(self.residual_transform.weight, mean=0.0, std=math.sqrt(0.5 / inp_chans))

        if pos_embed == "direct":
            self.pos_embed = nn.Parameter(torch.zeros(1, embed_dim, self.inp_shape_loc[0], self.inp_shape_loc[1]))
            self.pos_embed.is_shared_mp = []
            self.pos_embed.sharded_dims_mp = [None, None, "h", "w"]
            self.pos_embed.type = "direct"
            with torch.no_grad():
                nn.init.trunc_normal_(self.pos_embed, std=0.02)
        elif pos_embed == "frequency":
            if self.spatial_parallel:
                lmax_loc = self.itrans_up.l_shapes[self.itrans_up.comm_rank_polar]
                mmax_loc = self.itrans_up.m_shapes[self.itrans_up.comm_rank_azimuth]
            else:
                lmax_loc, mmax_loc = self.itrans_up.lmax, self.itrans_up.mmax
            rcoeffs = nn.Parameter(torch.tril(torch.randn(1, embed_dim, lmax_loc, mmax_loc), diagonal=0))
            ccoeffs = nn.Parameter(torch.tril(torch.randn(1, embed_dim, lmax_loc, mmax_loc - 1), diagonal=-1))
            with torch.no_grad():
                nn.init.trunc_normal_(rcoeffs, std=0.02)
                nn.init.trunc_normal_(ccoeffs, std=0.02)
            self.pos_embed = nn.ParameterList([rcoeffs, ccoeffs])
            self.pos_embed.type = "frequency"
            self.pos_embed.is_shared_mp = []
            self.pos_embed.sharded_dims_mp = [None, None, "h", "w"]

    def _add_pos_embed(self, x):
        if self.pos_embed.type == "frequency":
            pe = torch.stack([self.pos_embed[0], nn.functional.pad(self.pos_embed[1], (1, 0), "constant", 0)], dim=-1)
            pe = self.itrans_up(torch.view_as_complex(pe))
        else:
            pe = self.pos_embed
        return x + pe.to(dtype=x.dtype)

    def _init_spectral_transforms(self, model_grid_type, sht_grid_type, hard_thresholding_fraction, max_modes):
        if max_modes is not None:
            modes_lat, modes_lon = max_modes
        else:
            modes_lat = int(self.h * hard_thresholding_fraction)
            modes_lon = int((self.w // 2 + 1) * hard_thresholding_fraction)
        self.spatial_parallel = thd.ensure_initialized()
        sht, isht = (thd.DistributedRealSHT, thd.DistributedInverseRealSHT) if self.spatial_parallel else (RealSHT, InverseRealSHT)
        self.trans_down = sht(*self.inp_shape, lmax=modes_lat, mmax=modes_lon, grid=model_grid_type).float()
        self.itrans_up = isht(*self.out_shape, lmax=modes_lat, mmax=modes_lon, grid=model_grid_type).float()
        self.trans = sht(self.h, self.w, lmax=modes_lat, mmax=modes_lon, grid=sht_grid_type).float()
        self.itrans = isht(self.h, self.w, lmax=modes_lat, mmax=modes_lon, grid=sht_grid_type).float()
        if self.spatial_parallel:
            ih, iw = self.trans_down.comm_rank_polar, self.trans_down.comm_rank_azimuth
            self.inp_shape_loc = (self.trans_down.lat_shapes[ih], self.trans_down.lon_shapes[iw])
            self.out_shape_loc = (self.itrans_up.lat_shapes[ih], self.itrans_up.lon_shapes[iw])
            self.h_loc, self.w_loc = self.itrans.lat_shapes[ih], self.itrans.lon_shapes[iw]
        else:
            self.inp_shape_loc = (self.trans_down.nlat, self.trans_down.nlon)
            self.out_shape_loc = (self.itrans_up.nlat, self.itrans_up.nlon)
            self.h_loc, self.w_loc = self.itrans.nlat, self.itrans.nlon

    def no_weight_decay(self):
        return {"pos_embed", "cls_token"}

    def _forward_features(self, x):
        for blk in self.blocks:
            if self.checkpointing_level >= 3 and torch.is_grad_enabled():
                x = checkpoint(blk, x, use_reentrant=False)
            else:
                x = blk(x)
        return x

    @torch.compiler.disable(recursive=True)
    @device_guard
    def forward(self, x):
        if (x.is_cuda and x.dtype == torch.float32 and torch.is_autocast_enabled("cuda") and not x.requires_grad
# ... 24 lines not shown
```

Before: 28.01 samples/s.

## Fuse norm1 apply into outer-skip conv1x1 epilogue via per-plane affine residual

Norm1 is split into a stats-only pass that emits per-plane (scale, shift) pairs, and the normalization is then applied inside the epilogue of the outer-skip 1x1 conv as an affine transform of the residual load. This removes a full write and re-read of the normalized activation tensor at each block. The catch is a new kernel variant with extra register and shuffle pressure, plus a separate autograd path that recomputes the instance-norm backward. It only applies when the plan picks the two-group weight-stationary kernel.

```diff
diff --git a/include/makani_amd.h b/include/makani_amd.h
--- a/include/makani_amd.h
+++ b/include/makani_amd.h
@@ -99,6 +99,8 @@
 int mk_instnorm_fwd_fused(const void* x, void* y, int dtype, float* stats, const float* gamma, const float* beta,
                           const float* pre_bias, void* slots, void* depart, long long planes, int channels, long long hw,
                           float eps, int fuse_gelu, void* stream);
+int mk_instnorm_stats_fused(const void* x, int dtype, float* stats, float* affine, float* ws, const float* gamma, const float* beta,
+                            const float* pre_bias, long long planes, int channels, long long hw, float eps, void* stream);
 int mk_instnorm_bwd_fused(const void* x, const void* gy, void* gx, int dtype, const float* stats, const float* gamma,
                           const float* beta, const float* pre_bias, float* sums, void* slots, void* depart, long long planes,
                           int channels, long long hw, int fuse_gelu, void* stream);
@@ -129,6 +131,9 @@
 
 int mk_conv1x1_nn(const void* A, const void* X, void* Y, void* Ypre, const float* bias, const void* R, const void* G,
                   int M, int K, int lda, int B, long long N, int act, void* stream);
+int mk_conv1x1_nn_affine(const void* A, const void* X, void* Y, const void* R, const float* r_affine, const float* r_pre_bias,
+                         int M, int K, int lda, int B, long long N, void* stream);
+int mk_conv1x1_nn_affine_ok(int M, int K, int lda, int B, long long N);
 long long mk_conv1x1_wgrad_workspace(int M, int K, int B, long long N);
 int mk_conv1x1_wgrad(const void* G, const void* X, float* dW, float* part, int M, int K, int B, long long N,
                      int accumulate, void* stream);
diff --git a/makani_amd/_lib.py b/makani_amd/_lib.py
--- a/makani_amd/_lib.py
+++ b/makani_amd/_lib.py
@@ -72,6 +72,7 @@
     "mk_instnorm_apply": ([c_vp, c_vp, c_int, c_vp, c_vp, c_vp, c_ll, c_int, c_ll, c_int, c_vp], c_int),
     "mk_instnorm_fused_chunks": ([c_ll, c_int, c_ll, c_int], c_int),
     "mk_instnorm_fwd_fused": ([c_vp, c_vp, c_int, c_vp, c_vp, c_vp, c_vp, c_vp, c_vp, c_ll, c_int, c_ll, c_f, c_int, c_vp], c_int),
+    "mk_instnorm_stats_fused": ([c_vp, c_int, c_vp, c_vp, c_vp, c_vp, c_vp, c_vp, c_ll, c_int, c_ll, c_f, c_vp], c_int),
     "mk_instnorm_bwd_fused": ([c_vp, c_vp, c_vp, c_int, c_vp, c_vp, c_vp, c_vp, c_vp, c_vp, c_vp, c_ll, c_int, c_ll, c_int, c_vp], c_int),
     "mk_instnorm_bwd": ([c_vp, c_vp, c_vp, c_int, c_vp, c_vp, c_vp, c_vp, c_vp, c_f, c_vp, c_vp, c_ll, c_int, c_ll, c_ll, c_int, c_int, c_vp], c_int),
     "mk_chan_layernorm_chunks": ([c_int, c_ll], c_int),
@@ -80,6 +81,8 @@
     "mk_chan_layernorm_wgrad": ([c_vp, c_int, c_vp, c_int, c_vp, c_vp, c_int, c_int, c_ll, c_vp], c_int),
     "mk_bias_gelu_fwd": ([c_vp, c_vp, c_vp, c_int, c_ll, c_int, c_ll, c_vp], c_int),
     "mk_conv1x1_nn": ([c_vp, c_vp, c_vp, c_vp, c_vp, c_vp, c_vp, c_int, c_int, c_int, c_int, c_ll, c_int, c_vp], c_int),
+    "mk_conv1x1_nn_affine": ([c_vp, c_vp, c_vp, c_vp, c_vp, c_vp, c_int, c_int, c_int, c_int, c_ll, c_vp], c_int),
+    "mk_conv1x1_nn_affine_ok": ([c_int, c_int, c_int, c_int, c_ll], c_int),
     "mk_conv1x1_wgrad_workspace": ([c_int, c_int, c_int, c_ll], c_ll),
     "mk_conv1x1_wgrad": ([c_vp, c_vp, c_vp, c_vp, c_int, c_int, c_int, c_ll, c_int, c_vp], c_int),
     "mk_conv1x1_wgrad_fuses_bias": ([c_int, c_int, c_int, c_ll], c_int),
diff --git a/makani_amd/csrc/conv1x1.hip b/makani_amd/csrc/conv1x1.hip
--- a/makani_amd/csrc/conv1x1.hip
+++ b/makani_amd/csrc/conv1x1.hip
@@ -38,6 +38,8 @@
     long long N;
     int act;
     int nt;
+    const float* Raff;
+    const float* Rpb;
 };
 
 __device__ __forceinline__ uint4 ld16(const u16* p) { return *reinterpret_cast<const uint4*>(p); }
@@ -884,9 +886,10 @@
 #endif
 }
 
-template <bool PRE, bool EPI_LOADS>
-__global__ __launch_bounds__(512) void conv_nn_astat2_kernel(const ConvNN p, int slabs, long long tilesN) {
+template <bool PRE, bool EPI_LOADS, bool AFF>
+__device__ __forceinline__ void conv_nn_astat2_body(const ConvNN& p, int slabs, long long tilesN) {
 #if defined(__HIP_DEVICE_COMPILE__)
+    static_assert(!AFF || (EPI_LOADS && !PRE), "the affine mode is a form of the residual epilogue");
     typedef float f32x4_t __attribute__((ext_vector_type(4)));
     constexpr int KS = 12;
     constexpr int KCH = 128, NCH = 3, K4 = 4;
@@ -945,14 +948,25 @@
 #pragma unroll
     for (int ct = 0; ct < CT; ++ct) {
         const int mrow = m_base + ct * 16 + c16;
-        bvr[ct] = (p.bias && mrow < p.M) ? p.bias[mrow] : 0.f;
+        bvr[ct] = (!AFF && p.bias && mrow < p.M) ? p.bias[mrow] : 0.f;
+    }
+    float asc = 0.f, ash = 0.f, apb = 0.f;
+    if constexpr (AFF) {
+        const int j = min(lane, 47);
+        const int u2 = j / 24, ct = (j % 24) >> 3, r8 = j & 7;
+        const int m = min(slab * 384 + 192 * (wave >> 2) + 48 * (((wave & 3) >> 1) + 2 * u2) + 16 * ct + 8 * (wave & 1) + r8, p.M - 1);
+        const float2 a = reinterpret_cast<const float2*>(p.Raff)[(long long)blockIdx.y * p.M + m];
+        asc = a.x;
+        ash = a.y;
+        if (p.Rpb) apb = p.Rpb[m];
     }
 #pragma unroll
     for (int ct = 0; ct < CT; ++ct) {
 #pragma unroll
         for (int ks = 0; ks < KS; ++ks) asm volatile("" : "+v"(wf[ct][ks]));
-        asm volatile("" : "+v"(bvr[ct]));
-    }
+        if constexpr (!AFF) asm volatile("" : "+v"(bvr[ct]));
+    }
+    if constexpr (AFF) asm volatile("" : "+v"(asc), "+v"(ash), "+v"(apb));
 
     const unsigned lds0 = lds_addr(smem) + (unsigned)wave * (NP * 1024);
     const v4i_t rsX = make_rsrc(p.X + (long long)cb * p.K * p.N);
@@ -1047,7 +1061,7 @@
         const int c16 = ln & 15, q4 = ln >> 4;
 #pragma unroll
         for (int ct = 0; ct < CT; ++ct) {
-            const float bv = bvr[ct];
+            const float bv = AFF ? 0.f : bvr[ct];
             const int lrow = ct * 64 + wg * 16 + c16;
 #pragma unroll
             for (int pt = 0; pt < PT; ++pt) {
@@ -1062,9 +1076,17 @@
     auto readback_store = [&](int ts, int ct) __attribute__((always_inline)) {
         const unsigned cn0b = (unsigned)(pfirst + ts * pstride) * 128u;
         typedef unsigned int u32x4_t __attribute__((ext_vector_type(4)));
-        const int tg = (wg << 6) | lane_here();
+        const int lnr = lane_here();
+        const int tg = (wg << 6) | lnr;
 #pragma unroll
         for (int u2 = 0; u2 < 2; ++u2) {
+            float rsc = 0.f, rsh = 0.f, rpb = 0.f;
+            if constexpr (AFF) {
+                const int src = 24 * u2 + 8 * ct + (lnr >> 3);
+                rsc = __shfl(asc, src, 64);
+                rsh = __shfl(ash, src, 64);
+                if (p.Rpb) rpb = __shfl(apb, src, 64);
+            }
             const int idx = tg + 256 * u2;
             const int row = idx >> 3, ch = idx & 7;
             const int srow = ct * 64 + row;
@@ -1101,7 +1123,15 @@
                     }
                 }
                 if (EPI_LOADS && !p.G) {
-                    const uint32_t rw[4] = {ev.x, ev.y, ev.z, ev.w};
+                    uint32_t rw[4] = {ev.x, ev.y, ev.z, ev.w};
+                    if constexpr (AFF) {
+#pragma unroll
+                        for (int e = 0; e < 4; ++e) {
+                            if (p.Rpb) rw[e] = pack_bf16x2(__uint_as_float(rw[e] << 16) + rpb, __uint_as_float(rw[e] & 0xffff0000u) + rpb);
+                            rw[e] = pack_bf16x2(__builtin_fmaf(__uint_as_float(rw[e] << 16), rsc, rsh),
+                                                __builtin_fmaf(__uint_as_float(rw[e] & 0xffff0000u), rsc, rsh));
+                        }
+                    }
 #pragma unroll
                     for (int e = 0; e < 4; ++e) {
                         v[2 * e] += __uint_as_float(rw[e] << 16);
@@ -1216,6 +1246,14 @@
 #endif
 }
 
+template <bool PRE, bool EPI_LOADS>
+__global__ __launch_bounds__(512) void conv_nn_astat2_kernel(const ConvNN p, int slabs, long long tilesN) {
+    conv_nn_astat2_body<PRE, EPI_LOADS, false>(p, slabs, tilesN);
+}
+__global__ __launch_bounds__(512) void conv_nn_astat2_affine_kernel(const ConvNN p, int slabs, long long tilesN) {
+    conv_nn_astat2_body<false, true, true>(p, slabs, tilesN);
+}
+
 struct ConvWg {
     const u16* G;
     const u16* X;
@@ -1579,8 +1617,8 @@
     return e ? atoi(e) : -1;
 }
 
-extern "C" int mk_conv1x1_nn(const void* A, const void* X, void* Y, void* Ypre, const float* bias, const void* R,
-                             const void* G, int M, int K, int lda, int B, long long N, int act, void* stream) {
+static int conv1x1_nn_impl(const void* A, const void* X, void* Y, void* Ypre, const float* bias, const void* R, const void* G,
+                           const float* r_affine, const float* r_pre_bias, int M, int K, int lda, int B, long long N, int act, void* stream) {
     MK_REQUIRE(A && X && Y, "conv1x1_nn: null pointer");
     MK_REQUIRE(M > 0 && K > 0 && B > 0 && N > 0, "conv1x1_nn: bad shape M=%d K=%d B=%d N=%lld", M, K, B, N);
     MK_REQUIRE((lda % 8) == 0 && lda >= K, "conv1x1_nn: lda=%d must be a multiple of 8 and >= K=%d", lda, K);
@@ -1589,16 +1627,23 @@
     static const int nt_env = env_int("MAKANI_AMD_CONV_NT"), astat2_env = env_int("MAKANI_AMD_ASTAT2");
     const long long out_bytes = (long long)B * M * N * 2;
     const int nt = nt_env == 0 ? 0 : (nt_env == 1 ? 1 : out_bytes <= (256ll << 20));
-    ConvNN p{(const u16*)A, (const u16*)X, (u16*)Y, (u16*)Ypre, bias, (const u16*)R, (const u16*)G, M, K, lda, B, N, act, nt};
+    ConvNN p{(const u16*)A, (const u16*)X, (u16*)Y, (u16*)Ypre, bias, (const u16*)R, (const u16*)G, M, K, lda, B, N, act, nt, r_affine, r_pre_bias};
     hipStream_t s = (hipStream_t)stream;
     const bool pre = act && Ypre, epi_loads = R || G;
+    const ConvNnKernel kernel = conv_nn_plan(M, K, lda, B, N, pre, R != nullptr, G != nullptr, astat2_env, r_affine != nullptr);
+    if (r_affine || r_pre_bias) {
+        MK_REQUIRE(r_affine && R && !G && !bias && !act && !Ypre, "conv1x1_nn_affine: the affine residual takes R and no other epilogue");
+        MK_REQUIRE((((uintptr_t)r_affine) & 7) == 0, "conv1x1_nn_affine: the (scale, shift) pairs must be 8-byte aligned");
+        MK_REQUIRE(kernel == ConvNnKernel::astat2, "conv1x1_nn_affine: M=%d K=%d N=%lld does not run the two-group weight-stationary kernel "
+                   "(the only one with the affine residual epilogue)", M, K, N);
+    }
     const int slabs = (M + 383) / 384;
     const long long tn64 = (N + 63) / 64;
     auto stationary_grid = [&](int wgs) {
         const long long streams = tn64 < wgs / slabs ? tn64 : wgs / slabs;
         return dim3((unsigned)(streams * slabs), (unsigned)B);
     };
-    switch (conv_nn_plan(M, K, lda, B, N, pre, R != nullptr, G != nullptr, astat2_env)) {
+    switch (kernel) {
     case ConvNnKernel::astat73: {
         const dim3 grid = stationary_grid(epi_loads ? 256 : 512), blk(256);
         if (epi_loads) hipLaunchKernelGGL((conv_nn_astat_kernel<3, 96, false, true, 5>), grid, blk, 0, s, p, slabs, tn64);
@@ -1608,7 +1653,8 @@
     }
     case ConvNnKernel::astat2: {
         const dim3 grid = stationary_grid(256), blk(512);
-        if (epi_loads && pre) hipLaunchKernelGGL((conv_nn_astat2_kernel<true, true>), grid, blk, 0, s, p, slabs, tn64);
+        if (r_affine) hipLaunchKernelGGL(conv_nn_astat2_affine_kernel, grid, blk, 0, s, p, slabs, tn64);
+        else if (epi_loads && pre) hipLaunchKernelGGL((conv_nn_astat2_kernel<true, true>), grid, blk, 0, s, p, slabs, tn64);
         else if (epi_loads) hipLaunchKernelGGL((conv_nn_astat2_kernel<false, true>), grid, blk, 0, s, p, slabs, tn64);
         else if (pre) hipLaunchKernelGGL((conv_nn_astat2_kernel<true, false>), grid, blk, 0, s, p, slabs, tn64);
         else hipLaunchKernelGGL((conv_nn_astat2_kernel<false, false>), grid, blk, 0, s, p, slabs, tn64);
@@ -1652,6 +1698,23 @@
     }
     }
     return mk_check_launch("mk_conv1x1_nn");
+}
+
+extern "C" int mk_conv1x1_nn(const void* A, const void* X, void* Y, void* Ypre, const float* bias, const void* R,
+                             const void* G, int M, int K, int lda, int B, long long N, int act, void* stream) {
+    return conv1x1_nn_impl(A, X, Y, Ypre, bias, R, G, nullptr, nullptr, M, K, lda, B, N, act, stream);
+}
+
+extern "C" int mk_conv1x1_nn_affine(const void* A, const void* X, void* Y, const void* R, const float* r_affine, const float* r_pre_bias,
+                                    int M, int K, int lda, int B, long long N, void* stream) {
+    MK_REQUIRE(r_affine, "conv1x1_nn_affine: null pointer");
+    return conv1x1_nn_impl(A, X, Y, nullptr, nullptr, R, nullptr, r_affine, r_pre_bias, M, K, lda, B, N, 0, stream);
+}
+
+extern "C" int mk_conv1x1_nn_affine_ok(int M, int K, int lda, int B, long long N) {
+    static const int astat2_env = env_int("MAKANI_AMD_ASTAT2");
+    if (M <= 0 || K <= 0 || B <= 0 || N <= 0 || (N % 8) || (lda % 8) || lda < K) return 0;
+    return conv_nn_plan(M, K, lda, B, N, false, true, false, astat2_env, true) == ConvNnKernel::astat2 ? 1 : 0;
 }
 
 namespace {
diff --git a/makani_amd/csrc/conv1x1_plan.h b/makani_amd/csrc/conv1x1_plan.h
--- a/makani_amd/csrc/conv1x1_plan.h
+++ b/makani_amd/csrc/conv1x1_plan.h
@@ -8,11 +8,12 @@
     tile
 };
 
-inline ConvNnKernel conv_nn_plan(int M, int K, int lda, int B, long long N, bool pre, bool has_r, bool has_g, int astat2_env) {
+inline ConvNnKernel conv_nn_plan(int M, int K, int lda, int B, long long N, bool pre, bool has_r, bool has_g, int astat2_env,
+                                 bool r_affine = false) {
     const bool stationary = M >= 256 && (long long)M * N * 2 < (1ll << 31) && N >= 64 && !(has_r && has_g);
     if (stationary && lda == 80 && K > 64 && K <= 80 && (long long)K * N * 2 < (1ll << 32) && !((has_r || has_g) && pre))
         return ConvNnKernel::astat73;
-    const bool small_ring = M == 384 && (long long)B * N <= 32768 && !pre && astat2_env != 1;
+    const bool small_ring = M == 384 && (long long)B * N <= 32768 && !pre && astat2_env != 1 && !r_affine;
     if (stationary && K == 384 && !small_ring) return astat2_env == 0 ? ConvNnKernel::astat1 : ConvNnKernel::astat2;
     if (K >= 64 && M >= 192 && N * 2 * 64 < (1ll << 31) && (long long)M * lda * 2 < (1ll << 31) && N >= 256) return ConvNnKernel::ring;
     return ConvNnKernel::tile;
diff --git a/makani_amd/csrc/pointwise.hip b/makani_amd/csrc/pointwise.hip
--- a/makani_amd/csrc/pointwise.hip
+++ b/makani_amd/csrc/pointwise.hip
@@ -547,6 +547,99 @@
             if (GELU) gelu_n<T, VEC>(o);
             VecIO<T>::store(yp + e, o);
         }
+    }
+}
+
+template <typename T>
+__global__ __launch_bounds__(NT) void in_stats_fused_partial(const T* __restrict__ x, float* __restrict__ ws, int channels,
+                                                             long long hw, int chunks, const float* __restrict__ pre_bias) {
+    constexpr int VEC = VecIO<T>::N;
+    constexpr int FUSED_SLOTS = fused_slots(0);
+    typedef typename VecIO<T>::Raw Raw;
+    __shared__ float red[2 * NT / 64];
+    const long long plane = blockIdx.x / chunks;
+    const int chunk = blockIdx.x % chunks;
+    const int c = (int)(plane % channels);
+    const bool has_pb = pre_bias != nullptr;
+    const float pb = has_pb ? pre_bias[c] : 0.f;
+    const T* xp = x + plane * hw;
+    const long long len = chunk_len(hw, chunks, VEC);
+    const long long c0 = (long long)chunk * len;
+    const long long c1 = min(hw, c0 + len);
+    Raw raw[FUSED_SLOTS];
+#pragma unroll
+    for (int s = 0; s < FUSED_SLOTS; ++s) {
+        const long long e = c0 + ((long long)s * NT + threadIdx.x) * VEC;
+        raw[s] = VecIO<T>::load_raw(xp + (e < c1 ? e : c0));
+    }
+    const float pivot = pre<T>(VecIO<T>::load1(xp), pb, has_pb);
+    float s1 = 0.f, s2 = 0.f;
+#pragma unroll
+    for (int s = 0; s < FUSED_SLOTS; ++s) {
+        const long long e = c0 + ((long long)s * NT + threadIdx.x) * VEC;
+        if (e < c1) {
+            float v[VEC];
+            VecIO<T>::unpack(raw[s], v);
+#pragma unroll
+            for (int i = 0; i < VEC; ++i) {
+                const float d = pre<T>(v[i], pb, has_pb) - pivot;
+                s1 += d;
+                s2 += d * d;
+            }
+        }
+    }
+    block_reduce2(s1, s2, red);
+    if (threadIdx.x == 0) {
+        ws[2 * (long long)blockIdx.x] = s1;
+        ws[2 * (long long)blockIdx.x + 1] = s2;
+    }
+}
+
+template <typename T>
+__global__ __launch_bounds__(NT) void in_stats_fused_final(const T* __restrict__ x, const float* __restrict__ ws, float* __restrict__ stats,
+                                                           float* __restrict__ affine, const float* __restrict__ gamma,
+                                                           const float* __restrict__ beta, float eps, int channels, long long hw,
+                                                           int chunks, const float* __restrict__ pre_bias) {
+    __shared__ double redd[2 * NT / 64];
+    const long long plane = blockIdx.x;
+    const int c = (int)(plane % channels);
+    const bool has_pb = pre_bias != nullptr;
+    const float pb = has_pb ? pre_bias[c] : 0.f;
+    const float pivot = pre<T>(VecIO<T>::load1(x + plane * hw), pb, has_pb);
+    double a = 0.0, b2 = 0.0;
+    if ((int)threadIdx.x < chunks) {
+        a = (double)ws[2 * (plane * chunks + threadIdx.x)];
+        b2 = (double)ws[2 * (plane * chunks + threadIdx.x) + 1];
+    }
+#pragma unroll
+    for (int o = 32; o > 0; o >>= 1) {
+        a += __shfl_down(a, o, 64);
+        b2 += __shfl_down(b2, o, 64);
+    }
+    const int lane = threadIdx.x & 63, w = threadIdx.x >> 6;
+    if (lane == 0) {
+        redd[2 * w] = a;
+        redd[2 * w + 1] = b2;
+    }
+    __syncthreads();
+    if (threadIdx.x != 0) return;
+    double t1 = 0.0, t2 = 0.0;
+    for (int i = 0; i < NT / 64; ++i) {
+        t1 += redd[2 * i];
+        t2 += redd[2 * i + 1];
+    }
+    const double m = t1 / (double)hw;
+    double var = t2 / (double)hw - m * m;
+    if (var < 0.0) var = 0.0;
+    const float mean = (float)((double)pivot + m);
+    const float rstd = (float)(1.0 / sqrt(var + (double)eps));
+    stats[2 * plane] = mean;
+    stats[2 * plane + 1] = rstd;
+    if (affine) {
+        const float g = gamma ? gamma[c] : 1.f, b = beta ? beta[c] : 0.f;
+        const float sc = rstd * g, sh = b - mean * rstd * g;
+        affine[2 * plane] = sc;
+        affine[2 * plane + 1] = sh;
     }
 }
 
@@ -1013,6 +1106,25 @@
     return mk_check_launch("mk_instnorm_fwd_fused");
 }
 
+extern "C" int mk_instnorm_stats_fused(const void* x, int dtype, float* stats, float* affine, float* ws, const float* gamma,
+                                       const float* beta, const float* pre_bias, long long planes, int channels, long long hw,
+                                       float eps, void* stream) {
+    int rc = check_common(x, planes, hw, dtype, "instnorm_stats_fused");
+    if (rc) return rc;
+    const int ch = mk_instnorm_fused_chunks(hw, dtype, planes, 0);
+    MK_REQUIRE(ch > 0, "instnorm_stats_fused: plane shape not served (hw = %lld)", hw);
+    MK_REQUIRE(stats && ws && channels > 0, "instnorm_stats_fused: bad args");
+    hipStream_t s = (hipStream_t)stream;
+    if (dtype == MK_F32) {
+        hipLaunchKernelGGL(in_stats_fused_partial<float>, dim3((unsigned)(planes * ch)), dim3(NT), 0, s, (const float*)x, ws, channels, hw, ch, pre_bias);
+        hipLaunchKernelGGL(in_stats_fused_final<float>, dim3((unsigned)planes), dim3(NT), 0, s, (const float*)x, ws, stats, affine, gamma, beta, eps, channels, hw, ch, pre_bias);
+    } else {
+        hipLaunchKernelGGL(in_stats_fused_partial<u16>, dim3((unsigned)(planes * ch)), dim3(NT), 0, s, (const u16*)x, ws, channels, hw, ch, pre_bias);
+        hipLaunchKernelGGL(in_stats_fused_final<u16>, dim3((unsigned)planes), dim3(NT), 0, s, (const u16*)x, ws, stats, affine, gamma, beta, eps, channels, hw, ch, pre_bias);
+    }
+    return mk_check_launch("mk_instnorm_stats_fused");
+}
+
 extern "C" int mk_instnorm_bwd_fused(const void* x, const void* gy, void* gx, int dtype, const float* stats, const float* gamma,
                                      const float* beta, const float* pre_bias, float* sums, void* slots, void* depart, long long planes,
                                      int channels, long long hw, int fuse_gelu, void* stream) {
diff --git a/makani_amd/ops.py b/makani_amd/ops.py
--- a/makani_amd/ops.py
+++ b/makani_amd/ops.py
@@ -863,28 +863,48 @@
     @staticmethod
     def backward(ctx, gy):
         x, stats, g, b, pb, quad = ctx.saved_tensors
-        B, Cc, H, W = x.shape
-        planes, hw = B * Cc, H * W
-        gy = gy.contiguous()
-        if gy.dtype != x.dtype:
-            gy = gy.to(x.dtype)
-        gx = torch.empty_like(x)
-        sums = torch.empty((2, planes), dtype=torch.float32, device=x.device)
-        ch = _fused_norm_chunks(x, planes, hw, quad, 2 if ctx.fuse_gelu else 1)
-        if ch:
-            slots, depart = _fused_sync(planes * ch, planes, x.device)
-            with _timed(f"instnorm_bwd{'_gelu' if ctx.fuse_gelu else ''}_n{hw}", nbytes=3.0 * x.numel() * x.element_size()):
-                check(lib().mk_instnorm_bwd_fused(ptr(x), ptr(gy), ptr(gx), dtype_code(x), ptr(stats), ptr(g), ptr(b), ptr(pb), ptr(sums),
-                                                  ptr(slots), ptr(depart), planes, Cc, hw, 1 if ctx.fuse_gelu else 0, stream()), "instnorm_bwd_fused")
-        else:
-            ws = _ws(planes, hw, x.dtype, x.device)
-            with _timed(f"instnorm_bwd{'_gelu' if ctx.fuse_gelu else ''}_n{hw}", nbytes=5.0 * x.numel() * x.element_size()):
-                check(lib().mk_instnorm_bwd(ptr(x), ptr(gy), ptr(gx), dtype_code(x), ptr(stats), ptr(g), ptr(b), ptr(pb), ptr(quad),
-                                            ctx.quad_sum, ptr(sums), ptr(ws), planes, Cc, hw, hw, 0, 1 if ctx.fuse_gelu else 0,
-                                            stream()), "instnorm_bwd")
-        s = _batch_sum(sums, B, Cc)
+        gx, s = _instnorm_backward(x, stats, g, b, pb, quad, ctx.quad_sum, ctx.fuse_gelu, gy)
         gpb = torch.zeros_like(pb) if (pb is not None and ctx.needs_input_grad[5]) else None
         return gx, (s[1] if g is not None else None), (s[0] if b is not None else None), None, None, gpb, None, None
+
+
+def _instnorm_backward(x, stats, g, b, pb, quad, quad_sum, fuse_gelu, gy):
+    B, Cc, H, W = x.shape
+    planes, hw = B * Cc, H * W
+    gy = gy.contiguous()
+    if gy.dtype != x.dtype:
+        gy = gy.to(x.dtype)
+    gx = torch.empty_like(x)
+    sums = torch.empty((2, planes), dtype=torch.float32, device=x.device)
+    ch = _fused_norm_chunks(x, planes, hw, quad, 2 if fuse_gelu else 1)
+    if ch:
+        slots, depart = _fused_sync(planes * ch, planes, x.device)
+        with _timed(f"instnorm_bwd{'_gelu' if fuse_gelu else ''}_n{hw}", nbytes=3.0 * x.numel() * x.element_size()):
+            check(lib().mk_instnorm_bwd_fused(ptr(x), ptr(gy), ptr(gx), dtype_code(x), ptr(stats), ptr(g), ptr(b), ptr(pb), ptr(sums),
+                                              ptr(slots), ptr(depart), planes, Cc, hw, 1 if fuse_gelu else 0, stream()), "instnorm_bwd_fused")
+    else:
+        ws = _ws(planes, hw, x.dtype, x.device)
+        with _timed(f"instnorm_bwd{'_gelu' if fuse_gelu else ''}_n{hw}", nbytes=5.0 * x.numel() * x.element_size()):
+            check(lib().mk_instnorm_bwd(ptr(x), ptr(gy), ptr(gx), dtype_code(x), ptr(stats), ptr(g), ptr(b), ptr(pb), ptr(quad),
+                                        quad_sum, ptr(sums), ptr(ws), planes, Cc, hw, hw, 0, 1 if fuse_gelu else 0,
+                                        stream()), "instnorm_bwd")
+    return gx, _batch_sum(sums, B, Cc)
+
+
+def instance_norm_stats(x, gamma=None, beta=None, eps=1e-5, pre_bias=None):
+    x = x.contiguous()
+    B, Cc, H, W = x.shape
+    planes, hw = B * Cc, H * W
+    ch = int(lib().mk_instnorm_fused_chunks(hw, dtype_code(x), planes, 0))
+    if not ch:
+        raise RuntimeError(f"instance_norm_stats: the one-pass norm does not serve planes of {hw} elements")
+    stats = torch.empty((planes, 2), dtype=torch.float32, device=x.device)
+    affine = torch.empty((planes, 2), dtype=torch.float32, device=x.device)
+    ws = torch.empty((planes * ch * 2,), dtype=torch.float32, device=x.device)
+    with _timed(f"instnorm_stats_n{hw}", nbytes=1.0 * x.numel() * x.element_size()):
+        check(lib().mk_instnorm_stats_fused(ptr(x), dtype_code(x), ptr(stats), ptr(affine), ptr(ws), ptr(gamma), ptr(beta), ptr(pre_bias),
+                                            planes, Cc, hw, eps, stream()), "instnorm_stats_fused")
+    return stats, affine
 
 
 class ChannelLayerNormFn(torch.autograd.Function):
@@ -975,13 +995,21 @@
 
 
 def conv1x1_nn(A: torch.Tensor, K: int, x: torch.Tensor, bias=None, act=False, want_pre=False, residual=None,
-               gelu_grad_of=None):
+               gelu_grad_of=None, r_affine=None):
     B, Kx, H, W = x.shape
     assert Kx == K and x.dtype == torch.bfloat16 and A.dtype == torch.bfloat16
     x = x.contiguous()
     M, lda = A.shape
     N = H * W
     y = torch.empty((B, M, H, W), dtype=torch.bfloat16, device=x.device)
+    if r_affine is not None:
+        assert residual is not None and residual.dtype == torch.bfloat16 and bias is None and not act and gelu_grad_of is None
+        aff, rpb = r_affine
+        r = residual.contiguous()
+        with _timed(f"conv1x1_nn_affine_m{M}_k{K}_n{N}", flops=2.0 * B * M * K * N, nbytes=2.0 * B * N * (2 * M + K)):
+            check(lib().mk_conv1x1_nn_affine(ptr(A), ptr(x), ptr(y), ptr(r), ptr(aff), ptr(rpb), M, K, lda, B, N, stream()),
+                  "mk_conv1x1_nn_affine")
+        return y, None
     ypre = torch.empty_like(y) if (act and want_pre) else None
     bf = bias.float().contiguous() if bias is not None else None
     r = residual.contiguous() if residual is not None else None
@@ -1056,6 +1084,51 @@
         if ctx.has_res and ctx.needs_input_grad[3]:
             gr = gy
         return gx, gw, gb, gr
+
+
+def norm_skip_fusable(z: torch.Tensor, x: torch.Tensor, weight: torch.Tensor) -> bool:
+    if os.environ.get("MAKANI_AMD_FUSE_NORM1_SKIP", "1") == "0" or os.environ.get("MAKANI_AMD_NORM_FUSED", "1") != "1":
+        return False
+    if not (z.is_cuda and z.dtype == torch.bfloat16 and z.dim() == 4 and x.dim() == 4):
+        return False
+    B, K, H, W = x.shape
+    M = weight.shape[0]
+    if tuple(z.shape) != (B, M, H, W) or weight.shape[1] != K:
+        return False
+    return bool(lib().mk_instnorm_fused_chunks(H * W, _lib.MK_BF16, B * M, 0)) and bool(lib().mk_conv1x1_nn_affine_ok(M, K, round8(K), B, H * W))
+
+
+class NormSkipFn(torch.autograd.Function):
+
+    @staticmethod
+    def forward(ctx, z, gamma, beta, eps, pre_bias, x, weight):
+        z, x = z.contiguous(), x.contiguous()
+        M, K = weight.shape[0], weight.shape[1]
+        g = gamma.float().contiguous() if gamma is not None else None
+        b = beta.float().contiguous() if beta is not None else None
+        pb = pre_bias.float().contiguous() if pre_bias is not None else None
+        stats, affine = instance_norm_stats(z, g, b, eps, pb)
+        A, At = weight_operands(weight, need_t=ctx.needs_input_grad[5])
+        y, _ = conv1x1_nn(A, K, x, residual=z, r_affine=(affine, pb))
+        ctx.save_for_backward(z, stats, g, b, pb, x, weight, At)
+        return y
+
+    @staticmethod
+    def backward(ctx, gy):
+        z, stats, g, b, pb, x, weight, At = ctx.saved_tensors
+        M = weight.shape[0]
+        gy = gy.contiguous()
+        gz = gg = gb = gpb = gx = gw = None
+        if any(ctx.needs_input_grad[i] for i in (0, 1, 2)):
+            gz, s = _instnorm_backward(z, stats, g, b, pb, None, 0.0, False, gy)
+            gg, gb = (s[1] if g is not None else None), (s[0] if b is not None else None)
+        if pb is not None and ctx.needs_input_grad[4]:
+            gpb = torch.zeros_like(pb)
+        if ctx.needs_input_grad[5]:
+            gx, _ = conv1x1_nn(At, M, gy)
+        if ctx.needs_input_grad[6]:
+            gw = conv1x1_wgrad(gy, x).view_as(weight)
+        return gz, gg, gb, None, gpb, gx, gw
 
 
 class ConvGeluConvFn(torch.autograd.Function):
diff --git a/makani_amd/sfno.py b/makani_amd/sfno.py
--- a/makani_amd/sfno.py
+++ b/makani_amd/sfno.py
@@ -8,7 +8,9 @@
 from torch.utils.checkpoint import checkpoint
 
 from . import distributed as thd
-from .layers import MLP, ChannelLayerNorm, DropPath, EncoderDecoder, GeometricInstanceNormS2, InstanceNorm2d, PointwiseConv
+from . import ops
+from .layers import (MLP, ChannelLayerNorm, DropPath, EncoderDecoder, GeometricInstanceNormS2, InstanceNorm2d, PointwiseConv,
+                     hip_conv_eligible)
 from .sht import InverseRealSHT, RealSHT
 from .spectral_conv import SpectralConv
 
@@ -71,6 +73,12 @@
         if final_activation:
             self.act_layer1 = act_layer()
 
+    def _norm1_rides_in_skip(self, z, residual):
+        return (type(self.norm1) is InstanceNorm2d and hasattr(self, "mlp") and hasattr(self, "outer_skip")
+                and self.outer_skip.bias is None and isinstance(self.drop_path, nn.Identity) and not hasattr(self, "act_layer1")
+                and z.dim() == 4 and z.shape[1] == self.norm1.num_features and hip_conv_eligible(residual)
+                and ops.norm_skip_fusable(z, residual, self.outer_skip.weight))
+
     @torch.compiler.disable(recursive=True)
     def forward(self, x):
         x, residual = self.filter(x)
@@ -80,13 +88,15 @@
         else:
             x = self.act_layer0(self.norm0(x))
 
+        pb = None
         if hasattr(self, "mlp") and type(self.norm1) is InstanceNorm2d and self.mlp.can_defer_output_bias(x):
             x, pb = self.mlp.forward_deferred_bias(x)
-            x = self.norm1(x, pre_bias=pb)
-        else:
-            if hasattr(self, "mlp"):
-                x = self.mlp(x)
-            x = self.norm1(x)
+        elif hasattr(self, "mlp"):
+            x = self.mlp(x)
+        if self._norm1_rides_in_skip(x, residual):
+            return ops.NormSkipFn.apply(x, self.norm1.weight, self.norm1.bias, self.norm1.eps, pb,
+                                        residual.to(torch.bfloat16), self.outer_skip.weight)
+        x = self.norm1(x, pre_bias=pb) if pb is not None else self.norm1(x)
         x = self.drop_path(x)
 
         if hasattr(self, "outer_skip"):
```

Measured after the change: 28.32 samples/s (median of 6 runs). +1.1%, better.
